# MCG-NJU/LinK

Hardware: AMD Instinct MI355X
Metric: voxels/s through one LinK (3x7)^3 block, 100k active voxels C=64 (higher is better)
Workload: dtype f32

## Files before the change

include/link_amd.h:

```cpp
#ifndef LINK_AMD_H_
#define LINK_AMD_H_

#include <stddef.h>
#include <stdint.h>

#ifdef __cplusplus
extern "C" {
#endif

#define LINK_OK 0
#define LINK_ERR_ARG (-1)
#define LINK_ERR_LAUNCH (-2)
#define LINK_ERR_WORKSPACE (-3)
#define LINK_BATCH_TIMEOUT (-4)

int link_abi_version(void);
int32_t link_abi_struct_size(int32_t which);
const char *link_last_error(void);


int link_hash(const int32_t *coords, int64_t n, int64_t *out, void *stream);

int link_kernel_hash(const int32_t *coords, int64_t n, const int32_t *offsets, int64_t k,
                     int64_t *out, void *stream);
// ... 70 lines not shown
                               const int32_t *counts, const int32_t *nbr_t, const float *denom,
                               int64_t n, int64_t m, int64_t c, int64_t k, float *g_new,
                               float *g_small, void *stream);
int link_aux_to_voxel_forward_grid(const float *small_f, const int32_t *counts, const int32_t *blk_coords,
                                   const int32_t *cell_blk, const link_grid_t *grid ,
                                   const int32_t *hdr, const int64_t *idx, int64_t n, int64_t m, int32_t w,
                                   int32_t r, float *S, float *new_feat, float *denom, float *out,
                                   void *stream);
int link_aux_to_voxel_forward_scatter(const float *small_f, const int32_t *counts, const int32_t *blk_coords,
                                      const int32_t *cell_blk, const link_grid_t *grid , const int32_t *hdr,
                                      const int32_t *blk_start, const int32_t *perm, int64_t n, int64_t m, int32_t w, int32_t r,
                                      float *S , float *denom, float *out, void *stream);


#define LINK_OP_COS 0
#define LINK_OP_SIN 1
#define LINK_OP_COSX 2

typedef struct {
  int32_t op;
  int32_t c;
  int32_t cg;
  int32_t r;
  float coord_div;
  float eps;
  int32_t flags;
} link_elk_desc_t;
#define LINK_ELK_LANE_CHANNEL 1
#define LINK_ELK_NO_PAIR 2
#define LINK_ELK_FUSED_GATHER 4
#define LINK_ELK_NO_DENSE_GRID 8
#define LINK_ELK_LEAN_CS 32
#define LINK_ELK_LEAN_NO_CS 64
#define LINK_ELK_LEAN_PM 128
#define LINK_ELK_LEAN_NO_PM 256
#define LINK_ELK_TILES 16

int link_premix_ln(const float *feats, const float *w_pre, const float *ln_w, const float *ln_b,
                   int64_t n, int32_t c, float eps, float *fin, void *stream);

int link_modulate_block_sum(const float *fin, const int32_t *vox_sorted, const float *w_pos,
                            const float *alpha, const int32_t *blk_start,
                            const int32_t *hdr, const link_elk_desc_t *desc , int64_t n,
                            int64_t m_cap, float *S, void *stream);

int link_gather_demod_ln(const float *S, const float *fin, const int32_t *vox_sorted,
                         const float *w_pos, const float *alpha, const float *ln_w, const float *ln_b,
                         const int32_t *blk_start, const int32_t *blk_coords,
                         const int32_t *cell_blk, const link_grid_t *grid ,
                         const int32_t *hdr, const link_elk_desc_t *desc , int64_t n,
                         int64_t m_cap, float *out, void *stream);

int link_block_gather(const float *S, const int32_t *blk_coords, const int32_t *cell_blk,
                      const link_grid_t *grid , const int32_t *hdr,
                      const link_elk_desc_t *desc , int64_t m_cap, float *A, void *stream);
int link_voxel_demod_ln(const float *A, const float *fin, const int32_t *vox_sorted,
                        const int32_t *pos_blk, const float *w_pos, const float *alpha, const float *ln_w,
                        const float *ln_b, const int32_t *hdr, const link_elk_desc_t *desc ,
                        int64_t n, float *out, void *stream);

typedef struct {
  const void *feats;
  const int32_t *coords;
  const float *w_pre, *pre_ln_w, *pre_ln_b;
  const float *w_pos, *alpha;
  const float *ln_w, *ln_b;
  uint32_t *cell_counts; void *scratch; size_t scratch_bytes;
  int32_t *cell_blk, *vox_blk; int64_t *idx_query; int32_t *perm, *vox_sorted, *pos_blk, *blk_start, *blk_coords, *counts, *hdr;
  float *fin;
  float *S;
  float *A;
  void *out;
  int64_t s_bytes;
  int32_t io_dtype;
  int32_t reserved;
  uint64_t *cell_pair;
} link_elk_buffers_t;

int64_t link_elk_tiles_table_bytes(const link_elk_desc_t *desc , int64_t n, int64_t m_cap);
int link_elk_premix_modsum_tiles(const float *feats, const int32_t *vox_sorted, const int32_t *pos_blk,
                                 const int32_t *blk_start, const int32_t *hdr, const float *w_pre,
                                 const float *pre_ln_w, const float *pre_ln_b, const float *w_pos, const float *alpha,
                                 const link_elk_desc_t *desc , int64_t n, int64_t m_cap, float *S,
                                 int64_t s_bytes, float *fin, void *stream);
int link_elk_gather_demod_tiles(const float *S, const float *fin, const int32_t *vox_sorted, const int32_t *pos_blk,
                                const int32_t *blk_coords, const int32_t *cell_blk, const link_grid_t *grid ,
                                const int32_t *hdr, const float *w_pos, const float *alpha, const float *ln_w,
                                const float *ln_b, const link_elk_desc_t *desc , int64_t n, int64_t m_cap,
                                float *out, void *stream);
int link_elk_premix_modsum_tiles_io(const void *feats, int32_t io_dtype, const int32_t *vox_sorted, const int32_t *pos_blk,
                                    const int32_t *blk_start, const int32_t *hdr, const float *w_pre, const float *pre_ln_w,
                                    const float *pre_ln_b, const float *w_pos, const float *alpha,
                                    const link_elk_desc_t *desc , int64_t n, int64_t m_cap, float *S,
                                    int64_t s_bytes, float *fin, void *stream);
int link_elk_gather_demod_tiles_io(const float *S, const float *fin, const int32_t *vox_sorted, const int32_t *pos_blk,
                                   const int32_t *blk_coords, const int32_t *cell_blk, const link_grid_t *grid ,
                                   const int32_t *hdr, const float *w_pos, const float *alpha, const float *ln_w,
                                   const float *ln_b, const link_elk_desc_t *desc , int64_t n, int64_t m_cap,
                                   void *out, int32_t io_dtype, void *stream);

int link_elk_core_forward(const link_elk_buffers_t *buf , const link_grid_t *grid ,
                          const link_elk_desc_t *desc , int64_t n, int64_t m_cap,
                          int32_t build_index, void *stream);

typedef struct {
  const void *feats;
  const int32_t *coords;
  const float *w_pre, *pre_ln_w, *pre_ln_b, *w_pos, *alpha, *ln_w, *ln_b;
  uint32_t *cnt, *cnt_prev;
  int32_t *list;
  int32_t *rec2;
  int32_t *occ, *occ_prev;
  uint32_t *ctrl, *ctrl_prev;
  float *X;
  float *S;
  int32_t *hdr;
  void *out;
  int64_t seg_cap;
  int32_t k;
  int32_t io_dtype;
  int32_t cnt_shift;
  int32_t reserved;
} link_lean_buffers_t;
int link_elk_core_lean_forward(const link_lean_buffers_t *buf , const link_grid_t *grid ,
                               const link_elk_desc_t *desc , int64_t n, int64_t n_prev, int32_t build_index,
                               void *stream);

int link_elk_mid_forward(const float *fin, const int32_t *vox_sorted, const int32_t *pos_blk,
                         const int32_t *blk_start, const int32_t *blk_coords, const int32_t *cell_blk,
                         const link_grid_t *grid , const int32_t *hdr, const float *w_pos,
                         const float *alpha, const link_elk_desc_t *desc , const float *ln_w,
                         const float *ln_b, int64_t n, int64_t m_cap, float *S, float *A, float *den,
                         float *out, void *stream);
int32_t link_elk_mid_partial_rows(void);
int link_elk_out_ln_backward(const float *g_out, const float *A, const float *fin, const int32_t *vox_sorted,
                             const int32_t *pos_blk, const float *w_pos, const float *alpha,
                             const float *ln_w, const int32_t *hdr, const link_elk_desc_t *desc ,
                             int64_t n, float *g_new, float *partials, void *stream);
int link_elk_mid_backward(const float *g_new, const float *fin, const float *A, const float *den,
                          const int32_t *vox_sorted, const int32_t *pos_blk, const int32_t *blk_start,
                          const int32_t *blk_coords, const int32_t *cell_blk,
                          const link_grid_t *grid , const int32_t *hdr, const float *w_pos,
                          const float *alpha, const link_elk_desc_t *desc , int64_t n, int64_t m_cap,
                          float *S, float *gS, float *g_fin, float *partials, void *stream);
int link_premix_ln_backward(const float *feats, const float *w_pre, const float *ln_w, const float *g_fin,
                            int64_t n, int32_t c, float eps, float *g_pre, float *g_feats, float *partials,
                            void *stream);
int link_ln_add_relu_forward(const float *x, const float *addend, const float *ln_w, const float *ln_b,
                             int64_t n, int32_t c, float eps, float *y, void *stream);
int link_ln_add_relu_backward(const float *g_y, const float *y, const float *x, const float *ln_w, int64_t n,
                              int32_t c, float eps, float *g_addend, float *g_x, float *partials, void *stream);
int link_premix_ln_io(const void *feats, int32_t io_dtype, const float *w_pre, const float *ln_w, const float *ln_b,
                      int64_t n, int32_t c, float eps, float *fin, void *stream);
int link_premix_ln_backward_io(const void *feats, int32_t io_dtype, const float *w_pre, const float *ln_w,
                               const float *g_fin, int64_t n, int32_t c, float eps, float *g_pre, void *g_feats,
                               float *partials, void *stream);
int link_ln_add_relu_forward_io(const void *x, int32_t io_dtype, const float *addend, const float *ln_w,
                                const float *ln_b, int64_t n, int32_t c, float eps, float *y, void *stream);
int link_ln_add_relu_backward_io(const float *g_y, const float *y, const void *x, int32_t io_dtype, const float *ln_w,
                                 int64_t n, int32_t c, float eps, float *g_addend, void *g_x, float *partials,
                                 void *stream);
int link_sum_partials(const float *p0, int32_t cols0, const float *p1, int32_t cols1, const float *p2,
                      int32_t cols2, int64_t rows, float *out, void *stream);

int link_subm_conv_forward(const float *feats, const int32_t *nbr, const float *w, const int32_t *order,
                           int64_t n, int32_t cin, int32_t cout, int32_t kvol, float *out, void *stream);
int link_subm_conv_ln_add_relu(const float *feats, const int32_t *nbr, const float *w, const int32_t *order,
                               int64_t n, int32_t cin, int32_t cout, int32_t kvol, const float *ln_w,
                               const float *ln_b, float eps, const float *addend, int32_t relu, float *out,
                               void *stream);
int32_t link_subm_conv_wgrad_chunks(void);
int link_subm_conv_wgrad(const float *feats, const float *gout, const int32_t *nbr_t, int64_t n, int32_t c,
                         int32_t kvol, float *partial, void *stream);
int link_subm_conv_wgrad_split(const float *feats, const float *gout, const int32_t *nbr_t, int64_t n, int32_t c, int32_t kvol,
                               int32_t chunks, int32_t centre_extra, float *partial, void *stream);
int link_subm_conv_wgrad_reduce(const float *partial, int32_t c, int32_t kvol, int32_t chunks, int32_t centre_extra, float *gw,
                                void *stream);

int link_conv_pairs_supported(int32_t cin, int32_t cout);
int link_conv_pairs_gemm(const float *feats, const int32_t *pair_in, const int32_t *wg_k, int64_t rows_pad,
                         const float *w, int32_t cin, int32_t cout, float *contrib, void *stream);
int link_conv_pairs_sum(const float *contrib, const int32_t *ext_start, const int32_t *ext_list, int64_t n,
                        int64_t n_direct, int32_t cout, const float *bias, const float *ln_w, const float *ln_b,
                        float eps, const float *addend, int32_t relu, float *out, void *stream);
int32_t link_conv_out_candidate_count(const int32_t *kernel, const int32_t *stride);
int link_conv_out_candidates(const int32_t *indices, int64_t n, const int32_t *kernel, const int32_t *stride,
                             const int32_t *padding, const int32_t *out_shape, int32_t *cand, void *stream);
int link_conv_site_table(const int32_t *indices, int64_t n, const int32_t *in_shape, int32_t batch, int32_t *table,
                         int32_t clear, void *stream);
int link_conv_gather_table(const int32_t *out_indices, int64_t m, const int32_t *kernel, const int32_t *stride,
                           const int32_t *padding, const int32_t *in_shape, int32_t batch, const int32_t *site_table,
                           int32_t *table, void *stream);
int32_t link_kmap_candidate_count(const int32_t *kernel, const int32_t *stride);
int link_kmap_out_candidates(const int32_t *coords, int64_t n, const int32_t *kernel, const int32_t *stride,
                             const int32_t *tensor_stride, const int32_t *lo, int32_t *cand, void *stream);
int link_kmap_box_table(const int32_t *rows, int64_t m, const int32_t *cell_tab, const link_grid_t *grid,
                        const int32_t *kernel, const int32_t *step, int32_t *table, void *stream);
int link_kmap_transpose(const int32_t *table, int64_t m, int32_t kvol, int64_t n_in, int32_t *back, void *stream);
int link_pair_plan_count(const int32_t *nbr, int64_t n, int32_t kvol, int32_t *wg_counts, int32_t *row_info, void *stream);
int link_pair_plan_fill(const int32_t *nbr, int64_t n, int32_t kvol, int32_t skip_centre, const int32_t *base_k,
                        const int32_t *wg_base, const int32_t *ext_start, int32_t *pair_in, int32_t *pair_out,
                        int32_t *ext_list, void *stream);
int link_pair_plan_layout(const int32_t *wg_counts, int64_t n, int32_t kvol, int32_t skip_centre, int64_t gran_cap,
                          int32_t *base_k, int32_t *wg_base, int32_t *gran_start, int32_t *wg_k, int32_t *hdr, void *stream);
int link_pair_plan_build(const int32_t *nbr, int64_t n, int32_t kvol, int32_t skip_centre, int64_t gran_cap, int32_t *wg_counts,
                         int32_t *row_info, int32_t *base_k, int32_t *wg_base, int32_t *gran_start, int32_t *wg_ext,
                         int32_t *wg_k, int32_t *hdr, int32_t *ext_start, int32_t *pair_in, int32_t *pair_out,
                         int32_t *ext_list, void *stream);
int link_conv_pairs_gemm_io(const void *feats, int32_t io_dtype, const int32_t *pair_in, const int32_t *wg_k, int64_t rows_pad,
                            const float *w, int32_t cin, int32_t cout, float *contrib, void *stream);
int link_conv_pairs_sum_io(const float *contrib, const int32_t *ext_start, const int32_t *ext_list, int64_t n,
                           int64_t n_direct, int32_t cout, const float *bias, const float *ln_w, const float *ln_b, float eps,
                           const void *addend, int32_t relu, void *out, int32_t io_dtype, void *stream);
int link_conv_centre_sum_io(const void *feats, const float *w, int32_t centre, const float *contrib, int64_t contrib_rows,
                            const int32_t *ext_start, const int32_t *ext_list, int64_t n, int32_t cin, int32_t cout,
                            const float *bias, const float *ln_w, const float *ln_b, float eps, const void *addend,
                            int32_t relu, void *out, int32_t io_dtype, void *stream);
int link_conv_pairs_gemm_split(const float *feats, const int32_t *pair_in, const int32_t *wg_k, int64_t rows_pad, const void *ws,
                               const float *w, const int32_t *w_big, int32_t cin, int32_t cout, float *contrib, void *stream);
int link_conv_pairs_gemm_amp(const void *feats, int32_t io_dtype, const int32_t *pair_in, const int32_t *wg_k, int64_t rows_pad,
                             const void *wt, int32_t cin, int32_t cout, void *contrib, int32_t contrib_dtype, void *stream);
int link_conv_centre_sum_amp(const void *feats, const void *wt, int32_t centre, const void *contrib, int32_t contrib_dtype,
                             int64_t contrib_rows, const int32_t *ext_start, const int32_t *ext_list, int64_t n, int32_t cin,
                             int32_t cout, const float *bias, const float *ln_w, const float *ln_b, float eps,
                             const void *addend, int32_t relu, void *out, int32_t io_dtype, void *stream);
int link_subm_conv_resident_amp(const void *feats, int32_t io_dtype, const int32_t *nbr, const void *wt, const int32_t *order,
                                int64_t n, int32_t cin, int32_t cout, int32_t kvol, const float *ln_w, const float *ln_b,
                                float eps, const void *addend, int32_t relu, void *out, void *stream);
int link_conv_pairs_wgrad(const float *feats, const float *gout, const int32_t *pair_in, const int32_t *pair_out,
                          const int32_t *wg_k, const int32_t *gran_start, int64_t rows_pad, int32_t kvol, int64_t n_direct,
                          int32_t cin, int32_t cout, float *partial, float *gw, void *stream);
int link_conv_centre_sum(const float *feats, const float *w, int32_t centre, const float *contrib,
                         int64_t contrib_rows, const int32_t *ext_start, const int32_t *ext_list, int64_t n, int32_t cin, int32_t cout,
                         const float *bias, const float *ln_w, const float *ln_b, float eps, const float *addend,
                         int32_t relu, float *out, void *stream);

typedef struct {
  int32_t s;
  int32_t lo[4];
  int32_t dim[4];
  int32_t pdim[3];
  int32_t k;
  int64_t vp;
} link_dc_grid_t;
int64_t link_dc_grid_from(const link_grid_t *grid, int32_t k, link_dc_grid_t *out);

#define LINK_HDR_STATUS_ACC 3

#define LINK_IO_F32 0
#define LINK_IO_F16 1
#define LINK_IO_BF16 2
typedef struct {
  int32_t k1_wgs;
  int32_t k2_zsplit;
  int32_t k1_lds_pad;
  int32_t k2_lds_pad;
  int32_t k1_form;
  int32_t k2_form;
  int32_t mode;
  int32_t reserved0;
  int32_t reserved;
  uint64_t *k1_dbg;
  uint64_t *k2_dbg;
} link_dc_tuning_t;

typedef struct {
  const void *feats;
  const int32_t *coords;
  const float *w_pre, *pre_ln_w, *pre_ln_b, *w_pos, *alpha, *ln_w, *ln_b;
  uint32_t *cnt;
  int32_t *slots;
  uint32_t *sid;
  int32_t *vrec;
  int32_t *vcell;
  int32_t *cell_n;
  int32_t *hdr;
  float *fin;
  float *S;
  float *A;
  void *out;
  int32_t io_dtype;
  link_dc_tuning_t tune;
} link_dc_buffers_t;

int link_dc_premix_insert(const float *feats, const int32_t *coords, const float *w_pre, const float *ln_w,
                          const float *ln_b, int64_t n, int32_t c, float eps, const link_dc_grid_t *g ,
                          int32_t insert, float *fin, uint32_t *cnt, int32_t *slots, int32_t *vrec,
                          int32_t *vcell, int32_t *hdr, void *stream);
int link_dc_modsum(const float *fin, const int32_t *slots, uint32_t *cnt, int32_t *cell_n, const float *w_pos,
                   const float *alpha, const link_elk_desc_t *desc , const link_dc_grid_t *g ,
                   int32_t warm, float *S, int32_t *hdr, void *stream);
int link_dc_gather(const float *S, const int32_t *cell_n, const link_elk_desc_t *desc ,
                   const link_dc_grid_t *g , float *A, void *stream);
int link_dc_index(const int32_t *coords, int64_t n, const link_dc_grid_t *g , uint32_t *cnt,
                  int32_t *slots, int32_t *vcell, int32_t *hdr, void *stream);
int link_dc_premix_modsum(const link_dc_buffers_t *buf , const link_dc_grid_t *g ,
                          const link_elk_desc_t *desc , int64_t n, int32_t warm, void *stream);
int link_dc_demod(const float *A, const float *fin, const int32_t *coords, const int32_t *vcell,
                  const float *w_pos, const float *alpha, const float *ln_w, const float *ln_b,
                  const link_elk_desc_t *desc , const link_dc_grid_t *g , int64_t n, void *out,
                  int32_t io_dtype, void *stream);
int link_dc_gather_demod(const link_dc_buffers_t *buf , const link_dc_grid_t *g ,
                         const link_elk_desc_t *desc , int64_t n, void *stream);
int link_elk_core_dense_forward(const link_dc_buffers_t *buf , const link_dc_grid_t *g ,
                                const link_elk_desc_t *desc , int64_t n, int32_t build_index,
                                void *stream);
int link_dc_index_probe(const link_dc_buffers_t *buf , const link_dc_grid_t *g , int64_t n, int32_t *stats,
                        void *stream);
int link_dc_index_ids(const int32_t *coords, int64_t n, const link_dc_grid_t *g , uint32_t *cnt,
                      uint32_t *sid, int32_t *vcell, int32_t *hdr, void *stream);

int32_t link_bn_partial_workgroups(int64_t n, int32_t c);
int link_bn_forward_stats(const float *x, int64_t n, int32_t c, float eps, float momentum, double *partial, float *mean,
                          float *invstd, float *running_mean, float *running_var, const float *weight ,
                          const float *bias , float *scale , float *shift, void *stream);
int link_bn_backward_reduce(const float *g, const float *x, const float *mean, const float *invstd, int64_t n, int32_t c,
                            double *partial, float *sum_g, float *sum_gx, const float *weight ,
                            float *coef , void *stream);
int link_bn_apply_forward(const float *x, const float *mean, const float *scale, const float *shift, int64_t n, int32_t c,
                          int32_t relu, float *y, void *stream);
int link_bn_backward_reduce_relu(const float *g, const float *x, const float *mean, const float *invstd, const float *scale,
                                 const float *shift, int64_t n, int32_t c, double *partial, float *sum_g, float *sum_gx,
                                 const float *weight , float *coef , void *stream);
int link_bn_apply_backward(const float *g, const float *x, const float *mean, const float *coef, const float *scale ,
                           const float *shift, int64_t n, int32_t c, float *gx, void *stream);
int link_bn_forward_stats_io(const void *x, int32_t io_dtype, int64_t n, int32_t c, float eps, float momentum, double *partial,
                             float *mean, float *invstd, float *running_mean, float *running_var, const float *weight,
                             const float *bias, float *scale, float *shift, void *stream);
int link_bn_apply_forward_io(const void *x, int32_t io_dtype, const float *mean, const float *scale, const float *shift, int64_t n,
                             int32_t c, int32_t relu, void *y, void *stream);
int link_bn_backward_reduce_io(const void *g, const void *x, int32_t io_dtype, const float *mean, const float *invstd, int64_t n,
                               int32_t c, double *partial, float *sum_g, float *sum_gx, const float *weight, float *coef,
                               void *stream);
int link_bn_backward_reduce_relu_io(const void *g, const void *x, int32_t io_dtype, const float *mean, const float *invstd,
                                    const float *scale, const float *shift, int64_t n, int32_t c, double *partial, float *sum_g,
                                    float *sum_gx, const float *weight, float *coef, void *stream);
int link_bn_apply_backward_io(const void *g, const void *x, int32_t io_dtype, const float *mean, const float *coef,
                              const float *scale , const float *shift, int64_t n, int32_t c, void *gx,
                              void *stream);

typedef struct link_block_ctx link_block_ctx_t;
int link_block_ctx_create(link_block_ctx_t **out);
int link_block_ctx_destroy(link_block_ctx_t *ctx);
int64_t link_pair_plan_arena(int64_t n, int32_t kvol, int32_t skip_centre, int64_t offs[11]);

int link_dc_neighbor_map(const int32_t *coords, int64_t n, const link_dc_grid_t *g , const uint32_t *cnt,
                         const int32_t *slots, int32_t step, int32_t *nbr, void *stream);

#define LINK_BLOCK_DONE 0
#define LINK_BLOCK_MISS 1
typedef struct {
  const link_dc_buffers_t *buf;
  const link_dc_grid_t *g;
  const link_elk_desc_t *desc;
  int64_t n;
  int32_t mean_max, cell_max;
  int32_t ts;
  int32_t subm;
  int32_t *nbr;
  int32_t *pair_arena;
  int64_t pair_arena_words;
  float *contrib;
  int64_t contrib_rows;
  const float *w;
  const void *ws;
  const int32_t *w_big;
  const float *nl_w, *nl_b;
  float nl_eps;
  int32_t flags;
  void *out;
  int32_t bbox[8];
  int32_t stats[4];
  int32_t verdict;
  int32_t reserved;
} link_block_args_t;
int link_elk_block_forward(link_block_ctx_t *ctx, link_block_args_t *args , void *stream);

typedef struct link_dc_batch link_dc_batch_t;
int link_dc_batch_create(link_dc_batch_t **out);
int link_dc_batch_destroy(link_dc_batch_t *ctx);
int link_elk_core_dense_forward_batch(link_dc_batch_t *ctx, const link_dc_buffers_t *frames ,
                                      const int64_t *n , int32_t nframes, const link_dc_grid_t *g ,
                                      const link_elk_desc_t *desc , void *stream);
int link_dc_batch_submit(link_dc_batch_t *ctx, const link_dc_buffers_t *frames , const int64_t *n ,
                         int32_t nframes, const link_dc_grid_t *g , const link_elk_desc_t *desc , void *stream,
                         int64_t *ticket );
int link_dc_batch_join(link_dc_batch_t *ctx, int64_t ticket, void *stream);
int link_dc_batch_status(link_dc_batch_t *ctx, int32_t *out );
int link_dc_batch_set_timing(link_dc_batch_t *ctx, int32_t on);
int link_dc_batch_kernel_times(link_dc_batch_t *ctx, int64_t ticket, float *ms );
int link_dc_batch_set_debug(link_dc_batch_t *ctx, uint64_t *k1_rows, uint64_t *k2_rows);
int link_streams_share_queue(void *stream_a, void *stream_b, double *delay_us );
int link_dc_batch_probe_streams(link_dc_batch_t *ctx, hipStream_t stream, double *delays_us );

#ifdef __cplusplus
}
#endif
#endif
```

link_amd/_lib.py:

```python
from __future__ import annotations

import ctypes
import os
from ctypes import POINTER, Structure, c_char_p, c_float, c_int, c_int32, c_int64, c_size_t, c_void_p

_HERE = os.path.dirname(os.path.abspath(__file__))
SO_PATH = os.path.join(_HERE, "lib", "liblink_amd.so")

LINK_OK, LINK_ERR_ARG, LINK_ERR_LAUNCH, LINK_ERR_WORKSPACE, LINK_BATCH_TIMEOUT = 0, -1, -2, -3, -4
HDR_M, HDR_STATUS, HDR_NVALID, HDR_STATUS_ACC, HDR_WORDS = 0, 1, 2, 3, 8
OP_COS, OP_SIN, OP_COSX = 0, 1, 2
ELK_LANE_CHANNEL, ELK_NO_PAIR, ELK_FUSED_GATHER, ELK_NO_DENSE_GRID, ELK_TILES = 1, 2, 4, 8, 16
ELK_LEAN_CS, ELK_LEAN_NO_CS, ELK_LEAN_PM, ELK_LEAN_NO_PM = 32, 64, 128, 256
IO_F32, IO_F16, IO_BF16 = 0, 1, 2
ABI_VERSION = 13
DEBUG = os.environ.get("LINK_AMD_DEBUG", "0") not in ("", "0")


class LinkGrid(Structure):
    _fields_ = [("s", c_int32), ("lo", c_int32 * 4), ("dim", c_int32 * 4)]

    @property
    def cells(self) -> int:
        v = 1
        for d in self.dim:
            v *= int(d)
        return v

    def key(self):
        return (int(self.s), tuple(int(x) for x in self.lo), tuple(int(x) for x in self.dim))


class LinkElkDesc(Structure):
    _fields_ = [("op", c_int32), ("c", c_int32), ("cg", c_int32), ("r", c_int32),
                ("coord_div", c_float), ("eps", c_float), ("flags", c_int32)]


class LinkElkBuffers(Structure):
    _fields_ = [(k, c_void_p) for k in ("feats", "coords", "w_pre", "pre_ln_w", "pre_ln_b", "w_pos", "alpha",
                                        "ln_w", "ln_b", "cell_counts", "scratch")] + \
               [("scratch_bytes", c_size_t)] + \
               [(k, c_void_p) for k in ("cell_blk", "vox_blk", "idx_query", "perm", "vox_sorted", "pos_blk", "blk_start",
                                        "blk_coords", "counts", "hdr", "fin", "S", "A", "out")] + \
               [("s_bytes", c_int64), ("io_dtype", c_int32), ("reserved", c_int32), ("cell_pair", c_void_p)]


class LinkDcGrid(Structure):
    _fields_ = [("s", c_int32), ("lo", c_int32 * 4), ("dim", c_int32 * 4), ("pdim", c_int32 * 3),
                ("k", c_int32), ("vp", c_int64)]

    @property
    def interior_cells(self) -> int:
        v = 1
        for d in self.dim:
            v *= int(d)
        return v


class LinkDcTuning(Structure):
    _fields_ = [(k, c_int32) for k in ("k1_wgs", "k2_zsplit", "k1_lds_pad", "k2_lds_pad", "k1_form", "k2_form", "mode",
                                       "reserved0", "reserved")] + [("k1_dbg", c_void_p), ("k2_dbg", c_void_p)]


class LinkDcBuffers(Structure):
    _fields_ = [(k, c_void_p) for k in ("feats", "coords", "w_pre", "pre_ln_w", "pre_ln_b", "w_pos", "alpha",
                                        "ln_w", "ln_b", "cnt", "slots", "sid", "vrec", "vcell", "cell_n", "hdr", "fin",
                                        "S", "A", "out")] + [("io_dtype", c_int32), ("tune", LinkDcTuning)]


class LinkLeanBuffers(Structure):
    _fields_ = [(k, c_void_p) for k in ("feats", "coords", "w_pre", "pre_ln_w", "pre_ln_b", "w_pos", "alpha", "ln_w", "ln_b",
                                        "cnt", "cnt_prev", "list", "rec2", "occ", "occ_prev", "ctrl", "ctrl_prev", "X", "S",
                                        "hdr", "out")] + [("seg_cap", c_int64), ("k", c_int32), ("io_dtype", c_int32), ("cnt_shift", c_int32), ("reserved", c_int32)]


LEAN_KMAX, LEAN_SEGS, LEAN_CHUNK = 352, 16, 32
BLOCK_DONE, BLOCK_MISS = 0, 1


class LinkBlockArgs(Structure):
    _fields_ = [("buf", POINTER(LinkDcBuffers)), ("g", POINTER(LinkDcGrid)), ("desc", POINTER(LinkElkDesc)), ("n", c_int64),
                ("mean_max", c_int32), ("cell_max", c_int32), ("ts", c_int32), ("subm", c_int32),
                ("nbr", c_void_p), ("pair_arena", c_void_p),
                ("pair_arena_words", c_int64), ("contrib", c_void_p), ("contrib_rows", c_int64), ("w", c_void_p), ("ws", c_void_p),
                ("w_big", c_void_p), ("nl_w", c_void_p), ("nl_b", c_void_p), ("nl_eps", c_float), ("flags", c_int32),
                ("out", c_void_p), ("bbox", c_int32 * 8), ("stats", c_int32 * 4), ("verdict", c_int32), ("reserved", c_int32)]


SIGNATURES = {
    "link_abi_version": (c_int, []),
    "link_abi_struct_size": (c_int32, [c_int32]),
    "link_last_error": (c_char_p, []),
    "link_hash": (c_int, [c_void_p, c_int64, c_void_p, c_void_p]),
    "link_kernel_hash": (c_int, [c_void_p, c_int64, c_void_p, c_int64, c_void_p, c_void_p]),
    "link_hash_query_workspace_bytes": (c_size_t, [c_int64]),
    "link_hash_query": (c_int, [c_void_p, c_int64, c_void_p, c_void_p, c_int64, c_void_p, c_void_p,
                                c_size_t, c_void_p]),
    "link_count": (c_int, [c_void_p, c_int64, c_void_p, c_int64, c_void_p]),
    "link_ti_weights": (c_int, [c_void_p, c_void_p, c_int64, c_float, c_void_p, c_void_p]),
    "link_voxelize_forward": (c_int, [c_void_p, c_void_p, c_void_p, c_int64, c_int64, c_int64, c_void_p,
                                      c_void_p]),
    "link_voxelize_backward": (c_int, [c_void_p, c_void_p, c_void_p, c_int64, c_int64, c_void_p, c_void_p]),
    "link_devoxelize_forward": (c_int, [c_void_p, c_void_p, c_void_p, c_int64, c_int64, c_int64, c_void_p,
                                        c_void_p]),
    "link_devoxelize_backward": (c_int, [c_void_p, c_void_p, c_void_p, c_int64, c_int64, c_int64, c_int64,
                                         c_void_p, c_void_p]),
    "link_grid_from_bounds": (c_int64, [POINTER(c_int32), POINTER(c_int32), c_int32, POINTER(LinkGrid)]),
    "link_coords_bbox": (c_int, [c_void_p, c_int64, c_void_p, c_void_p]),
    "link_index_scratch_bytes": (c_size_t, [c_int64, c_int64]),
    "link_index_build": (c_int, [c_void_p, c_int64, POINTER(LinkGrid), c_void_p, c_void_p, c_size_t,
                                 c_void_p, c_void_p, c_void_p, c_void_p, c_void_p, c_void_p, c_void_p,
                                 c_void_p, c_void_p, c_void_p, c_void_p]),
    "link_index_build_first": (c_int, [c_void_p, c_int64, POINTER(LinkGrid), c_void_p, c_void_p, c_size_t] + [c_void_p] * 11),
    "link_block_gather": (c_int, [c_void_p, c_void_p, c_void_p, POINTER(LinkGrid), c_void_p,
                                  POINTER(LinkElkDesc), c_int64, c_void_p, c_void_p]),
    "link_voxel_demod_ln": (c_int, [c_void_p, c_void_p, c_void_p, c_void_p, c_void_p, c_void_p, c_void_p,
                                    c_void_p, c_void_p, POINTER(LinkElkDesc), c_int64, c_void_p, c_void_p]),
    "link_neighbor_map": (c_int, [c_void_p, c_void_p, POINTER(LinkGrid), c_void_p, c_int64, c_int32,
                                  c_int32, c_int32, c_void_p, c_void_p]),
    "link_cell_table_build": (c_int, [c_void_p, c_int64, POINTER(LinkGrid), c_void_p, c_void_p, c_void_p]),
    "link_conv_site_table": (c_int, [c_void_p, c_int64, c_void_p, c_int32, c_void_p, c_int32, c_void_p]),
    "link_conv_gather_table": (c_int, [c_void_p, c_int64, c_void_p, c_void_p, c_void_p, c_void_p, c_int32, c_void_p, c_void_p,
                                       c_void_p]),
    "link_cell_table_clear": (c_int, [c_void_p, c_int64, POINTER(LinkGrid), c_void_p, c_void_p]),
    "link_block_mean": (c_int, [c_void_p, c_void_p, c_void_p, c_void_p, c_int64, c_int64, c_int64,
                                c_void_p, c_void_p]),
    "link_aux_to_voxel_forward": (c_int, [c_void_p, c_void_p, c_void_p, c_void_p, c_int64, c_int64,
                                          c_int64, c_int64, c_void_p, c_void_p, c_void_p, c_void_p]),
    "link_aux_to_voxel_backward": (c_int, [c_void_p, c_void_p, c_void_p, c_void_p, c_void_p, c_void_p,
                                           c_int64, c_int64, c_int64, c_int64, c_void_p, c_void_p,
                                           c_void_p]),
    "link_premix_ln": (c_int, [c_void_p, c_void_p, c_void_p, c_void_p, c_int64, c_int32, c_float,
                               c_void_p, c_void_p]),
    "link_modulate_block_sum": (c_int, [c_void_p, c_void_p, c_void_p, c_void_p, c_void_p,
                                        c_void_p, POINTER(LinkElkDesc), c_int64, c_int64, c_void_p,
                                        c_void_p]),
    "link_gather_demod_ln": (c_int, [c_void_p, c_void_p, c_void_p, c_void_p, c_void_p, c_void_p, c_void_p,
                                     c_void_p, c_void_p, c_void_p, POINTER(LinkGrid), c_void_p,
                                     POINTER(LinkElkDesc), c_int64, c_int64, c_void_p, c_void_p]),
    "link_elk_core_forward": (c_int, [POINTER(LinkElkBuffers), POINTER(LinkGrid), POINTER(LinkElkDesc),
                                      c_int64, c_int64, c_int32, c_void_p]),
    "link_elk_tiles_table_bytes": (c_int64, [POINTER(LinkElkDesc), c_int64, c_int64]),
    "link_elk_premix_modsum_tiles": (c_int, [c_void_p] * 10 + [POINTER(LinkElkDesc), c_int64, c_int64, c_void_p, c_int64,
                                             c_void_p, c_void_p]),
    "link_elk_gather_demod_tiles": (c_int, [c_void_p] * 6 + [POINTER(LinkGrid)] + [c_void_p] * 5 +
                                    [POINTER(LinkElkDesc), c_int64, c_int64, c_void_p, c_void_p]),
    "link_elk_premix_modsum_tiles_io": (c_int, [c_void_p, c_int32] + [c_void_p] * 9 + [POINTER(LinkElkDesc), c_int64, c_int64, c_void_p,
                                                c_int64, c_void_p, c_void_p]),
    "link_elk_gather_demod_tiles_io": (c_int, [c_void_p] * 6 + [POINTER(LinkGrid)] + [c_void_p] * 5 +
                                       [POINTER(LinkElkDesc), c_int64, c_int64, c_void_p, c_int32, c_void_p]),
    "link_elk_mid_forward": (c_int, [c_void_p] * 6 + [POINTER(LinkGrid), c_void_p, c_void_p, c_void_p,
                                     POINTER(LinkElkDesc), c_void_p, c_void_p, c_int64, c_int64] + [c_void_p] * 5),
    "link_elk_out_ln_backward": (c_int, [c_void_p] * 9 + [POINTER(LinkElkDesc), c_int64, c_void_p, c_void_p,
                                         c_void_p]),
    "link_subm_conv_forward": (c_int, [c_void_p, c_void_p, c_void_p, c_void_p, c_int64, c_int32, c_int32, c_int32,
                                       c_void_p, c_void_p]),
    "link_aux_to_voxel_forward_grid": (c_int, [c_void_p] * 4 + [POINTER(LinkGrid), c_void_p, c_void_p, c_int64,
                                               c_int64, c_int32, c_int32] + [c_void_p] * 5),
    "link_aux_to_voxel_forward_scatter": (c_int, [c_void_p] * 4 + [POINTER(LinkGrid), c_void_p, c_void_p, c_void_p, c_int64,
                                                  c_int64, c_int32, c_int32] + [c_void_p] * 4),
    "link_conv_pairs_supported": (c_int, [c_int32, c_int32]),
    "link_conv_pairs_gemm": (c_int, [c_void_p, c_void_p, c_void_p, c_int64, c_void_p, c_int32, c_int32, c_void_p, c_void_p]),
    "link_conv_pairs_sum": (c_int, [c_void_p, c_void_p, c_void_p, c_int64, c_int64, c_int32, c_void_p, c_void_p, c_void_p,
                                    c_float, c_void_p, c_int32, c_void_p, c_void_p]),
    "link_index_cells": (c_int, [c_void_p, c_int64, POINTER(LinkGrid), c_void_p, c_void_p, c_size_t, c_void_p, c_void_p, c_void_p,
                                 c_void_p, c_void_p, c_void_p]),
    "link_conv_out_candidate_count": (c_int32, [c_void_p, c_void_p]),
    "link_conv_out_candidates": (c_int, [c_void_p, c_int64, c_void_p, c_void_p, c_void_p, c_void_p, c_void_p, c_void_p]),
    "link_kmap_candidate_count": (c_int32, [c_void_p, c_void_p]),
    "link_kmap_out_candidates": (c_int, [c_void_p, c_int64, c_void_p, c_void_p, c_void_p, c_void_p, c_void_p, c_void_p]),
    "link_kmap_box_table": (c_int, [c_void_p, c_int64, c_void_p, POINTER(LinkGrid), c_void_p, c_void_p, c_void_p, c_void_p]),
    "link_kmap_transpose": (c_int, [c_void_p, c_int64, c_int32, c_int64, c_void_p, c_void_p]),
    "link_conv_pairs_gemm_io": (c_int, [c_void_p, c_int32, c_void_p, c_void_p, c_int64, c_void_p, c_int32, c_int32, c_void_p, c_void_p]),
    "link_conv_pairs_sum_io": (c_int, [c_void_p, c_void_p, c_void_p, c_int64, c_int64, c_int32, c_void_p, c_void_p, c_void_p,
                                       c_float, c_void_p, c_int32, c_void_p, c_int32, c_void_p]),
    "link_conv_centre_sum_io": (c_int, [c_void_p, c_void_p, c_int32, c_void_p, c_int64, c_void_p, c_void_p, c_int64, c_int32, c_int32,
                                        c_void_p, c_void_p, c_void_p, c_float, c_void_p, c_int32, c_void_p, c_int32, c_void_p]),
    "link_conv_pairs_gemm_amp": (c_int, [c_void_p, c_int32, c_void_p, c_void_p, c_int64, c_void_p, c_int32, c_int32, c_void_p, c_int32, c_void_p]),
    "link_conv_centre_sum_amp": (c_int, [c_void_p, c_void_p, c_int32, c_void_p, c_int32, c_int64, c_void_p, c_void_p, c_int64, c_int32, c_int32,
                                         c_void_p, c_void_p, c_void_p, c_float, c_void_p, c_int32, c_void_p, c_int32, c_void_p]),
    "link_bn_partial_workgroups": (c_int32, [c_int64, c_int32]),
    "link_bn_forward_stats": (c_int, [c_void_p, c_int64, c_int32, c_float, c_float, c_void_p, c_void_p, c_void_p, c_void_p, c_void_p,
                                      c_void_p, c_void_p, c_void_p, c_void_p, c_void_p]),
    "link_bn_backward_reduce": (c_int, [c_void_p, c_void_p, c_void_p, c_void_p, c_int64, c_int32, c_void_p, c_void_p, c_void_p,
                                        c_void_p, c_void_p, c_void_p]),
    "link_bn_apply_forward": (c_int, [c_void_p, c_void_p, c_void_p, c_void_p, c_int64, c_int32, c_int32, c_void_p, c_void_p]),
    "link_bn_backward_reduce_relu": (c_int, [c_void_p, c_void_p, c_void_p, c_void_p, c_void_p, c_void_p, c_int64, c_int32, c_void_p,
                                             c_void_p, c_void_p, c_void_p, c_void_p, c_void_p]),
    "link_bn_apply_backward": (c_int, [c_void_p, c_void_p, c_void_p, c_void_p, c_void_p, c_void_p, c_int64, c_int32, c_void_p, c_void_p]),
    "link_conv_pairs_gemm_split": (c_int, [c_void_p, c_void_p, c_void_p, c_int64, c_void_p, c_void_p, c_void_p, c_int32, c_int32, c_void_p, c_void_p]),
    "link_pair_plan_count": (c_int, [c_void_p, c_int64, c_int32, c_void_p, c_void_p, c_void_p]),
    "link_pair_plan_fill": (c_int, [c_void_p, c_int64, c_int32, c_int32, c_void_p, c_void_p, c_void_p, c_void_p, c_void_p, c_void_p,
                                    c_void_p]),
    "link_subm_conv_resident_amp": (c_int, [c_void_p, c_int32, c_void_p, c_void_p, c_void_p, c_int64, c_int32, c_int32, c_int32,
                                            c_void_p, c_void_p, c_float, c_void_p, c_int32, c_void_p, c_void_p]),
    "link_pair_plan_build": (c_int, [c_void_p, c_int64, c_int32, c_int32, c_int64] + [c_void_p] * 13),
    "link_pair_plan_layout": (c_int, [c_void_p, c_int64, c_int32, c_int32, c_int64, c_void_p, c_void_p, c_void_p, c_void_p, c_void_p,
                                      c_void_p]),
    "link_conv_pairs_wgrad": (c_int, [c_void_p, c_void_p, c_void_p, c_void_p, c_void_p, c_void_p, c_int64, c_int32, c_int64,
                                      c_int32, c_int32, c_void_p, c_void_p, c_void_p]),
    "link_conv_centre_sum": (c_int, [c_void_p, c_void_p, c_int32, c_void_p, c_int64, c_void_p, c_void_p, c_int64, c_int32, c_int32,
                                     c_void_p, c_void_p, c_void_p, c_float, c_void_p, c_int32, c_void_p, c_void_p]),
    "link_subm_conv_wgrad_chunks": (c_int32, []),
    "link_subm_conv_wgrad": (c_int, [c_void_p, c_void_p, c_void_p, c_int64, c_int32, c_int32, c_void_p, c_void_p]),
    "link_subm_conv_wgrad_split": (c_int, [c_void_p, c_void_p, c_void_p, c_int64, c_int32, c_int32, c_int32, c_int32, c_void_p, c_void_p]),
    "link_subm_conv_wgrad_reduce": (c_int, [c_void_p, c_int32, c_int32, c_int32, c_int32, c_void_p, c_void_p]),
    "link_subm_conv_ln_add_relu": (c_int, [c_void_p, c_void_p, c_void_p, c_void_p, c_int64, c_int32, c_int32, c_int32,
                                           c_void_p, c_void_p, c_float, c_void_p, c_int32, c_void_p, c_void_p]),
    "link_ln_add_relu_forward": (c_int, [c_void_p] * 4 + [c_int64, c_int32, c_float, c_void_p, c_void_p]),
    "link_ln_add_relu_backward": (c_int, [c_void_p] * 4 + [c_int64, c_int32, c_float] + [c_void_p] * 4),
    "link_sum_partials": (c_int, [c_void_p, c_int32, c_void_p, c_int32, c_void_p, c_int32, c_int64, c_void_p,
                                  c_void_p]),
    "link_premix_ln_backward": (c_int, [c_void_p] * 4 + [c_int64, c_int32, ctypes.c_float] + [c_void_p] * 4),
    "link_premix_ln_io": (c_int, [c_void_p, c_int32] + [c_void_p] * 3 + [c_int64, c_int32, c_float, c_void_p, c_void_p]),
    "link_premix_ln_backward_io": (c_int, [c_void_p, c_int32] + [c_void_p] * 3 + [c_int64, c_int32, c_float] + [c_void_p] * 4),
    "link_ln_add_relu_forward_io": (c_int, [c_void_p, c_int32] + [c_void_p] * 3 + [c_int64, c_int32, c_float, c_void_p, c_void_p]),
    "link_ln_add_relu_backward_io": (c_int, [c_void_p] * 3 + [c_int32, c_void_p, c_int64, c_int32, c_float] + [c_void_p] * 4),
    "link_bn_forward_stats_io": (c_int, [c_void_p, c_int32, c_int64, c_int32, c_float, c_float] + [c_void_p] * 10),
    "link_bn_apply_forward_io": (c_int, [c_void_p, c_int32, c_void_p, c_void_p, c_void_p, c_int64, c_int32, c_int32, c_void_p, c_void_p]),
    "link_bn_backward_reduce_io": (c_int, [c_void_p, c_void_p, c_int32, c_void_p, c_void_p, c_int64, c_int32] + [c_void_p] * 6),
    "link_bn_backward_reduce_relu_io": (c_int, [c_void_p, c_void_p, c_int32] + [c_void_p] * 4 + [c_int64, c_int32] + [c_void_p] * 6),
    "link_bn_apply_backward_io": (c_int, [c_void_p, c_void_p, c_int32] + [c_void_p] * 4 + [c_int64, c_int32, c_void_p, c_void_p]),
    "link_elk_mid_partial_rows": (c_int32, []),
    "link_dc_grid_from": (c_int64, [POINTER(LinkGrid), c_int32, POINTER(LinkDcGrid)]),
    "link_dc_premix_insert": (c_int, [c_void_p] * 5 + [c_int64, c_int32, c_float, POINTER(LinkDcGrid), c_int32] +
                              [c_void_p] * 7),
    "link_dc_modsum": (c_int, [c_void_p] * 6 + [POINTER(LinkElkDesc), POINTER(LinkDcGrid), c_int32, c_void_p,
                               c_void_p, c_void_p]),
    "link_dc_gather": (c_int, [c_void_p, c_void_p, POINTER(LinkElkDesc), POINTER(LinkDcGrid), c_void_p, c_void_p]),
    "link_elk_core_dense_forward": (c_int, [POINTER(LinkDcBuffers), POINTER(LinkDcGrid), POINTER(LinkElkDesc),
                                            c_int64, c_int32, c_void_p]),
    "link_elk_core_lean_forward": (c_int, [POINTER(LinkLeanBuffers), POINTER(LinkGrid), POINTER(LinkElkDesc), c_int64, c_int64,
                                           c_int32, c_void_p]),
    "link_dc_index_probe": (c_int, [POINTER(LinkDcBuffers), POINTER(LinkDcGrid), c_int64, c_void_p, c_void_p]),
    "link_dc_index_ids": (c_int, [c_void_p, c_int64, POINTER(LinkDcGrid)] + [c_void_p] * 5),
    "link_dc_index": (c_int, [c_void_p, c_int64, POINTER(LinkDcGrid)] + [c_void_p] * 5),
    "link_dc_premix_modsum": (c_int, [POINTER(LinkDcBuffers), POINTER(LinkDcGrid), POINTER(LinkElkDesc), c_int64,
                                      c_int32, c_void_p]),
    "link_dc_gather_demod": (c_int, [POINTER(LinkDcBuffers), POINTER(LinkDcGrid), POINTER(LinkElkDesc), c_int64, c_void_p]),
    "link_dc_demod": (c_int, [c_void_p] * 8 + [POINTER(LinkElkDesc), POINTER(LinkDcGrid), c_int64, c_void_p, c_int32,
                              c_void_p]),
    "link_block_ctx_create": (c_int, [POINTER(c_void_p)]),
    "link_block_ctx_destroy": (c_int, [c_void_p]),
    "link_pair_plan_arena": (c_int64, [c_int64, c_int32, c_int32, POINTER(c_int64)]),
    "link_dc_neighbor_map": (c_int, [c_void_p, c_int64, POINTER(LinkDcGrid), c_void_p, c_void_p, c_int32, c_void_p, c_void_p]),
    "link_elk_block_forward": (c_int, [c_void_p, POINTER(LinkBlockArgs), c_void_p]),
    "link_dc_batch_create": (c_int, [POINTER(c_void_p)]),
    "link_dc_batch_destroy": (c_int, [c_void_p]),
    "link_elk_core_dense_forward_batch": (c_int, [c_void_p, POINTER(LinkDcBuffers), POINTER(c_int64), c_int32, POINTER(LinkDcGrid),
                                                  POINTER(LinkElkDesc), c_void_p]),
    "link_dc_batch_submit": (c_int, [c_void_p, POINTER(LinkDcBuffers), POINTER(c_int64), c_int32, POINTER(LinkDcGrid),
                                     POINTER(LinkElkDesc), c_void_p, POINTER(c_int64)]),
    "link_dc_batch_join": (c_int, [c_void_p, c_int64, c_void_p]),
    "link_dc_batch_set_timing": (c_int, [c_void_p, c_int32]),
    "link_dc_batch_kernel_times": (c_int, [c_void_p, c_int64, POINTER(c_float)]),
    "link_dc_batch_status": (c_int, [c_void_p, POINTER(c_int32)]),
    "link_dc_batch_set_debug": (c_int, [c_void_p, c_void_p, c_void_p]),
    "link_dc_batch_probe_streams": (c_int, [c_void_p, c_void_p, POINTER(ctypes.c_double)]),
    "link_streams_share_queue": (c_int, [c_void_p, c_void_p, POINTER(ctypes.c_double)]),
    "link_elk_mid_backward": (c_int, [c_void_p] * 9 + [POINTER(LinkGrid), c_void_p, c_void_p, c_void_p,
                                      POINTER(LinkElkDesc), c_int64, c_int64] + [c_void_p] * 5),
}

_lib = None


class LinkAmdError(RuntimeError):
    pass


def lib() -> ctypes.CDLL:
    global _lib
    if _lib is None:
        if not os.path.exists(SO_PATH):
            raise LinkAmdError(
                f"{SO_PATH} not found: the HIP extension is not built. Run `python link_amd/build.py` "
                "(or __graft_entry__.build()). link_amd has no CPU/PyTorch fallback.")
        handle = ctypes.CDLL(SO_PATH)
        for name, (res, args) in SIGNATURES.items():
            fn = getattr(handle, name)
            fn.restype = res
            fn.argtypes = args
        if handle.link_abi_version() != ABI_VERSION:
            raise LinkAmdError("liblink_amd.so ABI version mismatch; rebuild with link_amd/build.py")
        for which, cls in enumerate((LinkGrid, LinkElkDesc, LinkElkBuffers, LinkDcGrid, LinkDcTuning, LinkDcBuffers, LinkLeanBuffers, LinkBlockArgs)):
            if handle.link_abi_struct_size(which) != ctypes.sizeof(cls):
                raise LinkAmdError(f"liblink_amd.so: layout of {cls.__name__} differs from include/link_amd.h "
                                   f"({ctypes.sizeof(cls)} bytes here, {handle.link_abi_struct_size(which)} in the library)")
        _lib = handle
    return _lib


def current_stream_handle() -> int:
    import torch
    try:
        return torch._C._cuda_getCurrentRawStream(torch._C._cuda_getDevice())
    except AttributeError:
        return torch.cuda.current_stream().cuda_stream


def check(rc: int, what: str) -> None:
    if rc != LINK_OK:
        msg = {LINK_ERR_ARG: "invalid argument", LINK_ERR_LAUNCH: "HIP launch failure",
               LINK_ERR_WORKSPACE: "workspace too small",
               LINK_BATCH_TIMEOUT: "a bounded wait inside a persistent batch kernel gave up"}.get(rc, f"error {rc}")
        detail = lib().link_last_error()
        raise LinkAmdError(f"{what}: {msg}" + (f" ({detail.decode()})" if detail else ""))


def grid_from_bounds(lo, hi, s: int) -> LinkGrid:
    g = LinkGrid()
    lo_a = (c_int32 * 4)(*[int(x) for x in lo])
    hi_a = (c_int32 * 4)(*[int(x) for x in hi])
    v = lib().link_grid_from_bounds(lo_a, hi_a, int(s), ctypes.byref(g))
    if v < 0:
        raise LinkAmdError(f"grid_from_bounds({list(lo)}, {list(hi)}, s={s}): bounds invalid or grid "
                           ">= 2^30 cells")
    return g


def dc_grid_from(grid: LinkGrid, k: int = 0):
    g = LinkDcGrid()
    v = lib().link_dc_grid_from(ctypes.byref(grid), int(k), ctypes.byref(g))
    return g if v > 0 else None
```

link_amd/csrc/dense_batch_impl.h:

```cpp
#include <stdlib.h>

#include <type_traits>
#include <vector>

#include "dense_batch_common.h"
#include "dense_gather.h"
#include "dense_io.h"

namespace DC_IO_NS {
using namespace link;

#include "dense_k1_impl.h"
#include "dense_k2_cfg.h"
#include "dense_gather_quad_impl.h"

static_assert(DC_ST_AUX == 16, "the S rows must leave the L2 (sc1) for the in-launch hand-off K1 -> K2");

struct dc_bt_frame_t {
  const void *feats; const int4 *coords; int4 *slots; uint32_t *cnt; int32_t *cell_n; int32_t *vcell; float *S; int32_t *hdr;
  void *out; int64_t n;
};
struct dc_bt_frames_t { dc_bt_frame_t f[DC_BT_MAX]; };
struct dc_bt_par_t {
  const float *w_pre, *pre_ln_w, *pre_ln_b, *w_pos, *ln_w, *ln_b;
  int cg; float eps;
  unsigned long long *dbg1, *dbg2;
};
__device__ __forceinline__ void bt_row(unsigned long long *dbg, unsigned long long r, unsigned long long a, unsigned long long b,
                                       unsigned long long c, unsigned long long d, unsigned long long e, unsigned long long f) {
  if (!DC_BT_PROF || !dbg) return;
  if (r + 1 >= dbg[1]) return;
  unsigned long long *o = dbg + 8 * (r + 1);
  o[0] = a; o[1] = b; o[2] = c; o[3] = d; o[4] = e; o[5] = f; o[6] = 1;
}


template <typename P>
__device__ __forceinline__ bool bt_wait_ge(P sync, int word, int target, const int nap = 8) {
  int ok = 1;
  if ((threadIdx.x & 63) == 0) {
    const unsigned long long t0 = __builtin_amdgcn_s_memrealtime();
    int spins = 0;
    while (__hip_atomic_load(&sync[word], __ATOMIC_RELAXED, __HIP_MEMORY_SCOPE_AGENT) < target) {
      if (nap > 8) __builtin_amdgcn_s_sleep(64); else __builtin_amdgcn_s_sleep(8);
      if ((++spins & 15) == 0) {
        if (__hip_atomic_load(&sync[bt_err()], __ATOMIC_RELAXED, __HIP_MEMORY_SCOPE_AGENT) != 0) { ok = 0; break; }
        if (__builtin_amdgcn_s_memrealtime() - t0 > DC_BT_TIMEOUT_TICKS) {
          __hip_atomic_store(&sync[bt_err()], 1 + word, __ATOMIC_RELAXED, __HIP_MEMORY_SCOPE_AGENT);
          ok = 0;
          break;
        }
      }
    }
  }
  return __builtin_amdgcn_readfirstlane(ok) != 0;
}

struct dc_bt_ins_args_t { dc_bt_frames_t fr; link_dc_grid_t g; int nframes, wpf; int32_t *sync; };
__global__ void __launch_bounds__(64) k_dc_batch_insert(dc_bt_ins_args_t args_by_value) {
  (void)args_by_value;
#if defined(__HIP_DEVICE_COMPILE__)
  typedef const __attribute__((address_space(4))) dc_bt_ins_args_t *args_ptr_t;
  for (;;) {
    args_ptr_t a = (args_ptr_t)__builtin_amdgcn_kernarg_segment_ptr();
    asm volatile("" : "+s"(a));
    int t = 0;
    if (threadIdx.x == 0) t = __hip_atomic_fetch_add(&a->sync[bt_inscur()], 1, __ATOMIC_RELAXED, __HIP_MEMORY_SCOPE_AGENT);
    t = __builtin_amdgcn_readfirstlane(t);
    const int wpf = a->wpf;
    if (t >= a->nframes * wpf) break;
    const int f = t / wpf, j = t - f * wpf;
    if (f >= DC_BT_INS_LEAD && !bt_wait_ge(a->sync, bt_k1(f - DC_BT_INS_LEAD), 1, 64)) break;
    const link_dc_grid_t g = a->g;
    const int n = (int)a->fr.f[f].n;
    const int4 *__restrict__ coords = a->fr.f[f].coords;
    int32_t *__restrict__ vcell = a->fr.f[f].vcell;
    int32_t *__restrict__ hdr = a->fr.f[f].hdr;
    const __amdgpu_buffer_rsrc_t r_slots = dc_rsrc(a->fr.f[f].slots, (uint32_t)((int64_t)g.vp * g.k * 16));
    const __amdgpu_buffer_rsrc_t r_cnt = dc_rsrc(a->fr.f[f].cnt, (uint32_t)(g.vp * 4));
    if (j == 0 && threadIdx.x == 0) hdr[LINK_HDR_NVALID] = n;
    _Pragma("unroll 1") for (int k = 0; k < 4; k++) {
      const int v = (4 * j + k) * 64 + (int)threadIdx.x;
      if (v >= n) break;
      const int4 rc = coords[v];
      const unsigned ux = (unsigned)(floordiv(rc.x, g.s) - g.lo[0]), uy = (unsigned)(floordiv(rc.y, g.s) - g.lo[1]);
      const unsigned uz = (unsigned)(floordiv(rc.z, g.s) - g.lo[2]), ub = (unsigned)(rc.w - g.lo[3]);
      const bool inside = ux < (unsigned)g.dim[0] && uy < (unsigned)g.dim[1] && uz < (unsigned)g.dim[2] && ub < (unsigned)g.dim[3];
      if (!inside) atomicOr(&hdr[LINK_HDR_STATUS_ACC], 1);
      const int pcell = inside ? dc_cell(g, (int)ux, (int)uy, (int)uz, (int)ub) : 0;
      const int rank = __builtin_amdgcn_raw_ptr_buffer_atomic_add_i32(1, r_cnt, pcell ? (uint32_t)pcell * 4u : DC_OOB, 0, 0);
      const bool full = pcell != 0 && rank >= g.k;
      if (full) atomicOr(&hdr[LINK_HDR_STATUS_ACC], 2);
      const bool keep = pcell != 0 && !full;
      st16i_c<true>(r_slots, keep ? dc_slot(g, pcell, rank) * 16u : DC_OOB, make_int4(rc.x, rc.y, rc.z, v));
      vcell[v] = keep ? pcell : 0;
    }
    asm volatile("s_waitcnt vmcnt(0)" ::: "memory");
    if (threadIdx.x == 0) __hip_atomic_fetch_add(&a->sync[bt_ins(f)], 1, __ATOMIC_RELAXED, __HIP_MEMORY_SCOPE_AGENT);
  }
#endif
}

template <int OP, int NB>
__global__ void __launch_bounds__(64 * DC_K1_NW, DC_K1_WAVES) k_dc_batch_k1(dc_bt_frames_t fr, dc_bt_par_t p, link_dc_grid_t g, int nframes,
                                                                           int cpw, int nranges, int wpf, int32_t *__restrict__ sync) {
  constexpr int C = 64;
  extern __shared__ __attribute__((aligned(16))) char smem_raw[];
  const int tid = threadIdx.x, lane = tid & 63;
  bool w_big = false, th_big = false;
  dc_k1_stage<C, OP>(smem_raw, p.w_pre, p.pre_ln_w, p.pre_ln_b, p.w_pos, nullptr, p.cg, 1.0f, g, tid, w_big, th_big);
  w_big = DC_K1_SPLIT ? (__syncthreads_or(w_big) != 0) : (__syncthreads(), false);
  const bool th_slow = DC_THETA_BOUND ? __syncthreads_or(th_big) != 0 : false;
  const int Vi = g.dim[0] * g.dim[1] * g.dim[2] * g.dim[3];
  const int x = (int)(__builtin_amdgcn_s_getreg((4 - 1) << 11 | 0 << 6 | 20) & 7u);
  const int per = (nranges + 7) >> 3;
  const int lo = x * per;
  const int mine = (lo + per < nranges ? lo + per : nranges) - lo;
  if (mine <= 0) return;
  const int total = nframes * mine;
  int32_t *cur = &sync[bt_k1cur(x)];
  int t_next = 0;
  if (lane == 0) t_next = __hip_atomic_fetch_add(cur, 1, __ATOMIC_RELAXED, __HIP_MEMORY_SCOPE_AGENT);
  int pend_f = -1;
  int ins_known = -1;
  for (;;) {
    const int t = __builtin_amdgcn_readfirstlane(t_next);
    if (t >= total) break;
    const unsigned long long tp0 = DC_BT_PROF ? __builtin_amdgcn_s_memrealtime() : 0;
    const int f = t / mine, i = lo + (t - f * mine);
    if (lane == 0) t_next = __hip_atomic_fetch_add(cur, 1, __ATOMIC_RELAXED, __HIP_MEMORY_SCOPE_AGENT);
    const dc_bt_frame_t &F = fr.f[f];
    int ins_a = wpf, ins_b = wpf;
    if (lane == 0) {
      if (f > ins_known) ins_a = __hip_atomic_load(&sync[bt_ins(f)], __ATOMIC_RELAXED, __HIP_MEMORY_SCOPE_AGENT);
      if (f + 1 < nframes && f + 1 > ins_known) ins_b = __hip_atomic_load(&sync[bt_ins(f + 1)], __ATOMIC_RELAXED, __HIP_MEMORY_SCOPE_AGENT);
    }
    const int c_begin = i * cpw;
    const int c_end = (c_begin + cpw < Vi) ? c_begin + cpw : Vi;
    int pc_f, nv_f;
    int4 rf0, rf1, rf2, rf3;
    if (f <= ins_known) dc_k1_prefetch<true>(pc_f, nv_f, rf0, rf1, rf2, rf3, g, F.slots, F.cnt, c_begin, c_end, lane);
    asm volatile("s_waitcnt vmcnt(0)" ::: "memory");
    if (pend_f >= 0 && lane == 0) __hip_atomic_fetch_add(&sync[bt_k1(pend_f)], 1, __ATOMIC_RELAXED, __HIP_MEMORY_SCOPE_AGENT);
    pend_f = f;
    if (f > ins_known) {
      if (__builtin_amdgcn_readfirstlane(ins_a) < wpf && !bt_wait_ge(sync, bt_ins(f), wpf)) return;
      ins_known = f;
      dc_k1_prefetch<true>(pc_f, nv_f, rf0, rf1, rf2, rf3, g, F.slots, F.cnt, c_begin, c_end, lane);
    }
    if (f + 1 < nframes && f + 1 > ins_known && __builtin_amdgcn_readfirstlane(ins_b) >= wpf) ins_known = f + 1;
    if (i == 0 && lane == 0) {
      F.hdr[LINK_HDR_STATUS] = __hip_atomic_load(&F.hdr[LINK_HDR_STATUS_ACC], __ATOMIC_RELAXED, __HIP_MEMORY_SCOPE_AGENT);
      __hip_atomic_store(&F.hdr[LINK_HDR_STATUS_ACC], 0, __ATOMIC_RELAXED, __HIP_MEMORY_SCOPE_AGENT);
    }
    const unsigned long long tp1 = DC_BT_PROF ? __builtin_amdgcn_s_memrealtime() : 0;
    dc_k1_range<C, OP, NB, false, true>(smem_raw, F.feats, F.slots, F.cnt, F.cell_n, p.w_pre, 1.0f, p.eps, F.n, g, false, F.S, nullptr,
                                        nullptr, c_begin, c_end, pc_f, nv_f, rf0, rf1, rf2, rf3, w_big, th_slow, i, 0, 0);
    if (DC_BT_PROF && lane == 0) bt_row(p.dbg1, (unsigned long long)f * nranges + i, (unsigned long long)f, (unsigned long long)i, tp0, tp1, __builtin_amdgcn_s_memrealtime(), (unsigned long long)(blockIdx.x * 4 + (tid >> 6)));
  }
  asm volatile("s_waitcnt vmcnt(0)" ::: "memory");
#if DC_BT_RELEASE_FENCE
  __builtin_amdgcn_fence(__ATOMIC_RELEASE, "agent");
  asm volatile("s_waitcnt vmcnt(0)" ::: "memory");
#endif
  if (pend_f >= 0 && lane == 0) __hip_atomic_fetch_add(&sync[bt_k1(pend_f)], 1, __ATOMIC_RELAXED, __HIP_MEMORY_SCOPE_AGENT);
}

struct dc_bt_k2_args_t {
  dc_bt_frames_t fr;
  dc_bt_par_t p;
  link_dc_grid_t g;
  int nframes, txn, tyn, zsplit, nwg, k1_target;
  int32_t *sync;
};

template <int OP, int R>
__global__ void __launch_bounds__(256 + 64 * (DC_K2Q_CW + (DC_K2Q_PMAP ? 1 : 0)), 4) k_dc_batch_k2(dc_bt_k2_args_t args_by_value) {
  (void)args_by_value;
#if defined(__HIP_DEVICE_COMPILE__)
  static_assert(DC_K2Q_PMAP == 1, "the mapper wave draws the items");
  typedef const __attribute__((address_space(4))) dc_bt_k2_args_t *args_ptr_t;
  constexpr unsigned CTL_THREAD = 256 + 64 * DC_K2Q_CW;
  __shared__ int s_ctl[2];
  const int x = (int)(__builtin_amdgcn_s_getreg((4 - 1) << 11 | 0 << 6 | 20) & 7u);
  int t_next = 0;
  if (threadIdx.x == CTL_THREAD) {
    args_ptr_t a = (args_ptr_t)__builtin_amdgcn_kernarg_segment_ptr();
    int32_t *sy = a->sync;
    const int per = (a->nwg + 7) >> 3;
    if (DC_BT_PROF)
      bt_row(a->p.dbg2, (unsigned long long)a->nframes * (8 * per) + blockIdx.x, 9999, 0, __builtin_amdgcn_s_memrealtime(), 0, 0, blockIdx.x);
    const int t = __hip_atomic_fetch_add(&sy[bt_cursor(x)], 1, __ATOMIC_RELAXED, __HIP_MEMORY_SCOPE_AGENT);
    t_next = __hip_atomic_fetch_add(&sy[bt_cursor(x)], 1, __ATOMIC_RELAXED, __HIP_MEMORY_SCOPE_AGENT);
    int f = t < a->nframes * per ? t / per : -1;
    if (f >= 0 && !bt_wait_ge(sy, bt_k1(f), a->k1_target)) f = -1;
    s_ctl[0] = f; s_ctl[1] = f >= 0 ? (t - f * per) * 8 + x : 0;
  }
  __syncthreads();
  for (;;) {
    args_ptr_t a = (args_ptr_t)__builtin_amdgcn_kernarg_segment_ptr();
    asm volatile("" : "+s"(a));
    const int f = __builtin_amdgcn_readfirstlane(s_ctl[0]), bid = __builtin_amdgcn_readfirstlane(s_ctl[1]);
    if (f < 0) break;
    const unsigned long long tq0 = DC_BT_PROF ? __builtin_amdgcn_s_memrealtime() : 0;
    __syncthreads();
    {
      const link_dc_grid_t g = a->g;
      unsigned tidx = threadIdx.x;
      asm volatile("" : "+v"(tidx));
      dc_k2q_body<OP, R, false, true>(a->fr.f[f].S, a->fr.f[f].cell_n, a->fr.f[f].slots, a->p.w_pos, nullptr, a->p.ln_w, a->p.ln_b, a->p.cg,
                                      1.0f, a->p.eps, a->fr.f[f].n, g, a->txn, a->tyn, a->zsplit, a->nwg, a->fr.f[f].out, nullptr, bid, tidx);
    }
    if (threadIdx.x == CTL_THREAD) {
      const unsigned long long tq1 = DC_BT_PROF ? __builtin_amdgcn_s_memrealtime() : 0;
      int32_t *sy = a->sync;
      const int per = (a->nwg + 7) >> 3;
      const int t = t_next;
      int fn = t < a->nframes * per ? t / per : -1;
      if (fn >= 0) {
        t_next = __hip_atomic_fetch_add(&sy[bt_cursor(x)], 1, __ATOMIC_RELAXED, __HIP_MEMORY_SCOPE_AGENT);
        if (!bt_wait_ge(sy, bt_k1(fn), a->k1_target)) fn = -1;
      }
      s_ctl[0] = fn; s_ctl[1] = fn >= 0 ? (t - fn * per) * 8 + x : 0;
      if (DC_BT_PROF) bt_row(a->p.dbg2, (unsigned long long)f * (8 * per) + bid, (unsigned long long)f, (unsigned long long)bid, tq0, tq1, __builtin_amdgcn_s_memrealtime(), (unsigned long long)blockIdx.x);
    }
    __syncthreads();
  }
#endif
}


template <int OP, int R>
static int batch_launch(const dc_bt_host_t &c, const dc_bt_frames_t &fr, const dc_bt_par_t &p, const link_dc_grid_t &g, const link_elk_desc_t &d,
                        int nframes, int64_t nmax) {
  using K1 = dc_k1_cfg<64, OP>;
  using KQ = dc_k2q_cfg<OP, R>;
  using KG = typename dc_k2_cfg<OP, R>::G;
  constexpr int LDS_GRAN = 1280, LDS_GRANS = 128, K1_STATIC = 256, K2_STATIC = 16;
  constexpr int k1_lds = 65 * LDS_GRAN - K1_STATIC;
  constexpr int k2_lds = KQ::LDS_BYTES;
  static_assert(k1_lds >= K1::LDS_BYTES && (k2_lds + K2_STATIC + LDS_GRAN - 1) / LDS_GRAN <= LDS_GRANS - 65, "LDS shaping of the two persistent roles");
  int32_t *sync = c.sync;
  const int64_t vi = (int64_t)g.dim[0] * g.dim[1] * g.dim[2] * g.dim[3];
  const int k1_wgs = c.cus;
  static const int rpw = [] { const char *e = getenv("LINK_DC_BATCH_RPW"); const int v = e ? atoi(e) : 1; return v < 1 ? 1 : (v > 16 ? 16 : v); }();
  int cpw = (int)((vi + (int64_t)k1_wgs * K1::NW * rpw - 1) / ((int64_t)k1_wgs * K1::NW * rpw));
  if (cpw < 1) cpw = 1;
  const int k1_target = (int)((vi + cpw - 1) / cpw);
  const int txn = (g.dim[0] + KG::TX - 1) / KG::TX, tyn = (g.dim[1] + KG::TY - 1) / KG::TY;
  static const int zs_env = [] { const char *e = getenv("LINK_DC_BATCH_ZSPLIT"); const int v = e ? atoi(e) : 1; return v < 1 ? 1 : (v > 8 ? 8 : v); }();
  int zsplit = zs_env;
  if (zsplit > g.dim[2]) zsplit = g.dim[2];
  const int64_t nwg = (int64_t)txn * tyn * g.dim[3] * zsplit;
  if (nwg > (1 << 20)) return LINK_ERR_ARG;
  int wpf = (int)((nmax + 255) / 256);
  if (wpf < 1) wpf = 1;
  (void)hipFuncSetAttribute(reinterpret_cast<const void *>(&k_dc_batch_k1<OP, 2>), hipFuncAttributeMaxDynamicSharedMemorySize, k1_lds);
  (void)hipFuncSetAttribute(reinterpret_cast<const void *>(&k_dc_batch_k2<OP, R>), hipFuncAttributeMaxDynamicSharedMemorySize, k2_lds);
  const int ins_wgs = c.cus;
  const dc_bt_ins_args_t a0{fr, g, nframes, wpf, sync};
  hipLaunchKernelGGL(k_dc_batch_insert, dim3((unsigned)ins_wgs * DC_BT_INS_WAVES), dim3(64), 0, c.sc, a0);
  int rc = check_launch("link_elk_core_dense_forward_batch (insert)");
  if (rc != LINK_OK) return rc;
  hipLaunchKernelGGL((k_dc_batch_k1<OP, 2>), dim3((unsigned)k1_wgs), dim3(64 * K1::NW), k1_lds, c.sa, fr, p, g, nframes, cpw, k1_target, wpf, sync);
  rc = check_launch("link_elk_core_dense_forward_batch (K1)");
  if (rc != LINK_OK) return rc;
  const dc_bt_k2_args_t a2{fr, p, g, nframes, txn, tyn, zsplit, (int)nwg, k1_target, sync};
  static_assert(sizeof(dc_bt_k2_args_t) <= 4096, "kernel arguments");
  hipLaunchKernelGGL((k_dc_batch_k2<OP, R>), dim3((unsigned)c.cus), dim3(KQ::THREADS), k2_lds, c.sb, a2);
  return check_launch("link_elk_core_dense_forward_batch (K2)");
}

int batch_set_launch(const dc_bt_host_t &c, const link_dc_buffers_t *frames, const int64_t *n, int nb, const link_dc_grid_t &g,
                     const link_elk_desc_t &d) {
  const link_dc_buffers_t &b0 = frames[0];
  const dc_bt_par_t p{b0.w_pre, b0.pre_ln_w, b0.pre_ln_b, b0.w_pos, b0.ln_w, b0.ln_b, d.cg, d.eps, c.dbg1, c.dbg2};
  dc_bt_frames_t fr{};
  int64_t nmax = 0;
  for (int i = 0; i < nb; i++) {
    const link_dc_buffers_t &b = frames[i];
    fr.f[i] = dc_bt_frame_t{b.feats, reinterpret_cast<const int4 *>(b.coords), reinterpret_cast<int4 *>(b.slots), b.cnt, b.cell_n, b.vcell, b.S,
                            b.hdr, b.out, n[i]};
    nmax = n[i] > nmax ? n[i] : nmax;
  }
  if (d.op == LINK_OP_COS) return d.r == 3 ? batch_launch<LINK_OP_COS, 3>(c, fr, p, g, d, nb, nmax) : batch_launch<LINK_OP_COS, 2>(c, fr, p, g, d, nb, nmax);
  return d.r == 3 ? batch_launch<LINK_OP_SIN, 3>(c, fr, p, g, d, nb, nmax) : batch_launch<LINK_OP_SIN, 2>(c, fr, p, g, d, nb, nmax);
}
}
```

link_amd/csrc/dense_fused.hip:

```cpp
#define DC_IO 0
#define DC_IO_NS dcio_f32
#include "dense_fused_impl.h"

using namespace link;

namespace link {
int dc_tiles_modsum(const link_dc_buffers_t *b, const link_dc_grid_t *g, const link_elk_desc_t *d, int64_t n, bool warm, hipStream_t st);
}

#define DC_DECL_IO(NS)                                                                                                    \
  namespace NS {                                                                                                           \
  int run_premix_modsum(const link_dc_buffers_t *, const link_dc_grid_t &, const link_elk_desc_t &, int64_t, bool,        \
                        hipStream_t);                                                                                      \
  int run_demod(const float *, const float *, const int32_t *, const int32_t *, const float *, const float *,             \
                const float *, const float *, const link_elk_desc_t &, const link_dc_grid_t &, int64_t, void *,            \
                hipStream_t);                                                                                              \
  int run_gather_demod(const link_dc_buffers_t *, const link_dc_grid_t &, const link_elk_desc_t &, int64_t, hipStream_t); \
  }
DC_DECL_IO(dcio_f16)
DC_DECL_IO(dcio_bf16)
#undef DC_DECL_IO

template <bool STATS>
#ifndef DC_INDEX_THREADS
#define DC_INDEX_THREADS 256
#endif
__global__ void __launch_bounds__(DC_INDEX_THREADS) k_dc_index(const int4 *__restrict__ coords, int64_t n, link_dc_grid_t g,
                                                  uint32_t *__restrict__ cnt, int4 *__restrict__ slots,
                                                  int32_t *__restrict__ vcell, int32_t *__restrict__ hdr,
                                                  int32_t *__restrict__ stats) {
  int st_in = 0, st_first = 0, st_max = 0;
  dc_index_body<STATS>(coords, n, g, cnt, slots, vcell, hdr, (int)blockIdx.x, (int)gridDim.x, DC_INDEX_THREADS, st_in, st_first, st_max);
  if (STATS) dc_index_stats_flush(stats, st_in, st_first, st_max);
}

extern "C" int link_dc_index(const int32_t *coords, int64_t n, const link_dc_grid_t *g, uint32_t *cnt,
                             int32_t *slots, int32_t *vcell, int32_t *hdr, void *stream) {
  if (n < 0 || !g) return LINK_ERR_ARG;
  if (n == 0) return LINK_OK;
  if (!coords || !cnt || !slots || !vcell || !hdr) return LINK_ERR_ARG;
  if (g->k < DC_INL || g->vp * (int64_t)g->k * 16 >= (1LL << 32) || n >= (1LL << 29)) return LINK_ERR_ARG;
  int64_t wgs = (n + DC_INDEX_THREADS - 1) / DC_INDEX_THREADS;
  if (wgs > 4096) wgs = 4096;
  hipLaunchKernelGGL(k_dc_index<false>, dim3((unsigned)wgs), dim3(DC_INDEX_THREADS), 0, S(stream), reinterpret_cast<const int4 *>(coords), n,
                     *g, cnt, reinterpret_cast<int4 *>(slots), vcell, hdr, (int32_t *)nullptr);
  return check_launch("link_dc_index");
}

__device__ __host__ inline int dc_probe_scratch_word(int i) {
  const int j = i >= 16 ? (i - 16) & 15 : -1;
  return (j >= 4 && j < 8) ? INT_MAX : ((j >= 8 && j < 12) ? INT_MIN : 0);
}
__global__ void k_dc_probe_scratch_init(int32_t *w) { w[threadIdx.x] = dc_probe_scratch_word((int)threadIdx.x); }
__global__ void __launch_bounds__(256) k_dc_index_probe_bbox(const int4 *__restrict__ coords, int64_t n, link_dc_grid_t g,
                                                             uint32_t *__restrict__ cnt, int4 *__restrict__ slots,
                                                             int32_t *__restrict__ vcell, int32_t *__restrict__ hdr,
                                                             int32_t *__restrict__ cur, int32_t *__restrict__ next,
                                                             int32_t *__restrict__ host, int seq) {
  const __amdgpu_buffer_rsrc_t r_slots = dc_rsrc(slots, (uint32_t)((int64_t)g.vp * g.k * 16));
  const __amdgpu_buffer_rsrc_t r_cnt = dc_rsrc(cnt, (uint32_t)(g.vp * 4));
  if (blockIdx.x == 0) {
    if (threadIdx.x == 0) hdr[LINK_HDR_NVALID] = (int32_t)n;
    for (int i = threadIdx.x; i < 272; i += 256) next[i] = dc_probe_scratch_word(i);
  }
  int st_in = 0, st_first = 0, st_max = 0;
  int mn[4] = {INT_MAX, INT_MAX, INT_MAX, INT_MAX}, mx[4] = {INT_MIN, INT_MIN, INT_MIN, INT_MIN};
  for (int64_t v = (int64_t)blockIdx.x * 256 + threadIdx.x; v < n; v += (int64_t)gridDim.x * 256) {
    const int4 rc = coords[v];
    mn[0] = min(mn[0], rc.x); mx[0] = max(mx[0], rc.x); mn[1] = min(mn[1], rc.y); mx[1] = max(mx[1], rc.y);
    mn[2] = min(mn[2], rc.z); mx[2] = max(mx[2], rc.z); mn[3] = min(mn[3], rc.w); mx[3] = max(mx[3], rc.w);
    const unsigned ux = (unsigned)(floordiv(rc.x, g.s) - g.lo[0]), uy = (unsigned)(floordiv(rc.y, g.s) - g.lo[1]);
    const unsigned uz = (unsigned)(floordiv(rc.z, g.s) - g.lo[2]), ub = (unsigned)(rc.w - g.lo[3]);
    const bool inside = ux < (unsigned)g.dim[0] && uy < (unsigned)g.dim[1] && uz < (unsigned)g.dim[2] && ub < (unsigned)g.dim[3];
    if (!inside) atomicOr(&hdr[LINK_HDR_STATUS_ACC], 1);
    const int pcell = inside ? dc_cell(g, (int)ux, (int)uy, (int)uz, (int)ub) : 0;
    const int rank = __builtin_amdgcn_raw_ptr_buffer_atomic_add_i32(1, r_cnt, pcell ? (uint32_t)pcell * 4u : DC_OOB, 0, 0);
    const bool full = pcell != 0 && rank >= g.k;
    if (full) atomicOr(&hdr[LINK_HDR_STATUS_ACC], 2);
    const bool keep = pcell != 0 && !full;
    st16i(r_slots, keep ? dc_slot(g, pcell, rank) * 16u : DC_OOB, make_int4(rc.x, rc.y, rc.z, (int)v));
    vcell[v] = keep ? pcell : 0;
    st_in += pcell != 0; st_first += (pcell != 0 && rank == 0); st_max = max(st_max, pcell != 0 ? rank + 1 : 0);
  }
#pragma unroll
  for (int o = 32; o > 0; o >>= 1) {
    st_in += __shfl_xor(st_in, o, 64); st_first += __shfl_xor(st_first, o, 64); st_max = max(st_max, __shfl_xor(st_max, o, 64));
#pragma unroll
    for (int a = 0; a < 4; a++) { mn[a] = min(mn[a], __shfl_xor(mn[a], o, 64)); mx[a] = max(mx[a], __shfl_xor(mx[a], o, 64)); }
  }
  __shared__ int s_part[4][11];
  __shared__ int s_last;
  const int lane = (int)(threadIdx.x & 63), wave = (int)(threadIdx.x >> 6);
  if (lane == 0) {
    s_part[wave][0] = st_in; s_part[wave][1] = st_first; s_part[wave][2] = st_max;
    for (int a = 0; a < 4; a++) { s_part[wave][3 + a] = mn[a]; s_part[wave][7 + a] = mx[a]; }
  }
  __syncthreads();
  if (threadIdx.x == 0) {
    int a_ = 0, f_ = 0, m_ = 0;
    for (int w = 0; w < 4; w++) { a_ += s_part[w][0]; f_ += s_part[w][1]; m_ = max(m_, s_part[w][2]); }
    int32_t *slot = cur + 16 + (blockIdx.x % DC_STATS_SLOTS) * 16;
    int dep = atomicAdd(&slot[0], a_) & 0;
    dep |= atomicAdd(&slot[1], f_) & 0;
    dep |= atomicMax(&slot[2], m_) & 0;
    for (int a = 0; a < 4; a++) {
      dep |= atomicMin(&slot[4 + a], min(min(s_part[0][3 + a], s_part[1][3 + a]), min(s_part[2][3 + a], s_part[3][3 + a]))) & 0;
      dep |= atomicMax(&slot[8 + a], max(max(s_part[0][7 + a], s_part[1][7 + a]), max(s_part[2][7 + a], s_part[3][7 + a]))) & 0;
    }
    asm volatile("s_waitcnt vmcnt(0)" ::: "memory");
    const int share = ((int)gridDim.x - 1 - (int)(blockIdx.x % DC_STATS_SLOTS)) / DC_STATS_SLOTS + 1;
    int last = 0;
    if (atomicAdd(&slot[3], 1 + dep) == share - 1) {
      const int live = (int)gridDim.x < DC_STATS_SLOTS ? (int)gridDim.x : DC_STATS_SLOTS;
      last = atomicAdd(&cur[8], 1) == live - 1;
    }
    s_last = last;
  }
  __syncthreads();
  if (!s_last) return;
  if (threadIdx.x < 64) {
    const int k = (int)threadIdx.x & 15;
    int32_t *slot = cur + 16 + k * 16;
    int vin = __hip_atomic_load(&slot[0], __ATOMIC_RELAXED, __HIP_MEMORY_SCOPE_AGENT);
    int vfi = __hip_atomic_load(&slot[1], __ATOMIC_RELAXED, __HIP_MEMORY_SCOPE_AGENT);
    int vmx = __hip_atomic_load(&slot[2], __ATOMIC_RELAXED, __HIP_MEMORY_SCOPE_AGENT);
    int bmn[4], bmx[4];
#pragma unroll
    for (int a = 0; a < 4; a++) {
      bmn[a] = __hip_atomic_load(&slot[4 + a], __ATOMIC_RELAXED, __HIP_MEMORY_SCOPE_AGENT);
      bmx[a] = __hip_atomic_load(&slot[8 + a], __ATOMIC_RELAXED, __HIP_MEMORY_SCOPE_AGENT);
    }
#pragma unroll
    for (int o = 8; o > 0; o >>= 1) {
      vin += __shfl_xor(vin, o, 64); vfi += __shfl_xor(vfi, o, 64); vmx = max(vmx, __shfl_xor(vmx, o, 64));
#pragma unroll
      for (int a = 0; a < 4; a++) { bmn[a] = min(bmn[a], __shfl_xor(bmn[a], o, 64)); bmx[a] = max(bmx[a], __shfl_xor(bmx[a], o, 64)); }
    }
    if (threadIdx.x == 0) {
#pragma unroll
      for (int a = 0; a < 4; a++) {
        __hip_atomic_store(&host[a], bmn[a], __ATOMIC_RELAXED, __HIP_MEMORY_SCOPE_SYSTEM);
        __hip_atomic_store(&host[4 + a], bmx[a], __ATOMIC_RELAXED, __HIP_MEMORY_SCOPE_SYSTEM);
      }
      __hip_atomic_store(&host[16], vin, __ATOMIC_RELAXED, __HIP_MEMORY_SCOPE_SYSTEM);
      __hip_atomic_store(&host[17], vfi, __ATOMIC_RELAXED, __HIP_MEMORY_SCOPE_SYSTEM);
      __hip_atomic_store(&host[18], vmx, __ATOMIC_RELAXED, __HIP_MEMORY_SCOPE_SYSTEM);
      __threadfence_system();
      __hip_atomic_store(&host[8], seq, __ATOMIC_RELEASE, __HIP_MEMORY_SCOPE_SYSTEM);
    }
  }
}

namespace link {
int dc_probe_scratch_init_run(int32_t *w, hipStream_t st) {
  hipLaunchKernelGGL(k_dc_probe_scratch_init, dim3(1), dim3(272), 0, st, w);
  return check_launch("link_elk_block_forward (init)");
}
int dc_index_probe_bbox_run(const link_dc_buffers_t *b, const link_dc_grid_t *g, int64_t n, int32_t *cur, int32_t *next,
                            int32_t *host_dev, int seq, hipStream_t st) {
  if (!b->coords || !b->cnt || !b->slots || !b->vcell || !b->hdr || !cur || !next || !host_dev) return LINK_ERR_ARG;
  if (g->k < DC_INL || g->vp * (int64_t)g->k * 16 >= (1LL << 32) || n >= (1LL << 29) || n <= 0) return LINK_ERR_ARG;
  int64_t wgs = (n + 255) / 256;
  if (wgs > 4096) wgs = 4096;
  hipLaunchKernelGGL(k_dc_index_probe_bbox, dim3((unsigned)wgs), dim3(256), 0, st, reinterpret_cast<const int4 *>(b->coords), n, *g, b->cnt,
                     reinterpret_cast<int4 *>(b->slots), b->vcell, b->hdr, cur, next, host_dev, seq);
  return check_launch("link_elk_block_forward (probe)");
}
}

__device__ __forceinline__ int dc_floordiv_fast(int a, int s, float inv) {
  if (__builtin_expect(a >= (1 << 22) || a <= -(1 << 22), 0)) return link::floordiv(a, s);
  int q = (int)floorf((float)a * inv);
  const int r = a - q * s;
  q += (r >= s ? 1 : 0) - (r < 0 ? 1 : 0);
  return q;
}
template <bool COUNT>
__global__ void __launch_bounds__(768) k_dc_neighbor_map(const int4 *__restrict__ coords, int64_t n, link_dc_grid_t g,
                                                         const uint32_t *__restrict__ cnt, const int4 *__restrict__ slots, int step,
                                                         int32_t *__restrict__ nbr, int32_t *__restrict__ wg_counts,
                                                         int32_t *__restrict__ row_info) {
  __shared__ int32_t tile[256 * 27];
  __shared__ int32_t wcnt[4 * 28];
  const int64_t row0 = (int64_t)blockIdx.x * 256;
  const int rows = (int)((n - row0 < 256) ? n - row0 : 256);
  const int r = (int)threadIdx.x / 3, kx = (int)threadIdx.x - 3 * r;
  if (r < rows) {
    const int4 c = coords[row0 + r];
    const float inv = 1.0f / (float)g.s;
    const int tx = c.x + (kx - 1) * step;
    const unsigned ux = (unsigned)(dc_floordiv_fast(tx, g.s, inv) - g.lo[0]), ub = (unsigned)(c.w - g.lo[3]);
    const bool okx = ux < (unsigned)g.dim[0] && ub < (unsigned)g.dim[3];
    const int bz = dc_floordiv_fast(c.z, g.s, inv);
    const int rz = c.z - bz * g.s;
    const bool lowc = rz - step < 0, upc = rz + step >= g.s;
    const unsigned uzA = (unsigned)(bz - g.lo[2]);
    const unsigned uzB = (unsigned)((lowc ? dc_floordiv_fast(c.z - step, g.s, inv) : dc_floordiv_fast(c.z + step, g.s, inv)) - g.lo[2]);
    const unsigned uzU = (unsigned)(dc_floordiv_fast(c.z + step, g.s, inv) - g.lo[2]);
    const bool hasB = lowc || upc, both = lowc && upc;
    const bool any_both = __any(both);
#pragma unroll
    for (int ky = 0; ky < 3; ky++) {
      const int ty = c.y + (ky - 1) * step;
      const unsigned uy = (unsigned)(dc_floordiv_fast(ty, g.s, inv) - g.lo[1]);
      int f[3] = {-1, -1, -1};
      const bool okxy = okx && uy < (unsigned)g.dim[1];
      auto take = [&](const int4 &q) {
        if (q.x == tx && q.y == ty) {
          const int d = q.z - c.z;
          if (d == -step && (f[0] < 0 || q.w < f[0])) f[0] = q.w;
          if (d == 0 && (f[1] < 0 || q.w < f[1])) f[1] = q.w;
          if (d == step && (f[2] < 0 || q.w < f[2])) f[2] = q.w;
        }
      };
      const int pcA = (okxy && uzA < (unsigned)g.dim[2]) ? link::dc_cell(g, (int)ux, (int)uy, (int)uzA, (int)ub) : 0;
      const int pcB = (okxy && hasB && uzB < (unsigned)g.dim[2]) ? link::dc_cell(g, (int)ux, (int)uy, (int)uzB, (int)ub) : 0;
      int nA = (int)cnt[pcA], nB = (int)cnt[pcB];
      const int4 *iA = slots + (int64_t)pcA * DC_INL, *iB = slots + (int64_t)pcB * DC_INL;
      const int4 rA[4] = {iA[0], iA[1], iA[2], iA[3]}, rB[4] = {iB[0], iB[1], iB[2], iB[3]};
      nA = pcA ? (nA < g.k ? nA : g.k) : 0;
      nB = pcB ? (nB < g.k ? nB : g.k) : 0;
#pragma unroll
      for (int j = 0; j < 4; j++) {
        if (j < nA) take(rA[j]);
        if (j < nB) take(rB[j]);
      }
      for (int j = DC_INL; j < nA; j++) take(slots[link::dc_slot(g, pcA, j)]);
      for (int j = DC_INL; j < nB; j++) take(slots[link::dc_slot(g, pcB, j)]);
      if (any_both) {
        const int pcU = (okxy && both && uzU < (unsigned)g.dim[2]) ? link::dc_cell(g, (int)ux, (int)uy, (int)uzU, (int)ub) : 0;
        int nU = pcU ? (int)cnt[pcU] : 0;
        nU = nU < g.k ? nU : g.k;
        for (int j = 0; j < nU; j++) take(slots[link::dc_slot(g, pcU, j)]);
      }
      int32_t *o = tile + r * 27 + kx + 3 * ky;
      o[0] = f[0]; o[9] = f[1]; o[18] = f[2];
    }
  }
  __syncthreads();
  {
    const int tot = rows * 27;
    int32_t *dst = nbr + row0 * 27;
    if ((reinterpret_cast<uintptr_t>(nbr) & 15) == 0) {
      for (int e = threadIdx.x; e < (tot >> 2); e += 768) reinterpret_cast<int4 *>(dst)[e] = reinterpret_cast<const int4 *>(tile)[e];
      for (int e = (tot & ~3) + threadIdx.x; e < tot; e += 768) dst[e] = tile[e];
    } else {
      for (int e = threadIdx.x; e < tot; e += 768) dst[e] = tile[e];
    }
  }
  if (!COUNT) return;
  const int rr = (int)threadIdx.x;
  if (rr < 256) {
    const bool live = rr < rows;
    const int32_t *mine = tile + (live ? rr : 0) * 27;
    const int lane = rr & 63, wave = rr >> 6;
    int nvalid = 0, cvalid = 0;
    for (int k = 0; k < 27; k++) {
      const int v = live ? mine[k] : -1;
      const bool valid = v >= 0;
      if (k == 13) {
        cvalid = valid ? 1 : 0;
        const unsigned long long bad = __ballot(live && v != (int)(row0 + rr));
        if (lane == 0) wcnt[wave * 28 + 27] = __popcll(bad);
      }
      const unsigned long long m = __ballot(valid);
      if (lane == 0) wcnt[wave * 28 + k] = __popcll(m);
      nvalid += valid ? 1 : 0;
    }
    if (live) row_info[row0 + rr] = nvalid | (cvalid << 16);
  }
  __syncthreads();
  if (rr <= 27) wg_counts[(int64_t)blockIdx.x * 28 + rr] = wcnt[rr] + wcnt[28 + rr] + wcnt[56 + rr] + wcnt[84 + rr];
}

static int dc_neighbor_map_run(const int32_t *coords, int64_t n, const link_dc_grid_t *g, const uint32_t *cnt, const int32_t *slots,
                               int32_t step, int32_t *nbr, int32_t *wg_counts, int32_t *row_info, hipStream_t st) {
  if (n < 0 || !g || step <= 0) return LINK_ERR_ARG;
  if (n == 0) return LINK_OK;
  if (!coords || !cnt || !slots || !nbr || n * 27 >= (1LL << 31)) return LINK_ERR_ARG;
  const unsigned wgs = (unsigned)((n + 255) / 256);
  if (wg_counts && row_info)
    hipLaunchKernelGGL(k_dc_neighbor_map<true>, dim3(wgs), dim3(768), 0, st, reinterpret_cast<const int4 *>(coords), n, *g, cnt,
                       reinterpret_cast<const int4 *>(slots), (int)step, nbr, wg_counts, row_info);
  else
    hipLaunchKernelGGL(k_dc_neighbor_map<false>, dim3(wgs), dim3(768), 0, st, reinterpret_cast<const int4 *>(coords), n, *g, cnt,
                       reinterpret_cast<const int4 *>(slots), (int)step, nbr, (int32_t *)nullptr, (int32_t *)nullptr);
  return link::check_launch("link_dc_neighbor_map");
}
extern "C" int link_dc_neighbor_map(const int32_t *coords, int64_t n, const link_dc_grid_t *g, const uint32_t *cnt,
                                    const int32_t *slots, int32_t step, int32_t *nbr, void *stream) {
  return dc_neighbor_map_run(coords, n, g, cnt, slots, step, nbr, nullptr, nullptr, link::S(stream));
}
namespace link {
int dc_neighbor_map_count_run(const int32_t *coords, int64_t n, const link_dc_grid_t *g, const uint32_t *cnt, const int32_t *slots,
                              int32_t step, int32_t *nbr, int32_t *wg_counts, int32_t *row_info, hipStream_t st) {
  if (!wg_counts || !row_info) return LINK_ERR_ARG;
  return dc_neighbor_map_run(coords, n, g, cnt, slots, step, nbr, wg_counts, row_info, st);
}
}

namespace link {
int dc_index_stats_run(const link_dc_buffers_t *b, const link_dc_grid_t *g, int64_t n, int32_t *stats, hipStream_t st) {
  if (!b->coords || !b->cnt || !b->slots || !b->vcell || !b->hdr) return LINK_ERR_ARG;
  if (g->k < DC_INL || g->vp * (int64_t)g->k * 16 >= (1LL << 32) || n >= (1LL << 29)) return LINK_ERR_ARG;
  int64_t wgs = (n + DC_INDEX_THREADS - 1) / DC_INDEX_THREADS;
  if (wgs > 4096) wgs = 4096;
  hipLaunchKernelGGL(k_dc_index<true>, dim3((unsigned)wgs), dim3(DC_INDEX_THREADS), 0, st, reinterpret_cast<const int4 *>(b->coords), n, *g, b->cnt,
                     reinterpret_cast<int4 *>(b->slots), b->vcell, b->hdr, stats);
  return check_launch("link_dc_index_probe");
}
}

static int dc_common_ok(const link_dc_buffers_t *b, const link_dc_grid_t *g, const link_elk_desc_t *d, int64_t n) {
  if (!b || !g || !d || n < 0) return LINK_ERR_ARG;
  if (b->io_dtype < 0 || b->io_dtype > 2) return LINK_ERR_ARG;
  if (d->op < 0 || d->op > 2 || d->cg <= 0 || d->c % d->cg != 0 || g->k < DC_INL) return LINK_ERR_ARG;
  const int parts = d->op == LINK_OP_COSX ? 3 : 2;
  if ((g->vp + 1) * (int64_t)parts * d->c * 4 >= (1LL << 32) || g->vp * (int64_t)g->k * 16 >= (1LL << 32)) return LINK_ERR_ARG;
  if (n * (int64_t)d->c * 4 >= (1LL << 32)) return LINK_ERR_ARG;
  return LINK_OK;
}

extern "C" int link_dc_premix_modsum(const link_dc_buffers_t *b, const link_dc_grid_t *g, const link_elk_desc_t *d,
                                     int64_t n, int32_t warm, void *stream) {
  if (dc_common_ok(b, g, d, n) != LINK_OK) return LINK_ERR_ARG;
  if (d->c != 16 && d->c != 32 && d->c != 64) return LINK_ERR_ARG;
  if (g->k > 352) return LINK_ERR_ARG;
  if (d->op == LINK_OP_COSX && !b->fin) return LINK_ERR_ARG;
  if (n == 0) return LINK_OK;
  if (!b->feats || !b->slots || !b->cnt || !b->cell_n || !b->w_pre || !b->pre_ln_w || !b->pre_ln_b || !b->w_pos ||
      !b->S || !b->hdr)
    return LINK_ERR_ARG;
  hipStream_t st = S(stream);
  if (b->tune.k1_form == 1) return dc_tiles_modsum(b, g, d, n, warm != 0, st);
  switch (b->io_dtype) {
    case 1: return dcio_f16::run_premix_modsum(b, *g, *d, n, warm != 0, st);
    case 2: return dcio_bf16::run_premix_modsum(b, *g, *d, n, warm != 0, st);
    default: return dcio_f32::run_premix_modsum(b, *g, *d, n, warm != 0, st);
  }
}

extern "C" int link_dc_demod(const float *A, const float *fin, const int32_t *coords, const int32_t *vcell,
                             const float *w_pos, const float *alpha, const float *ln_w, const float *ln_b,
                             const link_elk_desc_t *d, const link_dc_grid_t *g, int64_t n, void *out, int32_t io_dtype,
                             void *stream) {
  if (!d || !g || n < 0 || !dc_width_ok(d->c) || d->op < 0 || d->op > 2 || d->cg <= 0 || d->c % d->cg != 0) return LINK_ERR_ARG;
  if (io_dtype < 0 || io_dtype > 2) return LINK_ERR_ARG;
  if (n == 0) return LINK_OK;
  if (!A || !coords || !vcell || !w_pos || !ln_w || !ln_b || !out || (d->op == LINK_OP_COSX && !fin)) return LINK_ERR_ARG;
  const int parts = d->op == LINK_OP_COSX ? 3 : 2;
  if ((g->vp + 1) * (int64_t)parts * d->c * 4 >= (1LL << 32) || n * (int64_t)d->c * 4 >= (1LL << 32)) return LINK_ERR_ARG;
  hipStream_t st = S(stream);
  switch (io_dtype) {
    case 1: return dcio_f16::run_demod(A, fin, coords, vcell, w_pos, alpha, ln_w, ln_b, *d, *g, n, out, st);
    case 2: return dcio_bf16::run_demod(A, fin, coords, vcell, w_pos, alpha, ln_w, ln_b, *d, *g, n, out, st);
    default: return dcio_f32::run_demod(A, fin, coords, vcell, w_pos, alpha, ln_w, ln_b, *d, *g, n, out, st);
  }
}

extern "C" int link_dc_gather_demod(const link_dc_buffers_t *b, const link_dc_grid_t *g, const link_elk_desc_t *d,
                                    int64_t n, void *stream) {
  if (dc_common_ok(b, g, d, n) != LINK_OK || !dc_width_ok(d->c) || (d->r != 2 && d->r != 3)) return LINK_ERR_ARG;
  if (n == 0) return LINK_OK;
  if (!b->S || !b->cell_n || !b->slots || !b->w_pos || !b->ln_w || !b->ln_b || !b->out || (d->op == LINK_OP_COSX && !b->fin))
    return LINK_ERR_ARG;
  hipStream_t st = S(stream);
  if (d->c != 64) return LINK_ERR_ARG;
  switch (b->io_dtype) {
    case 1: return dcio_f16::run_gather_demod(b, *g, *d, n, st);
    case 2: return dcio_bf16::run_gather_demod(b, *g, *d, n, st);
    default: return dcio_f32::run_gather_demod(b, *g, *d, n, st);
  }
}
```

link_amd/csrc/dense_fused_impl.h:

```cpp
#pragma once
#include <type_traits>

#include "dense_gather.h"
#include "dense_io.h"

namespace DC_IO_NS {
using namespace link;

#include "dense_k1_impl.h"

template <int C, int OP, int NB, bool PIPE>
static int launch_k1p(const link_dc_buffers_t *b, const link_dc_grid_t &g, const link_elk_desc_t &d, int64_t n,
                     bool warm, hipStream_t st) {
  using K = dc_k1_cfg<C, OP>;
  const int64_t vi = (int64_t)g.dim[0] * g.dim[1] * g.dim[2] * g.dim[3];
  int64_t waves = (int64_t)(b->tune.k1_wgs > 0 ? b->tune.k1_wgs : 512) * 4;
  int cpw = (int)((vi + waves - 1) / waves);
  if (cpw < 1) cpw = 1;
  const int64_t wgs = (vi + (int64_t)cpw * K::NW - 1) / ((int64_t)cpw * K::NW);
  int k1_pad = b->tune.k1_lds_pad;
  k1_pad = k1_pad < 0 ? 0 : (k1_pad > 16384 ? 16384 : k1_pad);
  const int lds_k1 = K::LDS_BYTES + k1_pad <= 160 * 1024 ? K::LDS_BYTES + k1_pad : K::LDS_BYTES;
  if (lds_k1 > 64 * 1024)
    (void)hipFuncSetAttribute(reinterpret_cast<const void *>(&k_dc_premix_modsum<C, OP, NB, PIPE>),
// ... 497 lines not shown
  const int tid = threadIdx.x & 255, lane = tid & 63, wave = __builtin_amdgcn_readfirstlane((threadIdx.x & 255) >> 6);
  const int per = (nwg + 7) >> 3;
  const int L = (blockIdx.x & 7) * per + (blockIdx.x >> 3);
  if (L >= nwg) return;
  int t = L;
  const int zseg = t % zsplit; t /= zsplit;
  const int ty = t % tyn; t /= tyn;
  const int tx = t % txn;
  const int b = t / txn;
  const int Dx = g.dim[0], Dy = g.dim[1], Dz = g.dim[2];
  const int PDx = g.pdim[0], PDy = g.pdim[1], PDz = g.pdim[2];
  const int x0 = tx * TX, y0 = ty * TY;
  const int zs = (int)(((long long)Dz * zseg) / zsplit), ze = (int)(((long long)Dz * (zseg + 1)) / zsplit);
  if (zs >= ze) return;
  const int nplanes = (ze - zs) + R - 1;
  const int pz0 = zs + 1 - HLO;
  auto col_cell0 = [&](int hx, int hy) {
    int px = x0 + 1 - HLO + hx, py = y0 + 1 - HLO + hy;
    px = px < PDx - 1 ? px : PDx - 1;
    py = py < PDy - 1 ? py : PDy - 1;
    return (uint32_t)(((b * PDx + px) * PDy + py) * PDz);
  };
  uint32_t src_off[K::PASSES];
#pragma unroll
  for (int i = 0; i < K::PASSES; i++) {
    int pid = i * 256 + tid;
    if (pid >= K::NPC) pid = K::NPC - 1;
    const int col = pid / K::RP, pcs = pid % K::RP;
    src_off[i] = col_cell0(col / HY, col % HY) * (uint32_t)RB + (uint32_t)pcs * 16u;
  }
  uint32_t cnt_cell0;
  {
    int e = wave * 64 + lane;
    if (e >= K::NCOL) e = K::NCOL - 1;
    cnt_cell0 = col_cell0(e / HY, e % HY);
  }
  uint32_t rec_cell0;
  int rec_k;
  {
    const int piece = wave * 16 + (lane & 15);
    const int col = piece >> 2;
    rec_k = piece & 3;
    rec_cell0 = col_cell0(col / TY + HLO, col % TY + HLO);
  }
  const char *Sb = reinterpret_cast<const char *>(S_);
  auto issue = [&](int plane) {
    int pz = pz0 + plane;
    pz = pz < PDz - 1 ? pz : PDz - 1;
    char *buf = lds + (plane % 3) * K2::SPLIT_BUF_BYTES;
#pragma unroll
    for (int i = 0; i < K::PASSES; i++) {
      const bool surplus = (i * 256 + wave * 64) >= K::NPC;
      const int ii = surplus ? 0 : i;
      const char *src = Sb + (size_t)(surplus ? src_off[0] : src_off[i]) + (size_t)pz * RB;
      __builtin_amdgcn_global_load_lds((const __attribute__((address_space(1))) void *)src,
                                       (__attribute__((address_space(3))) void *)(buf + (ii * 256 + wave * 64) * 16), 16, 0, 0);
    }
    const int32_t *csrc = cell_n + cnt_cell0 + pz;
    __builtin_amdgcn_global_load_lds((const __attribute__((address_space(1))) void *)csrc,
                                     (__attribute__((address_space(3))) void *)(buf + K2::SPLIT_PLANE + wave * 256), 4, 0, 0);
    int po = pz0 + plane - (R - 1) + HLO;
    po = po < 0 ? 0 : (po < PDz - 1 ? po : PDz - 1);
    const int4 *rsrc = slots + ((size_t)(rec_cell0 + po) * DC_INL + rec_k);
    if (lane < 16)
      __builtin_amdgcn_global_load_lds((const __attribute__((address_space(1))) void *)rsrc,
                                       (__attribute__((address_space(3))) void *)(lds + K2::SPLIT_REC_OFF + (plane & 3) * K2::REC_BYTES + wave * 256), 16, 0, 0);
  };
  const int grp = tid >> 4, li = tid & 15;
  const int ix = grp / TY, iy = grp % TY;
  const bool col_ok = (x0 + ix < Dx) && (y0 + iy < Dy);
  const uint32_t lds_base = (uint32_t)(size_t)(__attribute__((address_space(3))) char *)lds;
  const uint32_t row_lane = (uint32_t)((ix * HY + iy) * RB + li * 16);
  const uint32_t cnt_lane = (uint32_t)((ix * HY + iy) * 4);
  const uint32_t abuf0 = lds_base + K2::SPLIT_ABUF_OFF, ncnt0 = lds_base + K2::SPLIT_NCNT_OFF;
  const int rowbase = lane & ~15;
  const int ch0 = 4 * li;
  const bool hi = PAIR && li >= 8;
  const __amdgpu_buffer_rsrc_t r_out = dc_rsrc(out, (uint32_t)(n * C * IO_BYTES));
  float w0[4], w1[4], w2[4], al[4], gw[4], gb[4];
#pragma unroll
  for (int e = 0; e < 4; e++) {
    const int ch = ch0 + e, tc = ch % cg;
    w0[e] = w_pos[3 * tc + 0]; w1[e] = w_pos[3 * tc + 1]; w2[e] = w_pos[3 * tc + 2];
    al[e] = alpha ? alpha[tc] : 1.0f;
    gw[e] = ln_w[ch]; gb[e] = ln_b[ch];
  }
  float4 r0[P], r1[P];
  float c0 = 0.f, c1 = 0.f;
  int n_prev = 0;
#pragma unroll
  for (int pp = 0; pp < P; pp++) r0[pp] = r1[pp] = make_float4(0.f, 0.f, 0.f, 0.f);
  auto pairs_of = [&](int jp, int pstart) {
      if (DC_K2_ABL & 4) return;
      const uint32_t abuf = abuf0 + (uint32_t)((jp & 1) * K2::NG * RB), ncnt = ncnt0 + (uint32_t)((jp & 1) * K2::NG * 4);
      const int po = pz0 + jp - (R - 1) + HLO;
      const int nli = lds_rd_b32(ncnt + (uint32_t)(li * 4));
      int incl = nli;
      incl += __builtin_amdgcn_update_dpp(0, incl, 0x111, 0xF, 0xF, true);
      incl += __builtin_amdgcn_update_dpp(0, incl, 0x112, 0xF, 0xF, true);
      incl += __builtin_amdgcn_update_dpp(0, incl, 0x114, 0xF, 0xF, true);
      incl += __builtin_amdgcn_update_dpp(0, incl, 0x118, 0xF, 0xF, true);
      const int Tv = __builtin_amdgcn_readlane(incl, 15);
      const int npair = single ? Tv : (Tv + 1) >> 1;
      const uint32_t recb = lds_base + (uint32_t)(K2::SPLIT_REC_OFF + (jp & 3) * K2::REC_BYTES);
      for (int p = pstart; p < npair; p += DC_K2_SECOND_ROUND ? 32 : 16) {
        if (dbg) tq_iters++;
        const int vA = single ? p : 2 * p, vB = (!single && 2 * p + 1 < Tv) ? 2 * p + 1 : vA;
        const bool hasB = !single && 2 * p + 1 < Tv;
        const unsigned long long mA = __ballot(incl <= vA), mB = __ballot(incl <= vB);
        const int cA = __popc((unsigned)(mA >> rowbase) & 0xFFFFu), cB = __popc((unsigned)(mB >> rowbase) & 0xFFFFu);
        const int eA = cA ? __shfl(incl, rowbase + cA - 1, 64) : 0, eB = cB ? __shfl(incl, rowbase + cB - 1, 64) : 0;
        const int kA = vA - eA, kB = vB - eB;
        v4f_t qa, qb;
        v4f_t A0v, A1v, B0v, B1v, A2v = {0.f, 0.f, 0.f, 0.f}, B2v = {0.f, 0.f, 0.f, 0.f};
        lds_rd6_b128(recb + (uint32_t)((cA * DC_INL + (kA < DC_INL ? kA : 0)) * 16),
                     recb + (uint32_t)((cB * DC_INL + (kB < DC_INL ? kB : 0)) * 16),
                     abuf + (uint32_t)(cA * RB + li * 16), abuf + (uint32_t)(cA * RB + C * 4 + li * 16),
                     abuf + (uint32_t)(cB * RB + li * 16), abuf + (uint32_t)(cB * RB + C * 4 + li * 16), qa, qb, A0v, A1v, B0v, B1v);
        int4 recA = make_int4(__float_as_int(qa.x), __float_as_int(qa.y), __float_as_int(qa.z), __float_as_int(qa.w));
        int4 recB = make_int4(__float_as_int(qb.x), __float_as_int(qb.y), __float_as_int(qb.z), __float_as_int(qb.w));
        if (kA >= DC_INL || kB >= DC_INL) {
          const int pcA = ((b * PDx + x0 + cA / TY + 1) * PDy + y0 + cA % TY + 1) * PDz + po;
          const int pcB = ((b * PDx + x0 + cB / TY + 1) * PDy + y0 + cB % TY + 1) * PDz + po;
          if (kA >= DC_INL) recA = slots[dc_slot(g, pcA, kA)];
          if (kB >= DC_INL) recB = slots[dc_slot(g, pcB, kB)];
        }
        float4 fx = make_float4(0.f, 0.f, 0.f, 0.f), fy = fx;
        if (OP == LINK_OP_COSX) {
          lds_rd2_b128(abuf + (uint32_t)(cA * RB + 2 * C * 4 + li * 16), abuf + (uint32_t)(cB * RB + 2 * C * 4 + li * 16), A2v, B2v);
          fx = *reinterpret_cast<const float4 *>(&fin[(int64_t)recA.w * C + ch0]);
          fy = *reinterpret_cast<const float4 *>(&fin[(int64_t)recB.w * C + ch0]);
        }
        float thA[4], thB[4];
        bool big = false;
        {
          const bool swapped = PAIR && hi && hasB;
          float xa = (float)(swapped ? recB.x : recA.x), ya = (float)(swapped ? recB.y : recA.y), za = (float)(swapped ? recB.z : recA.z);
          float xb = (float)recB.x, yb = (float)recB.y, zb = (float)recB.z;
          if (DIV) { xa = xa / coord_div; ya = ya / coord_div; za = za / coord_div; xb = xb / coord_div; yb = yb / coord_div; zb = zb / coord_div; }
#pragma unroll
          for (int e = 0; e < 4; e++) {
            thA[e] = theta_of(xa, ya, za, w0[e], w1[e], w2[e], al[e]);
            thB[e] = PAIR ? thA[e] : theta_of(xb, yb, zb, w0[e], w1[e], w2[e], al[e]);
            big |= !(fabsf(thA[e]) < 32768.0f) || !(fabsf(thB[e]) < 32768.0f);
          }
        }
        float snA[4], csA[4], snB[4], csB[4];
        if (__builtin_expect(__any(big), 0)) {
#pragma unroll
          for (int e = 0; e < 4; e++) {
            sincos_nocall(thA[e], snA[e], csA[e]);
            if (PAIR) { snB[e] = snA[e]; csB[e] = csA[e]; } else sincos_nocall(thB[e], snB[e], csB[e]);
          }
        } else {
#pragma unroll
          for (int e = 0; e < 4; e++) {
            if (DC_K2_ABL & 1) { snA[e] = thA[e]; csA[e] = 1.0f - thA[e]; snB[e] = thB[e]; csB[e] = 1.0f - thB[e]; continue; }
            sincos_small(thA[e], snA[e], csA[e]);
            if (PAIR) { snB[e] = snA[e]; csB[e] = csA[e]; } else sincos_small(thB[e], snB[e], csB[e]);
          }
        }
        if (PAIR) {
          const bool swapped = hi && hasB;
#pragma unroll
          for (int e = 0; e < 4; e++) {
            const float sn = snA[e], cs = csA[e];
            const float so = partner<LPR>(sn), co = partner<LPR>(cs);
            snA[e] = swapped ? so : sn; csA[e] = swapped ? co : cs;
            snB[e] = hi ? sn : so;      csB[e] = hi ? cs : co;
          }
        }
        const float fxa[4] = {fx.x, fx.y, fx.z, fx.w}, fya[4] = {fy.x, fy.y, fy.z, fy.w};
        float nvA[4], nvB[4], sA = 0.f, sB = 0.f;
#pragma unroll
        for (int e = 0; e < 4; e++) {
          const float A0 = A0v[e], A1 = A1v[e], B0 = B0v[e], B1 = B1v[e];
          if (OP == LINK_OP_SIN) {
            nvA[e] = __fsub_rn(__fmul_rn(A0, csA[e]), __fmul_rn(A1, snA[e]));
            nvB[e] = __fsub_rn(__fmul_rn(B0, csB[e]), __fmul_rn(B1, snB[e]));
          } else {
            nvA[e] = __fadd_rn(__fmul_rn(A0, csA[e]), __fmul_rn(A1, snA[e]));
            nvB[e] = __fadd_rn(__fmul_rn(B0, csB[e]), __fmul_rn(B1, snB[e]));
          }
          if (OP == LINK_OP_COSX) {
            nvA[e] = __fadd_rn(nvA[e], __fsub_rn(A2v[e], link_mul_rn(fxa[e], thA[e])));
            nvB[e] = __fadd_rn(nvB[e], __fsub_rn(B2v[e], link_mul_rn(fya[e], thB[e])));
          }
          sA += nvA[e]; sB += nvB[e];
        }
        if (!(DC_K2_ABL & 2)) { sA = grp_sum<LPR>(sA); sB = grp_sum<LPR>(sB); }
        const float meanA = sA * (1.0f / C), meanB = sB * (1.0f / C);
        float qA = 0.f, qB = 0.f;
#pragma unroll
        for (int e = 0; e < 4; e++) {
          const float dA = nvA[e] - meanA, dB = nvB[e] - meanB;
          qA += dA * dA; qB += dB * dB;
        }
        if (!(DC_K2_ABL & 2)) { qA = grp_sum<LPR>(qA); qB = grp_sum<LPR>(qB); }
        const float rsA = __builtin_amdgcn_rsqf(qA * (1.0f / C) + eps), rsB = __builtin_amdgcn_rsqf(qB * (1.0f / C) + eps);
        float4 oa, ob;
        oa.x = (nvA[0] - meanA) * rsA * gw[0] + gb[0]; oa.y = (nvA[1] - meanA) * rsA * gw[1] + gb[1];
        oa.z = (nvA[2] - meanA) * rsA * gw[2] + gb[2]; oa.w = (nvA[3] - meanA) * rsA * gw[3] + gb[3];
        ob.x = (nvB[0] - meanB) * rsB * gw[0] + gb[0]; ob.y = (nvB[1] - meanB) * rsB * gw[1] + gb[1];
        ob.z = (nvB[2] - meanB) * rsB * gw[2] + gb[2]; ob.w = (nvB[3] - meanB) * rsB * gw[3] + gb[3];
        io_st4(r_out, (uint32_t)recA.w * (uint32_t)C + (uint32_t)ch0, !(DC_K2_ABL & 8) || oa.x == 123.456f, oa);
        io_st4(r_out, (uint32_t)recB.w * (uint32_t)C + (uint32_t)ch0, (!(DC_K2_ABL & 8) || ob.x == 123.456f) && hasB, ob);
      }
  };
  if (producer) {
    issue(0);
    if (nplanes > 1) issue(1);
  }
  for (int i = 0; i <= nplanes; i++) {
    unsigned long long tqa = dbg ? __builtin_amdgcn_s_memtime() : 0;
    if (producer) {
      if (i + 1 < nplanes) wait_vmcnt<K2::NI>(); else wait_vmcnt<0>();
      asm volatile("s_waitcnt lgkmcnt(0)" ::: "memory");
    }
    if (dbg) { const unsigned long long tqb = __builtin_amdgcn_s_memtime(); tq_dma += tqb - tqa; tqa = tqb; }
    asm volatile("s_barrier" ::: "memory");
    if (dbg) { const unsigned long long tqb = __builtin_amdgcn_s_memtime(); tq_bar += tqb - tqa; tqa = tqb; }
    if (producer && i >= nplanes) {
      if (DC_K2_SECOND_ROUND && i - 1 >= R - 1) pairs_of(i - 1, grp + 16);
      if (dbg) { const unsigned long long tqb = __builtin_amdgcn_s_memtime(); tq_pairs += tqb - tqa; }
      continue;
    }
    if (producer && i + 2 < nplanes) issue(i + 2);
    const uint32_t bufa = lds_base + (uint32_t)((i % 3) * K2::SPLIT_BUF_BYTES);
    const int j = producer ? i : i - 1;
    const uint32_t abuf = abuf0 + (uint32_t)((j & 1) * K2::NG * RB), ncnt = ncnt0 + (uint32_t)((j & 1) * K2::NG * 4);
    if (!producer) {
      if (j >= R - 1 && j < nplanes) pairs_of(j, grp);
      if (dbg) { const unsigned long long tqb = __builtin_amdgcn_s_memtime(); tq_pairs += tqb - tqa; }
      continue;
    }
    float4 cur[P];
    float cc = 0.f;
    int n_here = 0;
#pragma unroll
    for (int pp = 0; pp < P; pp++) cur[pp] = make_float4(0.f, 0.f, 0.f, 0.f);
    {
      const uint32_t ra = bufa + row_lane, ca = bufa + (uint32_t)K2::SPLIT_PLANE + cnt_lane;
      if constexpr (P == 2 && R == 3 && DC_K2_PIPE_READS) {
        dc_read_plane_p2r3<C>(ra, ca, cur, cc);
      } else {
        dc_read_dx<C, P, R, 0>(ra, ca, cur, cc);
        dc_read_dx<C, P, R, 1>(ra, ca, cur, cc);
        if (R == 3) dc_read_dx<C, P, R, R == 3 ? 2 : 1>(ra, ca, cur, cc);
      }
    }
    n_here = lds_rd_b32(bufa + (uint32_t)K2::SPLIT_PLANE + cnt_lane + (uint32_t)((HLO * HY + HLO) * 4));
    if (j >= R - 1) {
      float4 a[P];
      float den;
      if (R == 3) {
        den = (c0 + c1) + cc;
#pragma unroll
        for (int pp = 0; pp < P; pp++) {
          a[pp].x = (r0[pp].x + r1[pp].x) + cur[pp].x; a[pp].y = (r0[pp].y + r1[pp].y) + cur[pp].y;
          a[pp].z = (r0[pp].z + r1[pp].z) + cur[pp].z; a[pp].w = (r0[pp].w + r1[pp].w) + cur[pp].w;
        }
      } else {
        den = c1 + cc;
#pragma unroll
        for (int pp = 0; pp < P; pp++) {
          a[pp].x = r1[pp].x + cur[pp].x; a[pp].y = r1[pp].y + cur[pp].y;
          a[pp].z = r1[pp].z + cur[pp].z; a[pp].w = r1[pp].w + cur[pp].w;
        }
      }
      const float inv = den > 0.f ? 1.0f / den : 0.f;
#pragma unroll
      for (int pp = 0; pp < P; pp++)
        lds_wr_b128(abuf + (uint32_t)(grp * RB + pp * C * 4 + li * 16),
                    make_float4(a[pp].x * inv, a[pp].y * inv, a[pp].z * inv, a[pp].w * inv));
      if (li == 0) lds_wr_b32(ncnt + (uint32_t)(grp * 4), col_ok ? n_prev : 0);
    }
#pragma unroll
    for (int pp = 0; pp < P; pp++) { r0[pp] = r1[pp]; r1[pp] = cur[pp]; }
    c0 = c1; c1 = cc;
    n_prev = n_here;
    asm volatile("s_waitcnt lgkmcnt(0)" ::: "memory");
    if (dbg) { const unsigned long long tqb = __builtin_amdgcn_s_memtime(); tq_box += tqb - tqa; tqa = tqb; }
    if (DC_K2_SECOND_ROUND && i - 1 >= R - 1) pairs_of(i - 1, grp + 16);
    if (dbg) { const unsigned long long tqb = __builtin_amdgcn_s_memtime(); tq_pairs += tqb - tqa; }
  }
  if (dbg && lane == 0) {
    unsigned long long *d = dbg + ((size_t)L * 8 + (threadIdx.x >> 6)) * 8;
    const unsigned long long te = __builtin_amdgcn_s_memtime();
    d[0] = te - tq0; d[1] = tq_dma; d[2] = tq_bar; d[3] = tq_box; d[4] = tq_pairs; d[5] = tq_iters; d[6] = nplanes; d[7] = producer ? 1 : 2;
  }
}


template <int OP, int R>
static int launch_k2(const link_dc_buffers_t *b, const link_dc_grid_t &g, const link_elk_desc_t &d, int64_t n,
                     hipStream_t st) {
  using K2 = dc_k2_cfg<OP, R>;
  using K = typename K2::G;
  const int txn = (g.dim[0] + K::TX - 1) / K::TX, tyn = (g.dim[1] + K::TY - 1) / K::TY;
  int zsplit = b->tune.k2_zsplit;
  int k2_pad = b->tune.k2_lds_pad;
  k2_pad = k2_pad < 0 ? 0 : (k2_pad > 4096 ? 4096 : k2_pad);
  const int k2_single = (b->tune.k2_form & 2) ? 1 : 0;
  if (zsplit <= 0) {
    const int64_t tiles = (int64_t)txn * tyn * g.dim[3];
    zsplit = (int)(512 / tiles);
    if (zsplit < 1) zsplit = 1;
  }
  if (zsplit > g.dim[2]) zsplit = g.dim[2];
  const int64_t nwg = (int64_t)txn * tyn * g.dim[3] * zsplit;
  const int64_t grid = (nwg + 7) / 8 * 8;
  const bool two_part = d.op == LINK_OP_COS || d.op == LINK_OP_SIN;
  const bool pair = d.c == 2 * d.cg && two_part;
  const bool div = d.coord_div != 1.0f;
#define LINK_K2S(PP, DD)                                                                                              \
  do {                                                                                                                \
    (void)hipFuncSetAttribute(reinterpret_cast<const void *>(&k_dc_gather_demod_split<OP, R, PP, DD>),                \
                              hipFuncAttributeMaxDynamicSharedMemorySize, K2::SPLIT_LDS_BYTES + k2_pad);        \
    hipLaunchKernelGGL((k_dc_gather_demod_split<OP, R, PP, DD>), dim3((unsigned)grid), dim3(512), K2::SPLIT_LDS_BYTES + k2_pad, st, \
                       b->S, b->cell_n, reinterpret_cast<const int4 *>(b->slots), b->fin, b->w_pos, b->alpha, b->ln_w, \
                       b->ln_b, d.cg, d.coord_div, d.eps, n, g, txn, tyn, zsplit, (int)nwg, b->out, k2_single,       \
                       reinterpret_cast<unsigned long long *>(b->tune.k2_dbg));                                       \
  } while (0)
  const bool own = (b->tune.k2_form & 4) || (!(b->tune.k2_form & 1) && !K2::SPLIT_FITS && R == 3);
  if (own) {
    using KO = dc_k2o_cfg<OP, R>;
#define LINK_K2O(PP, DD)                                                                                              \
  do {                                                                                                                \
    (void)hipFuncSetAttribute(reinterpret_cast<const void *>(&k_dc_gather_demod_own<OP, R, PP, DD>),                  \
                              hipFuncAttributeMaxDynamicSharedMemorySize, KO::LDS_BYTES + k2_pad);                   \
    hipLaunchKernelGGL((k_dc_gather_demod_own<OP, R, PP, DD>), dim3((unsigned)grid), dim3(320), KO::LDS_BYTES + k2_pad, st, b->S, \
                       b->cell_n, reinterpret_cast<const int4 *>(b->slots), b->fin, b->w_pos, b->alpha, b->ln_w,      \
                       b->ln_b, d.cg, d.coord_div, d.eps, n, g, txn, tyn, zsplit, (int)nwg, b->out,                   \
                       reinterpret_cast<unsigned long long *>(b->tune.k2_dbg));                                       \
  } while (0)
    if (pair) { if (div) LINK_K2O(true, true); else LINK_K2O(true, false); }
    else { if (div) LINK_K2O(false, true); else LINK_K2O(false, false); }
#undef LINK_K2O
    return check_launch("link_dc_gather_demod");
  }
  if constexpr (dc_k2q_cfg<OP, R>::FITS) {
    if (pair && !b->alpha && !(b->tune.k2_form & 9) && !k2_single) {
      using KQ = dc_k2q_cfg<OP, R>;
#define LINK_K2Q(DD)                                                                                                  \
  do {                                                                                                                \
    (void)hipFuncSetAttribute(reinterpret_cast<const void *>(&k_dc_gather_demod_quad<OP, R, DD>),                     \
                              hipFuncAttributeMaxDynamicSharedMemorySize, KQ::LDS_BYTES + k2_pad);                   \
    hipLaunchKernelGGL((k_dc_gather_demod_quad<OP, R, DD>), dim3((unsigned)grid), dim3(KQ::THREADS), KQ::LDS_BYTES + k2_pad, st, b->S, \
                       b->cell_n, reinterpret_cast<const int4 *>(b->slots), b->w_pos, b->alpha, b->ln_w, b->ln_b, d.cg, \
                       d.coord_div, d.eps, n, g, txn, tyn, zsplit, (int)nwg, b->out,                                   \
                       reinterpret_cast<unsigned long long *>(b->tune.k2_dbg));                                       \
  } while (0)
      if (div) LINK_K2Q(true); else LINK_K2Q(false);
#undef LINK_K2Q
      return check_launch("link_dc_gather_demod");
    }
  }
  if (!(b->tune.k2_form & 1) && K2::SPLIT_FITS) {
    if (pair) { if (div) LINK_K2S(true, true); else LINK_K2S(true, false); }
    else { if (div) LINK_K2S(false, true); else LINK_K2S(false, false); }
    return check_launch("link_dc_gather_demod");
  }
#undef LINK_K2S
#define LINK_K2(PP, DD)                                                                                               \
  do {                                                                                                                \
    (void)hipFuncSetAttribute(reinterpret_cast<const void *>(&k_dc_gather_demod<OP, R, PP, DD>),                      \
                              hipFuncAttributeMaxDynamicSharedMemorySize, K2::LDS_BYTES);                             \
    hipLaunchKernelGGL((k_dc_gather_demod<OP, R, PP, DD>), dim3((unsigned)grid), dim3(256), K2::LDS_BYTES, st, b->S,  \
                       b->cell_n, reinterpret_cast<const int4 *>(b->slots), b->fin, b->w_pos, b->alpha, b->ln_w,      \
                       b->ln_b, d.cg, d.coord_div, d.eps, n, g, txn, tyn, zsplit, (int)nwg, b->out, k2_single);     \
  } while (0)
  if (pair) { if (div) LINK_K2(true, true); else LINK_K2(true, false); }
  else { if (div) LINK_K2(false, true); else LINK_K2(false, false); }
#undef LINK_K2
  return check_launch("link_dc_gather_demod");
}

int run_premix_modsum(const link_dc_buffers_t *b, const link_dc_grid_t &g, const link_elk_desc_t &d, int64_t n,
                      bool warm, hipStream_t st) {
  if (b->tune.k1_form == 2) {
    if (d.c == 64) return dispatch_k1m_op<64>(b, g, d, n, warm, st);
    if (d.c == 32) return dispatch_k1m_op<32>(b, g, d, n, warm, st);
  }
  switch (d.c) {
    case 16: return dispatch_k1_op<16>(b, g, d, n, warm, st);
    case 32: return dispatch_k1_op<32>(b, g, d, n, warm, st);
    default: return dispatch_k1_op<64>(b, g, d, n, warm, st);
  }
}

int run_demod(const float *A, const float *fin, const int32_t *coords, const int32_t *vcell, const float *w_pos,
              const float *alpha, const float *ln_w, const float *ln_b, const link_elk_desc_t &d,
              const link_dc_grid_t &g, int64_t n, void *out, hipStream_t st) {
  switch (d.c) {
    case 16: launch_dc_demod<4>(d, n, g.vp + 1, st, A, fin, coords, vcell, w_pos, alpha, ln_w, ln_b, out); break;
    case 32: launch_dc_demod<8>(d, n, g.vp + 1, st, A, fin, coords, vcell, w_pos, alpha, ln_w, ln_b, out); break;
    case 64: launch_dc_demod<16>(d, n, g.vp + 1, st, A, fin, coords, vcell, w_pos, alpha, ln_w, ln_b, out); break;
    default: launch_dc_demod<32>(d, n, g.vp + 1, st, A, fin, coords, vcell, w_pos, alpha, ln_w, ln_b, out); break;
  }
  return check_launch("link_dc_demod");
}

int run_gather_demod(const link_dc_buffers_t *b, const link_dc_grid_t &g, const link_elk_desc_t &d, int64_t n,
                     hipStream_t st) {
  if (d.r == 3) {
    switch (d.op) {
      case LINK_OP_COS: return launch_k2<LINK_OP_COS, 3>(b, g, d, n, st);
      case LINK_OP_SIN: return launch_k2<LINK_OP_SIN, 3>(b, g, d, n, st);
      default: return launch_k2<LINK_OP_COSX, 3>(b, g, d, n, st);
    }
  }
  switch (d.op) {
    case LINK_OP_COS: return launch_k2<LINK_OP_COS, 2>(b, g, d, n, st);
    case LINK_OP_SIN: return launch_k2<LINK_OP_SIN, 2>(b, g, d, n, st);
    default: return launch_k2<LINK_OP_COSX, 2>(b, g, d, n, st);
  }
}

}
```

link_amd/csrc/dense_gather.h:

```cpp
#pragma once
#include "dense_common.h"

namespace link {

template <int C, int P, int R>
struct dc_gather_cfg {
  static constexpr int LPR = C / 4;
  static constexpr int NG = 256 / LPR;
  static constexpr int TY = NG >= 64 ? 8 : (NG >= 16 ? 4 : 2);
  static constexpr int TX = NG / TY;
  static constexpr int HLO = (R == 3) ? 1 : 0;
  static constexpr int HX = TX + R - 1, HY = TY + R - 1;
  static constexpr int NCOL = HX * HY;
  static constexpr int RP = P * C / 4;
  static constexpr int NPC = NCOL * RP;
  static constexpr int PASSES = (NPC + 255) / 256;
  static constexpr int EPW = 64;
  static constexpr int NI = PASSES + 1;
  static constexpr int PLANE_BYTES = PASSES * 256 * 16;
  static constexpr int CNT_BYTES = 4 * 256;
  static constexpr int BUF_BYTES = PLANE_BYTES + CNT_BYTES;
  static constexpr int LDS_BYTES = 3 * BUF_BYTES;
  static_assert(NCOL <= 256, "count image: 4 waves x 64 entries");
  static_assert(NCOL * P * C * 4 + 3 * C * 4 < 65536, "ds_read immediate offsets are 16 bit");
};


typedef float v4f_t __attribute__((ext_vector_type(4)));
template <int C, int P, int R, int DX>
__device__ __forceinline__ void dc_read_dx(uint32_t ra, uint32_t ca, float4 (&cur)[P], float &cc) {
  using K = dc_gather_cfg<C, P, R>;
  constexpr int RB = P * C * 4;
#define O_(dy, pp) "i"(((DX * K::HY + (dy)) * RB) + (pp) * C * 4)
#define Q_(dy) "i"((DX * K::HY + (dy)) * 4)
  v4f_t v0, v1, v2, v3, v4, v5, v6, v7, v8;
  int n0, n1, n2 = 0;
  if constexpr (P == 2 && R == 3) {
    asm volatile(
        "ds_read_b128 %0, %9 offset:%c11\n\tds_read_b128 %1, %9 offset:%c12\n\t"
        "ds_read_b128 %2, %9 offset:%c13\n\tds_read_b128 %3, %9 offset:%c14\n\t"
        "ds_read_b128 %4, %9 offset:%c15\n\tds_read_b128 %5, %9 offset:%c16\n\t"
        "ds_read_b32 %6, %10 offset:%c17\n\tds_read_b32 %7, %10 offset:%c18\n\tds_read_b32 %8, %10 offset:%c19\n\t"
        "s_waitcnt lgkmcnt(0)"
        : "=&v"(v0), "=&v"(v1), "=&v"(v2), "=&v"(v3), "=&v"(v4), "=&v"(v5), "=&v"(n0), "=&v"(n1), "=&v"(n2)
        : "v"(ra), "v"(ca), O_(0, 0), O_(0, 1), O_(1, 0), O_(1, 1), O_(2, 0), O_(2, 1), Q_(0), Q_(1), Q_(2)
        : "memory");
    const v4f_t a = (v0 + v2) + v4, b = (v1 + v3) + v5;
    cur[0].x += a.x; cur[0].y += a.y; cur[0].z += a.z; cur[0].w += a.w;
    cur[1].x += b.x; cur[1].y += b.y; cur[1].z += b.z; cur[1].w += b.w;
  } else if constexpr (P == 3 && R == 3) {
    asm volatile(
        "ds_read_b128 %0, %12 offset:%c14\n\tds_read_b128 %1, %12 offset:%c15\n\tds_read_b128 %2, %12 offset:%c16\n\t"
        "ds_read_b128 %3, %12 offset:%c17\n\tds_read_b128 %4, %12 offset:%c18\n\tds_read_b128 %5, %12 offset:%c19\n\t"
        "ds_read_b128 %6, %12 offset:%c20\n\tds_read_b128 %7, %12 offset:%c21\n\tds_read_b128 %8, %12 offset:%c22\n\t"
        "ds_read_b32 %9, %13 offset:%c23\n\tds_read_b32 %10, %13 offset:%c24\n\tds_read_b32 %11, %13 offset:%c25\n\t"
        "s_waitcnt lgkmcnt(0)"
        : "=&v"(v0), "=&v"(v1), "=&v"(v2), "=&v"(v3), "=&v"(v4), "=&v"(v5), "=&v"(v6), "=&v"(v7), "=&v"(v8),
          "=&v"(n0), "=&v"(n1), "=&v"(n2)
        : "v"(ra), "v"(ca), O_(0, 0), O_(0, 1), O_(0, 2), O_(1, 0), O_(1, 1), O_(1, 2), O_(2, 0), O_(2, 1), O_(2, 2),
          Q_(0), Q_(1), Q_(2)
        : "memory");
    const v4f_t a = (v0 + v3) + v6, b = (v1 + v4) + v7, d = (v2 + v5) + v8;
    cur[0].x += a.x; cur[0].y += a.y; cur[0].z += a.z; cur[0].w += a.w;
    cur[1].x += b.x; cur[1].y += b.y; cur[1].z += b.z; cur[1].w += b.w;
    cur[P - 1].x += d.x; cur[P - 1].y += d.y; cur[P - 1].z += d.z; cur[P - 1].w += d.w;
  } else if constexpr (P == 2 && R == 2) {
    asm volatile(
        "ds_read_b128 %0, %6 offset:%c8\n\tds_read_b128 %1, %6 offset:%c9\n\t"
        "ds_read_b128 %2, %6 offset:%c10\n\tds_read_b128 %3, %6 offset:%c11\n\t"
        "ds_read_b32 %4, %7 offset:%c12\n\tds_read_b32 %5, %7 offset:%c13\n\t"
        "s_waitcnt lgkmcnt(0)"
        : "=&v"(v0), "=&v"(v1), "=&v"(v2), "=&v"(v3), "=&v"(n0), "=&v"(n1)
        : "v"(ra), "v"(ca), O_(0, 0), O_(0, 1), O_(1, 0), O_(1, 1), Q_(0), Q_(1)
        : "memory");
    const v4f_t a = v0 + v2, b = v1 + v3;
    cur[0].x += a.x; cur[0].y += a.y; cur[0].z += a.z; cur[0].w += a.w;
    cur[1].x += b.x; cur[1].y += b.y; cur[1].z += b.z; cur[1].w += b.w;
  } else {
    static_assert(P == 3 || P == 2, "parts");
    asm volatile(
        "ds_read_b128 %0, %8 offset:%c10\n\tds_read_b128 %1, %8 offset:%c11\n\tds_read_b128 %2, %8 offset:%c12\n\t"
        "ds_read_b128 %3, %8 offset:%c13\n\tds_read_b128 %4, %8 offset:%c14\n\tds_read_b128 %5, %8 offset:%c15\n\t"
        "ds_read_b32 %6, %9 offset:%c16\n\tds_read_b32 %7, %9 offset:%c17\n\t"
        "s_waitcnt lgkmcnt(0)"
        : "=&v"(v0), "=&v"(v1), "=&v"(v2), "=&v"(v3), "=&v"(v4), "=&v"(v5), "=&v"(n0), "=&v"(n1)
        : "v"(ra), "v"(ca), O_(0, 0), O_(0, 1), O_(0, 2), O_(1, 0), O_(1, 1), O_(1, 2), Q_(0), Q_(1)
        : "memory");
    const v4f_t a = v0 + v3, b = v1 + v4, d = v2 + v5;
    cur[0].x += a.x; cur[0].y += a.y; cur[0].z += a.z; cur[0].w += a.w;
    cur[1].x += b.x; cur[1].y += b.y; cur[1].z += b.z; cur[1].w += b.w;
    cur[P - 1].x += d.x; cur[P - 1].y += d.y; cur[P - 1].z += d.z; cur[P - 1].w += d.w;
  }
  cc += (float)n0 + (float)n1 + (float)n2;
#undef O_
#undef Q_
}

template <int C>
__device__ __forceinline__ void dc_read_plane_p2r3(uint32_t ra, uint32_t ca, float4 (&cur)[2], float &cc) {
  using K = dc_gather_cfg<C, 2, 3>;
  constexpr int RB = 2 * C * 4;
#define O_(dx, dy, pp) "i"((((dx) * K::HY + (dy)) * RB) + (pp) * C * 4)
#define Q_(dx, dy) "i"(((dx) * K::HY + (dy)) * 4)
  v4f_t a0, a1, a2, a3, a4, a5, b0, b1, b2, b3, b4, b5;
  int m0, m1, m2, n0, n1, n2;
  asm volatile(
      "ds_read_b128 %0, %18 offset:%c20\n\tds_read_b128 %1, %18 offset:%c21\n\t"
      "ds_read_b128 %2, %18 offset:%c22\n\tds_read_b128 %3, %18 offset:%c23\n\t"
      "ds_read_b128 %4, %18 offset:%c24\n\tds_read_b128 %5, %18 offset:%c25\n\t"
      "ds_read_b32 %6, %19 offset:%c26\n\tds_read_b32 %7, %19 offset:%c27\n\tds_read_b32 %8, %19 offset:%c28\n\t"
      "ds_read_b128 %9, %18 offset:%c29\n\tds_read_b128 %10, %18 offset:%c30\n\t"
      "ds_read_b128 %11, %18 offset:%c31\n\tds_read_b128 %12, %18 offset:%c32\n\t"
      "ds_read_b128 %13, %18 offset:%c33\n\tds_read_b128 %14, %18 offset:%c34\n\t"
      "ds_read_b32 %15, %19 offset:%c35\n\tds_read_b32 %16, %19 offset:%c36\n\tds_read_b32 %17, %19 offset:%c37\n\t"
      "s_waitcnt lgkmcnt(9)"
      : "=&v"(a0), "=&v"(a1), "=&v"(a2), "=&v"(a3), "=&v"(a4), "=&v"(a5), "=&v"(m0), "=&v"(m1), "=&v"(m2),
        "=&v"(b0), "=&v"(b1), "=&v"(b2), "=&v"(b3), "=&v"(b4), "=&v"(b5), "=&v"(n0), "=&v"(n1), "=&v"(n2)
      : "v"(ra), "v"(ca), O_(0, 0, 0), O_(0, 0, 1), O_(0, 1, 0), O_(0, 1, 1), O_(0, 2, 0), O_(0, 2, 1), Q_(0, 0), Q_(0, 1), Q_(0, 2),
        O_(1, 0, 0), O_(1, 0, 1), O_(1, 1, 0), O_(1, 1, 1), O_(1, 2, 0), O_(1, 2, 1), Q_(1, 0), Q_(1, 1), Q_(1, 2)
      : "memory");
  {
    const v4f_t a = (a0 + a2) + a4, b = (a1 + a3) + a5;
    cur[0].x += a.x; cur[0].y += a.y; cur[0].z += a.z; cur[0].w += a.w;
    cur[1].x += b.x; cur[1].y += b.y; cur[1].z += b.z; cur[1].w += b.w;
    cc += (float)m0 + (float)m1 + (float)m2;
  }
  asm volatile(
      "ds_read_b128 %0, %18 offset:%c20\n\tds_read_b128 %1, %18 offset:%c21\n\t"
      "ds_read_b128 %2, %18 offset:%c22\n\tds_read_b128 %3, %18 offset:%c23\n\t"
      "ds_read_b128 %4, %18 offset:%c24\n\tds_read_b128 %5, %18 offset:%c25\n\t"
      "ds_read_b32 %6, %19 offset:%c26\n\tds_read_b32 %7, %19 offset:%c27\n\tds_read_b32 %8, %19 offset:%c28\n\t"
      "s_waitcnt lgkmcnt(9)"
      : "=&v"(a0), "=&v"(a1), "=&v"(a2), "=&v"(a3), "=&v"(a4), "=&v"(a5), "=&v"(m0), "=&v"(m1), "=&v"(m2),
        "+v"(b0), "+v"(b1), "+v"(b2), "+v"(b3), "+v"(b4), "+v"(b5), "+v"(n0), "+v"(n1), "+v"(n2)
      : "v"(ra), "v"(ca), O_(2, 0, 0), O_(2, 0, 1), O_(2, 1, 0), O_(2, 1, 1), O_(2, 2, 0), O_(2, 2, 1), Q_(2, 0), Q_(2, 1), Q_(2, 2)
      : "memory");
  {
    const v4f_t a = (b0 + b2) + b4, b = (b1 + b3) + b5;
    cur[0].x += a.x; cur[0].y += a.y; cur[0].z += a.z; cur[0].w += a.w;
    cur[1].x += b.x; cur[1].y += b.y; cur[1].z += b.z; cur[1].w += b.w;
    cc += (float)n0 + (float)n1 + (float)n2;
  }
  asm volatile("s_waitcnt lgkmcnt(0)"
               : "+v"(a0), "+v"(a1), "+v"(a2), "+v"(a3), "+v"(a4), "+v"(a5), "+v"(m0), "+v"(m1), "+v"(m2)
               :
               : "memory");
  {
    const v4f_t a = (a0 + a2) + a4, b = (a1 + a3) + a5;
    cur[0].x += a.x; cur[0].y += a.y; cur[0].z += a.z; cur[0].w += a.w;
    cur[1].x += b.x; cur[1].y += b.y; cur[1].z += b.z; cur[1].w += b.w;
    cc += (float)m0 + (float)m1 + (float)m2;
  }
#undef O_
#undef Q_
}


}
```

link_amd/csrc/dense_gather_quad_impl.h:

```cpp
#pragma once
#ifndef DC_K2_MAP
#define DC_K2_MAP 1
#endif

#ifndef DC_K2Q_CW
#define DC_K2Q_CW 3
#endif
#ifndef DC_K2Q_PMAP
#define DC_K2Q_PMAP 1
#endif
#ifndef DC_K2Q_EARLY
#define DC_K2Q_EARLY 1
#endif
#ifndef DC_K2Q_RIM
#define DC_K2Q_RIM 1
#endif
#ifndef DC_K2Q_FMA
#define DC_K2Q_FMA 1
#endif

template <int OP, int R>
struct dc_k2q_cfg {
  using K2 = dc_k2_cfg<OP, R>;
  static constexpr int PAR_OFF = K2::SPLIT_LDS_BYTES;
  static constexpr int MAP_OFF = PAR_OFF + 2 * 64 * 4;
  static constexpr int MAP_BYTES = 64 * 4 + 16;
  static constexpr int LDS_BYTES = MAP_OFF + (DC_K2Q_PMAP ? 3 * MAP_BYTES : 0);
  static constexpr int THREADS = 256 + 64 * (DC_K2Q_CW + (DC_K2Q_PMAP ? 1 : 0));
  static constexpr bool FITS = K2::P == 2 && 2 * LDS_BYTES <= 160 * 1024;
};

__device__ __forceinline__ void lds_rd9_b128(uint32_t ar, uint32_t a0, uint32_t a1, v4f_t &r, v4f_t (&x)[2][4]) {
  asm volatile("ds_read_b128 %0, %9\n\t"
               "ds_read_b128 %1, %10\n\tds_read_b128 %2, %10 offset:64\n\tds_read_b128 %3, %10 offset:128\n\tds_read_b128 %4, %10 offset:192\n\t"
               "ds_read_b128 %5, %11\n\tds_read_b128 %6, %11 offset:64\n\tds_read_b128 %7, %11 offset:128\n\tds_read_b128 %8, %11 offset:192\n\t"
               "s_waitcnt lgkmcnt(0)"
               : "=&v"(r), "=&v"(x[0][0]), "=&v"(x[0][1]), "=&v"(x[0][2]), "=&v"(x[0][3]), "=&v"(x[1][0]), "=&v"(x[1][1]),
                 "=&v"(x[1][2]), "=&v"(x[1][3])
               : "v"(ar), "v"(a0), "v"(a1)
               : "memory");
}
__device__ __forceinline__ void lds_rd8_b128(uint32_t a0, uint32_t a1, v4f_t (&x)[2][4]) {
  asm volatile("ds_read_b128 %0, %8\n\tds_read_b128 %1, %8 offset:64\n\tds_read_b128 %2, %8 offset:128\n\tds_read_b128 %3, %8 offset:192\n\t"
               "ds_read_b128 %4, %9\n\tds_read_b128 %5, %9 offset:64\n\tds_read_b128 %6, %9 offset:128\n\tds_read_b128 %7, %9 offset:192\n\t"
               "s_waitcnt lgkmcnt(0)"
               : "=&v"(x[0][0]), "=&v"(x[0][1]), "=&v"(x[0][2]), "=&v"(x[0][3]), "=&v"(x[1][0]), "=&v"(x[1][1]), "=&v"(x[1][2]),
                 "=&v"(x[1][3])
               : "v"(a0), "v"(a1)
               : "memory");
}
#ifndef DC_K2Q_OVERLAP
#define DC_K2Q_OVERLAP 1
#endif
__device__ __forceinline__ void lds_rd9_b128_rec_first(uint32_t ar, uint32_t a0, uint32_t a1, v4f_t &r, v4f_t (&x)[2][4]) {
  asm volatile("ds_read_b128 %0, %9\n\t"
               "ds_read_b128 %1, %10\n\tds_read_b128 %2, %10 offset:64\n\tds_read_b128 %3, %10 offset:128\n\tds_read_b128 %4, %10 offset:192\n\t"
               "ds_read_b128 %5, %11\n\tds_read_b128 %6, %11 offset:64\n\tds_read_b128 %7, %11 offset:128\n\tds_read_b128 %8, %11 offset:192\n\t"
               "s_waitcnt lgkmcnt(8)"
               : "=&v"(r), "=&v"(x[0][0]), "=&v"(x[0][1]), "=&v"(x[0][2]), "=&v"(x[0][3]), "=&v"(x[1][0]), "=&v"(x[1][1]),
                 "=&v"(x[1][2]), "=&v"(x[1][3])
               : "v"(ar), "v"(a0), "v"(a1)
               : "memory");
}
__device__ __forceinline__ void lds_rd8_b128_nowait(uint32_t a0, uint32_t a1, v4f_t (&x)[2][4]) {
  asm volatile("ds_read_b128 %0, %8\n\tds_read_b128 %1, %8 offset:64\n\tds_read_b128 %2, %8 offset:128\n\tds_read_b128 %3, %8 offset:192\n\t"
               "ds_read_b128 %4, %9\n\tds_read_b128 %5, %9 offset:64\n\tds_read_b128 %6, %9 offset:128\n\tds_read_b128 %7, %9 offset:192"
               : "=&v"(x[0][0]), "=&v"(x[0][1]), "=&v"(x[0][2]), "=&v"(x[0][3]), "=&v"(x[1][0]), "=&v"(x[1][1]), "=&v"(x[1][2]),
                 "=&v"(x[1][3])
               : "v"(a0), "v"(a1)
               : "memory");
}
__device__ __forceinline__ void lds_wait_pieces(v4f_t (&x)[2][4]) {
  asm volatile("s_waitcnt lgkmcnt(0)"
               : "+v"(x[0][0]), "+v"(x[0][1]), "+v"(x[0][2]), "+v"(x[0][3]), "+v"(x[1][0]), "+v"(x[1][1]), "+v"(x[1][2]), "+v"(x[1][3])
               :
               : "memory");
}
template <int N>
__device__ __forceinline__ void lds_rd_counts(uint32_t base, const uint32_t (&off)[N], int (&cn)[N]) {
  if constexpr (N == 5) {
    asm volatile("ds_read_b32 %0, %5\n\tds_read_b32 %1, %6\n\tds_read_b32 %2, %7\n\tds_read_b32 %3, %8\n\tds_read_b32 %4, %9\n\t"
                 "s_waitcnt lgkmcnt(0)"
                 : "=&v"(cn[0]), "=&v"(cn[1]), "=&v"(cn[2]), "=&v"(cn[3]), "=&v"(cn[4])
                 : "v"(base + off[0]), "v"(base + off[1]), "v"(base + off[2]), "v"(base + off[3]), "v"(base + off[4])
                 : "memory");
  } else if constexpr (N == 4) {
    asm volatile("ds_read_b32 %0, %4\n\tds_read_b32 %1, %5\n\tds_read_b32 %2, %6\n\tds_read_b32 %3, %7\n\ts_waitcnt lgkmcnt(0)"
                 : "=&v"(cn[0]), "=&v"(cn[1]), "=&v"(cn[2]), "=&v"(cn[3])
                 : "v"(base + off[0]), "v"(base + off[1]), "v"(base + off[2]), "v"(base + off[3])
                 : "memory");
  } else {
#pragma unroll
    for (int i = 0; i < N; i++) cn[i] = lds_rd_b32(base + off[i]);
  }
}
__device__ __forceinline__ float dc_quad_sum(float v) {
  v += __builtin_bit_cast(float, __builtin_amdgcn_update_dpp(0, __builtin_bit_cast(int, v), 0xB1, 0xF, 0xF, true));
  v += __builtin_bit_cast(float, __builtin_amdgcn_update_dpp(0, __builtin_bit_cast(int, v), 0x4E, 0xF, 0xF, true));
  return v;
}

template <int OP, int R, bool DIV, bool COH = false>
__device__ __forceinline__ void dc_k2q_body(
    const float *__restrict__ S_, const int32_t *__restrict__ cell_n, const int4 *__restrict__ slots,
    const float *__restrict__ w_pos, const float *__restrict__ alpha, const float *__restrict__ ln_w,
    const float *__restrict__ ln_b, int cg, float coord_div, float eps, int64_t n, const link_dc_grid_t &g, int txn, int tyn,
    int zsplit, int nwg, void *__restrict__ out, unsigned long long *__restrict__ dbg, const int bid, const unsigned tidx) {
  using K2 = dc_k2_cfg<OP, R>;
  using KQ = dc_k2q_cfg<OP, R>;
  DC_PROF_PTR(dbg);
  unsigned long long tq0 = dbg ? DC_NOW() : 0, tq_dma = 0, tq_bar = 0, tq_work = 0;
  int tq_rounds = 0;
  using K = typename K2::G;
  constexpr int C = 64, P = 2, TY = K::TY, TX = K::TX, HY = K::HY, HLO = K::HLO;
  constexpr int RB = P * C * 4;
  static_assert(K2::P == 2, "two-part rows");
  extern __shared__ __attribute__((aligned(16))) char lds[];
  const bool producer = tidx < 256;
  const int tid = tidx & 255, lane = tid & 63, wave = __builtin_amdgcn_readfirstlane((tidx & 255) >> 6);
  const int per = (nwg + 7) >> 3;
  const int L = (bid & 7) * per + (bid >> 3);
  if (L >= nwg) return;
  int t = L;
  const int zseg = t % zsplit; t /= zsplit;
#if DC_K2_MAP
  const int per_b = txn * tyn;
  const int b = t / per_b;
  int tt2 = t - b * per_b;
  const int H = (tyn + 1) >> 1;
  int tx, ty;
  if (tt2 < txn * H) { tx = tt2 / H; ty = tt2 - tx * H; }
  else { tt2 -= txn * H; const int H2 = tyn - H; tx = tt2 / H2; ty = H + tt2 - tx * H2; }
#else
  const int ty = t % tyn; t /= tyn;
  const int tx = t % txn;
  const int b = t / txn;
#endif
  const int Dx = g.dim[0], Dy = g.dim[1], Dz = g.dim[2];
  const int PDx = g.pdim[0], PDy = g.pdim[1], PDz = g.pdim[2];
  const int x0 = tx * TX, y0 = ty * TY;
  const int zs = (int)(((long long)Dz * zseg) / zsplit), ze = (int)(((long long)Dz * (zseg + 1)) / zsplit);
  if (zs >= ze) return;
  const int nplanes = (ze - zs) + R - 1;
  const int pz0 = zs + 1 - HLO;
  const uint32_t lds_base = (uint32_t)(size_t)(__attribute__((address_space(3))) char *)lds;
  const uint32_t abuf0 = lds_base + K2::SPLIT_ABUF_OFF, ncnt0 = lds_base + K2::SPLIT_NCNT_OFF;
  if (tidx < 128) {
    float *par = reinterpret_cast<float *>(lds + KQ::PAR_OFF);
    par[tidx] = tidx < 64 ? ln_w[tidx] : ln_b[tidx - 64];
  }
  if (producer) {
    auto col_cell0 = [&](int hx, int hy) {
      int px = x0 + 1 - HLO + hx, py = y0 + 1 - HLO + hy;
      px = px < PDx - 1 ? px : PDx - 1;
      py = py < PDy - 1 ? py : PDy - 1;
      return (uint32_t)(((b * PDx + px) * PDy + py) * PDz);
    };
    uint32_t src_off[K::PASSES], cnt_off[K::PASSES];
#pragma unroll
    for (int i = 0; i < K::PASSES; i++) {
      int pid = i * 256 + tid;
      if (pid >= K::NPC) pid = K::NPC - 1;
      const int col = pid / K::RP, pcs = pid % K::RP;
      src_off[i] = col_cell0(col / HY, col % HY) * (uint32_t)RB + (uint32_t)pcs * 16u;
      cnt_off[i] = (uint32_t)col * 4u;
    }
    uint32_t cnt_cell0;
    {
      int e = wave * 64 + lane;
      if (e >= K::NCOL) e = K::NCOL - 1;
      cnt_cell0 = col_cell0(e / HY, e % HY);
    }
    const __amdgpu_buffer_rsrc_t r_S = dc_rsrc(S_, (uint32_t)((g.vp + 1) * RB));
    auto cnt_slot = [&](int plane, int pm3) -> uint32_t {
      (void)plane;
      return (uint32_t)(pm3 * K2::SPLIT_BUF_BYTES + K2::SPLIT_PLANE);
    };
    auto issue_cnt = [&](int plane, int pm3) {
      int pz = pz0 + plane;
      pz = pz < PDz - 1 ? pz : PDz - 1;
      const int32_t *csrc = cell_n + cnt_cell0 + pz;
      __builtin_amdgcn_global_load_lds((const __attribute__((address_space(1))) void *)csrc,
                                       (__attribute__((address_space(3))) void *)(lds + cnt_slot(plane, pm3) + wave * 256), 4, 0, COH ? 16 : 0);
    };
    uint32_t rec_cell0;
    int rec_k;
    {
      const int piece = wave * 16 + (lane & 15);
      const int col = piece >> 2;
      rec_k = piece & 3;
      rec_cell0 = col_cell0(col / TY + HLO, col % TY + HLO);
    }
    const char *Sb = reinterpret_cast<const char *>(S_);
    auto issue = [&](int plane, int pm3, bool) {
      int pz = pz0 + plane;
      pz = pz < PDz - 1 ? pz : PDz - 1;
      char *buf = lds + pm3 * K2::SPLIT_BUF_BYTES;
#pragma unroll
      for (int i = 0; i < K::PASSES; i++) {
        const bool surplus = (i * 256 + wave * 64) >= K::NPC;
        const int ii = surplus ? 0 : i;
        const char *src = Sb + (size_t)(surplus ? src_off[0] : src_off[i]) + (size_t)pz * RB;
        __builtin_amdgcn_global_load_lds((const __attribute__((address_space(1))) void *)src,
                                         (__attribute__((address_space(3))) void *)(buf + (ii * 256 + wave * 64) * 16), 16, 0, COH ? 16 : 0);
      }
      issue_cnt(plane, pm3);
      int po = pz0 + plane - (R - 1) + HLO;
      po = po < 0 ? 0 : (po < PDz - 1 ? po : PDz - 1);
      const int4 *rsrc = slots + ((size_t)(rec_cell0 + po) * DC_INL + rec_k);
      if (lane < 16)
        __builtin_amdgcn_global_load_lds((const __attribute__((address_space(1))) void *)rsrc,
                                         (__attribute__((address_space(3))) void *)(lds + K2::SPLIT_REC_OFF + (plane & 3) * K2::REC_BYTES + wave * 256), 16, 0, COH ? 16 : 0);
    };
    const int grp = tid >> 4, li = tid & 15;
    const bool rim_t = DC_K2Q_RIM && (y0 + TY > Dy) && (x0 + TX <= Dx);
    const int ix = rim_t ? grp % TX : grp / TY, iy = rim_t ? grp / TX : grp % TY;
    const int cell = ix * TY + iy;
    const bool col_ok = (x0 + ix < Dx) && (y0 + iy < Dy);
    const bool wave_has = (DC_K2Q_RIM && DC_K2Q_PMAP) ? __any(col_ok) : true;
    if (!wave_has && li == 0) {
      lds_wr_b32(ncnt0 + (uint32_t)(cell * 4), 0);
      lds_wr_b32(ncnt0 + (uint32_t)(K2::NG * 4 + cell * 4), 0);
    }
    const uint32_t row_lane = (uint32_t)((ix * HY + iy) * RB + li * 16);
    const uint32_t cnt_lane = (uint32_t)((ix * HY + iy) * 4);
    float4 r0[P], r1[P];
    float c0 = 0.f, c1 = 0.f;
    int n_prev = 0;
#pragma unroll
    for (int pp = 0; pp < P; pp++) r0[pp] = r1[pp] = make_float4(0.f, 0.f, 0.f, 0.f);
    issue(0, 0, false);
    if (nplanes > 1) issue(1, 1, false);
    int m3 = 0, m3p2 = 2;
    for (int i = 0; i <= nplanes; i++, m3 = m3 == 2 ? 0 : m3 + 1, m3p2 = m3p2 == 2 ? 0 : m3p2 + 1) {
      unsigned long long tqa = dbg ? DC_NOW() : 0;
      if (i < nplanes) {
        if (i + 1 < nplanes) wait_vmcnt<K2::NI>(); else wait_vmcnt<0>();
      }
      asm volatile("s_waitcnt lgkmcnt(0)" ::: "memory");
      if (dbg) { const unsigned long long tqb = DC_NOW(); tq_dma += tqb - tqa; tqa = tqb; }
      asm volatile("s_barrier" ::: "memory");
      if (dbg) { const unsigned long long tqb = DC_NOW(); tq_bar += tqb - tqa; tqa = tqb; }
      if (i >= nplanes) break;
      if (i + 2 < nplanes) issue(i + 2, m3p2, true);
      const uint32_t bufa = lds_base + (uint32_t)(m3 * K2::SPLIT_BUF_BYTES);
      if (!wave_has) continue;
      float4 cur[P];
      float cc = 0.f;
#pragma unroll
      for (int pp = 0; pp < P; pp++) cur[pp] = make_float4(0.f, 0.f, 0.f, 0.f);
      {
        const uint32_t ra = bufa + row_lane, ca = lds_base + cnt_slot(i, m3) + cnt_lane;
        if constexpr (R == 3) {
          dc_read_plane_p2r3<C>(ra, ca, cur, cc);
        } else {
          dc_read_dx<C, P, R, 0>(ra, ca, cur, cc);
          dc_read_dx<C, P, R, 1>(ra, ca, cur, cc);
        }
      }
      const int n_here = lds_rd_b32(lds_base + cnt_slot(i, m3) + cnt_lane + (uint32_t)((HLO * HY + HLO) * 4));
      if (i >= R - 1) {
        const uint32_t abuf = abuf0 + (uint32_t)((i & 1) * K2::NG * RB), ncnt = ncnt0 + (uint32_t)((i & 1) * K2::NG * 4);
        float4 a[P];
        float den;
        if (R == 3) {
          den = (c0 + c1) + cc;
#pragma unroll
          for (int pp = 0; pp < P; pp++) {
            a[pp].x = (r0[pp].x + r1[pp].x) + cur[pp].x; a[pp].y = (r0[pp].y + r1[pp].y) + cur[pp].y;
            a[pp].z = (r0[pp].z + r1[pp].z) + cur[pp].z; a[pp].w = (r0[pp].w + r1[pp].w) + cur[pp].w;
          }
        } else {
          den = c1 + cc;
#pragma unroll
          for (int pp = 0; pp < P; pp++) {
            a[pp].x = r1[pp].x + cur[pp].x; a[pp].y = r1[pp].y + cur[pp].y;
            a[pp].z = r1[pp].z + cur[pp].z; a[pp].w = r1[pp].w + cur[pp].w;
          }
        }
        const float inv = den > 0.f ? 1.0f / den : 0.f;
#pragma unroll
        for (int pp = 0; pp < P; pp++)
          lds_wr_b128(abuf + (uint32_t)(cell * RB + pp * C * 4 + li * 16),
                      make_float4(a[pp].x * inv, a[pp].y * inv, a[pp].z * inv, a[pp].w * inv));
        if (li == 0) lds_wr_b32(ncnt + (uint32_t)(cell * 4), col_ok ? n_prev : 0);
      }
#pragma unroll
      for (int pp = 0; pp < P; pp++) { r0[pp] = r1[pp]; r1[pp] = cur[pp]; }
      c0 = c1; c1 = cc;
      n_prev = n_here;
      if (dbg) { asm volatile("s_waitcnt lgkmcnt(0)" ::: "memory"); tq_work += DC_NOW() - tqa; }
    }
    if (dbg && lane == 0) {
      unsigned long long *d = dbg + ((size_t)L * 8 + (tidx >> 6)) * 8;
      d[0] = DC_NOW() - tq0; d[1] = tq_dma; d[2] = tq_bar; d[3] = tq_work; d[4] = tq0; d[5] = 0; d[6] = nplanes; d[7] = 1;
    }
    return;
  }
  constexpr int CW = DC_K2Q_CW, SLOTS = 16 * CW;
  if (DC_K2Q_PMAP && wave == CW) {
    int m3 = 0;
    for (int i = 0; i <= nplanes; i++, m3 = m3 == 2 ? 0 : m3 + 1) {
      asm volatile("s_barrier" ::: "memory");
      if (i >= nplanes) break;
      const uint32_t ca = lds_base + (uint32_t)(m3 * K2::SPLIT_BUF_BYTES + K2::SPLIT_PLANE);
      int run = 0, c_ = 0, start = 0;
#define Q_(k) "i"(((((k) / TY) + HLO) * HY + ((k) % TY) + HLO) * 4)
#define DC_MAP4(K0)                                                                                                          \
      {                                                                                                                      \
        int n0, n1, n2, n3;                                                                                                  \
        asm volatile("ds_read_b32 %0, %4 offset:%c5\n\tds_read_b32 %1, %4 offset:%c6\n\tds_read_b32 %2, %4 offset:%c7\n\t"     \
                     "ds_read_b32 %3, %4 offset:%c8\n\ts_waitcnt lgkmcnt(0)"                                                \
                     : "=&v"(n0), "=&v"(n1), "=&v"(n2), "=&v"(n3)                                                            \
                     : "v"(ca), Q_(K0), Q_(K0 + 1), Q_(K0 + 2), Q_(K0 + 3)                                                   \
                     : "memory");                                                                                            \
        const int nn[4] = {n0, n1, n2, n3};                                                                                  \
        _Pragma("unroll") for (int kk = 0; kk < 4; kk++) {                                                                   \
          const int k = K0 + kk;                                                                                             \
          const bool okk = (x0 + k / TY < Dx) && (y0 + k % TY < Dy);    \
          run += okk ? nn[kk] : 0;                                                                                           \
          if (k < 15) {                                                                                                      \
            const bool le = run <= lane;                                                                                     \
            c_ += le ? 1 : 0;                                                                                                \
            start = le ? run : start;                                                                                        \
          }                                                                                                                  \
        }                                                                                                                    \
      }
      DC_MAP4(0) DC_MAP4(4) DC_MAP4(8) DC_MAP4(12)
#undef DC_MAP4
#undef Q_
      const uint32_t mb = lds_base + (uint32_t)(KQ::MAP_OFF + m3 * KQ::MAP_BYTES);
      lds_wr_b32(mb + (uint32_t)(lane * 4), (c_ << 12) | ((lane - start) & 4095));
      if (lane == 0) lds_wr_b32(mb + 256u, run);
      asm volatile("s_waitcnt lgkmcnt(0)" ::: "memory");
    }
    return;
  }
  const int q = lane & 3, li16 = lane & 15;
  const int qd = wave * 16 + (lane >> 2);
  const __amdgpu_buffer_rsrc_t r_out = dc_rsrc(out, (uint32_t)(n * C * IO_BYTES));
  float w0[2][4], w1[2][4], w2[2][4];
#pragma unroll
  for (int j = 0; j < 2; j++)
#pragma unroll
    for (int e = 0; e < 4; e++) {
      const int tc = (16 * j + 4 * q + e) % cg;
      w0[j][e] = w_pos[3 * tc + 0]; w1[j][e] = w_pos[3 * tc + 1]; w2[j][e] = w_pos[3 * tc + 2];
    }
  const uint32_t par = lds_base + (uint32_t)KQ::PAR_OFF + (uint32_t)(q * 16);
  bool slow_k = false;
  if (DC_THETA_BOUND) {
    float ax, ay, az;
    dc_coord_absmax(g, DIV ? coord_div : 1.0f, ax, ay, az);
    bool b_ = false;
#pragma unroll
    for (int j = 0; j < 2; j++)
#pragma unroll
      for (int e = 0; e < 4; e++) b_ |= dc_theta_leaves_fast_range(ax, ay, az, w0[j][e], w1[j][e], w2[j][e], 1.0f);
    slow_k = __any(b_);
  }
  int m3p1 = 1;
  for (int i = 0; i <= nplanes; i++, m3p1 = m3p1 == 2 ? 0 : m3p1 + 1) {
    unsigned long long tqa = dbg ? DC_NOW() : 0;
    asm volatile("s_barrier" ::: "memory");
    if (dbg) { const unsigned long long tqb = DC_NOW(); tq_bar += tqb - tqa; tqa = tqb; }
    const int jp = i - 1;
    if (jp < R - 1 || jp >= nplanes) continue;
    const uint32_t abuf = abuf0 + (uint32_t)((jp & 1) * K2::NG * RB), ncnt = ncnt0 + (uint32_t)((jp & 1) * K2::NG * 4);
    const uint32_t recb = lds_base + (uint32_t)(K2::SPLIT_REC_OFF + (jp & 3) * K2::REC_BYTES);
    const int po = pz0 + jp - (R - 1) + HLO;
    int Tv, m0 = 0;
    uint32_t mb = 0;
    if (DC_K2Q_PMAP) {
      mb = lds_base + (uint32_t)(KQ::MAP_OFF + m3p1 * KQ::MAP_BYTES);
      int tv_;
      asm volatile("ds_read_b32 %0, %2\n\tds_read_b32 %1, %3 offset:256\n\ts_waitcnt lgkmcnt(0)"
                   : "=&v"(m0), "=&v"(tv_) : "v"(mb + (uint32_t)(qd * 4)), "v"(mb) : "memory");
      Tv = __builtin_amdgcn_readfirstlane(tv_);
    } else {
      Tv = 0;
    }
    int e_[16];
    if (!DC_K2Q_PMAP) {
      int incl = lds_rd_b32(ncnt + (uint32_t)(li16 * 4));
      incl += __builtin_amdgcn_update_dpp(0, incl, 0x111, 0xF, 0xF, true);
      incl += __builtin_amdgcn_update_dpp(0, incl, 0x112, 0xF, 0xF, true);
      incl += __builtin_amdgcn_update_dpp(0, incl, 0x114, 0xF, 0xF, true);
      incl += __builtin_amdgcn_update_dpp(0, incl, 0x118, 0xF, 0xF, true);
#pragma unroll
      for (int k = 0; k < 16; k++) e_[k] = __builtin_amdgcn_readlane(incl, k);
      Tv = e_[15];
    }
    for (int base = 0; base < Tv; base += SLOTS) {
      if (DC_K2Q_EARLY && base + wave * 16 >= Tv) break;
      if (dbg) tq_rounds++;
      const bool valid = base + qd < Tv;
      int c, k;
      if (DC_K2Q_PMAP) {
        if (Tv <= 64) {
          const int mm = base == 0 ? m0 : lds_rd_b32(mb + (uint32_t)((valid ? base + qd : 0) * 4));
          c = valid ? (mm >> 12) : 0;
          k = valid ? (mm & 4095) : 0;
        } else {
          const int v = valid ? base + qd : 0;
          int run = 0, start = 0;
          c = 0;
          for (int kk = 0; kk < 15; kk++) {
            run += lds_rd_b32(ncnt + (uint32_t)(kk * 4));
            const bool le = run <= v;
            c += le ? 1 : 0;
            start = le ? run : start;
          }
          k = v - start;
        }
      } else {
        const int v = valid ? base + qd : Tv - 1;
        c = 0;
        int start = 0;
#pragma unroll
        for (int kk = 0; kk < 15; kk++) {
          const bool le = e_[kk] <= v;
          c += le ? 1 : 0;
          start = le ? e_[kk] : start;
        }
        k = v - start;
      }
      v4f_t rq, Av[2][4];
      if (DC_K2Q_OVERLAP)
        lds_rd9_b128_rec_first(recb + (uint32_t)((c * DC_INL + (k < DC_INL ? k : 0)) * 16), abuf + (uint32_t)(c * RB + q * 16),
                               abuf + (uint32_t)(c * RB + C * 4 + q * 16), rq, Av);
      else
        lds_rd9_b128(recb + (uint32_t)((c * DC_INL + (k < DC_INL ? k : 0)) * 16), abuf + (uint32_t)(c * RB + q * 16),
                     abuf + (uint32_t)(c * RB + C * 4 + q * 16), rq, Av);
      int4 rec = make_int4(__float_as_int(rq.x), __float_as_int(rq.y), __float_as_int(rq.z), __float_as_int(rq.w));
      if (k >= DC_INL) {
        const int pcell = ((b * PDx + x0 + c / TY + 1) * PDy + y0 + c % TY + 1) * PDz + po;
        rec = ld16i_c<COH>(dc_rsrc(slots, (uint32_t)((int64_t)g.vp * g.k * 16)), slots, dc_slot(g, pcell, k));
      }
      float x = (float)rec.x, y = (float)rec.y, z = (float)rec.z;
      if (DIV) { x = x / coord_div; y = y / coord_div; z = z / coord_div; }
      float th[2][4], sn[2][4], cs[2][4];
      bool big = false;
#pragma unroll
      for (int j = 0; j < 2; j++)
#pragma unroll
        for (int e = 0; e < 4; e++) {
          th[j][e] = fmaf(z, w2[j][e], fmaf(y, w1[j][e], x * w0[j][e]));
        }
      if (!DC_THETA_BOUND) {
        float mx = fmaxf(fmaxf(fabsf(th[0][0]), fabsf(th[0][1])), fabsf(th[0][2]));
        mx = fmaxf(fmaxf(mx, fabsf(th[0][3])), fabsf(th[1][0]));
        mx = fmaxf(fmaxf(mx, fabsf(th[1][1])), fabsf(th[1][2]));
        mx = fmaxf(mx, fabsf(th[1][3]));
        big = valid && !(mx < 32768.0f);
      }
      if (__builtin_expect(DC_THETA_BOUND ? slow_k : __any(big), 0)) {
#pragma unroll
        for (int j = 0; j < 2; j++)
#pragma unroll
          for (int e = 0; e < 4; e++) sincos_nocall(th[j][e], sn[j][e], cs[j][e]);
      } else {
#pragma unroll
        for (int j = 0; j < 2; j++)
#pragma unroll
          for (int e = 0; e < 4; e++) sincos_small(th[j][e], sn[j][e], cs[j][e]);
      }
      if (DC_K2Q_OVERLAP) lds_wait_pieces(Av);
      float nv[4][4], s = 0.f;
#pragma unroll
      for (int j = 0; j < 4; j++)
#pragma unroll
        for (int e = 0; e < 4; e++) {
          const float A0 = Av[0][j][e], A1 = Av[1][j][e], cc_ = cs[j & 1][e], ss_ = sn[j & 1][e];
          if (DC_K2Q_FMA) {
            nv[j][e] = fmaf(OP == LINK_OP_SIN ? -A1 : A1, ss_, A0 * cc_);
          } else {
            if (OP == LINK_OP_SIN) nv[j][e] = __fsub_rn(__fmul_rn(A0, cc_), __fmul_rn(A1, ss_));
            else nv[j][e] = __fadd_rn(__fmul_rn(A0, cc_), __fmul_rn(A1, ss_));
          }
          s += nv[j][e];
        }
      v4f_t gwb[2][4];
      if (DC_K2Q_OVERLAP) lds_rd8_b128_nowait(par, par + 256u, gwb);
      s = dc_quad_sum(s);
      const float mean = s * (1.0f / C);
      float qq = 0.f;
#pragma unroll
      for (int j = 0; j < 4; j++)
#pragma unroll
        for (int e = 0; e < 4; e++) {
          const float d = nv[j][e] - mean;
          qq += d * d;
        }
      qq = dc_quad_sum(qq);
      const float rs = __builtin_amdgcn_rsqf(qq * (1.0f / C) + eps);
      if (DC_K2Q_OVERLAP) lds_wait_pieces(gwb); else lds_rd8_b128(par, par + 256u, gwb);
#pragma unroll
      for (int j = 0; j < 4; j++) {
        float4 o;
        o.x = (nv[j][0] - mean) * rs * gwb[0][j][0] + gwb[1][j][0]; o.y = (nv[j][1] - mean) * rs * gwb[0][j][1] + gwb[1][j][1];
        o.z = (nv[j][2] - mean) * rs * gwb[0][j][2] + gwb[1][j][2]; o.w = (nv[j][3] - mean) * rs * gwb[0][j][3] + gwb[1][j][3];
        io_st4(r_out, (uint32_t)rec.w * (uint32_t)C + (uint32_t)(16 * j + 4 * q), valid, o);
      }
    }
    if (dbg) tq_work += DC_NOW() - tqa;
  }
  if (dbg && lane == 0) {
    unsigned long long *d = dbg + ((size_t)L * 8 + (tidx >> 6)) * 8;
    d[0] = DC_NOW() - tq0; d[1] = tq0; d[2] = tq_bar; d[3] = 0; d[4] = tq_work; d[5] = tq_rounds; d[6] = nplanes; d[7] = 2;
  }
}

template <int OP, int R, bool DIV>
__global__ void __launch_bounds__(256 + 64 * (DC_K2Q_CW + (DC_K2Q_PMAP ? 1 : 0)), 4) k_dc_gather_demod_quad(
    const float *__restrict__ S_, const int32_t *__restrict__ cell_n, const int4 *__restrict__ slots,
    const float *__restrict__ w_pos, const float *__restrict__ alpha, const float *__restrict__ ln_w,
    const float *__restrict__ ln_b, int cg, float coord_div, float eps, int64_t n, link_dc_grid_t g, int txn, int tyn,
    int zsplit, int nwg, void *__restrict__ out, unsigned long long *__restrict__ dbg) {
  dc_k2q_body<OP, R, DIV>(S_, cell_n, slots, w_pos, alpha, ln_w, ln_b, cg, coord_div, eps, n, g, txn, tyn, zsplit, nwg, out, dbg,
                          (int)blockIdx.x, threadIdx.x);
}
```

Baseline: 2.963 billion.

## Pack rim tiles of the gather-demod kernel into half-populated paired workgroups

Moves the K2 tile enumeration into a shared header with a tile descriptor and an occupancy bitmask. When a grid dimension leaves a single-column remainder (dim mod 4 == 1), two such rim strips are packed into one 4x4 workgroup instead of launching mostly-empty tiles. The goal is to cut workgroups that do little work. The cost is a more complex tile decode, per-cell half offsets, and extra readfirstlane scalarisation. A host tile-map query function is also added. The packed layout is enabled in the batch kernel, but the standalone quad launch keeps it off by default through the DC_K2Q_PACK_LAUNCH switch.

```diff
diff --git a/include/link_amd.h b/include/link_amd.h
--- a/include/link_amd.h
+++ b/include/link_amd.h
@@ -396,6 +396,7 @@
                   int32_t io_dtype, void *stream);
 int link_dc_gather_demod(const link_dc_buffers_t *buf , const link_dc_grid_t *g ,
                          const link_elk_desc_t *desc , int64_t n, void *stream);
+int64_t link_dc_k2_tile_map(const link_dc_grid_t *g , int32_t zsplit, int32_t *out , int64_t cap);
 int link_elk_core_dense_forward(const link_dc_buffers_t *buf , const link_dc_grid_t *g ,
                                 const link_elk_desc_t *desc , int64_t n, int32_t build_index,
                                 void *stream);
diff --git a/link_amd/_lib.py b/link_amd/_lib.py
--- a/link_amd/_lib.py
+++ b/link_amd/_lib.py
@@ -238,6 +238,7 @@
     "link_dc_premix_modsum": (c_int, [POINTER(LinkDcBuffers), POINTER(LinkDcGrid), POINTER(LinkElkDesc), c_int64,
                                       c_int32, c_void_p]),
     "link_dc_gather_demod": (c_int, [POINTER(LinkDcBuffers), POINTER(LinkDcGrid), POINTER(LinkElkDesc), c_int64, c_void_p]),
+    "link_dc_k2_tile_map": (c_int64, [POINTER(LinkDcGrid), c_int32, c_void_p, c_int64]),
     "link_dc_demod": (c_int, [c_void_p] * 8 + [POINTER(LinkElkDesc), POINTER(LinkDcGrid), c_int64, c_void_p, c_int32,
                               c_void_p]),
     "link_block_ctx_create": (c_int, [POINTER(c_void_p)]),
diff --git a/link_amd/csrc/dense_batch_impl.h b/link_amd/csrc/dense_batch_impl.h
--- a/link_amd/csrc/dense_batch_impl.h
+++ b/link_amd/csrc/dense_batch_impl.h
@@ -170,7 +170,7 @@
   dc_bt_frames_t fr;
   dc_bt_par_t p;
   link_dc_grid_t g;
-  int nframes, txn, tyn, zsplit, nwg, k1_target;
+  int nframes, zsplit, nwg, k1_target;
   int32_t *sync;
 };
 
@@ -208,8 +208,8 @@
       const link_dc_grid_t g = a->g;
       unsigned tidx = threadIdx.x;
       asm volatile("" : "+v"(tidx));
-      dc_k2q_body<OP, R, false, true>(a->fr.f[f].S, a->fr.f[f].cell_n, a->fr.f[f].slots, a->p.w_pos, nullptr, a->p.ln_w, a->p.ln_b, a->p.cg,
-                                      1.0f, a->p.eps, a->fr.f[f].n, g, a->txn, a->tyn, a->zsplit, a->nwg, a->fr.f[f].out, nullptr, bid, tidx);
+      dc_k2q_body<OP, R, false, true, DC_K2Q_PACK && R == 3>(a->fr.f[f].S, a->fr.f[f].cell_n, a->fr.f[f].slots, a->p.w_pos, nullptr, a->p.ln_w, a->p.ln_b, a->p.cg,
+                                      1.0f, a->p.eps, a->fr.f[f].n, g, a->zsplit, a->nwg, a->fr.f[f].out, nullptr, bid, tidx);
     }
     if (threadIdx.x == CTL_THREAD) {
       const unsigned long long tq1 = DC_BT_PROF ? __builtin_amdgcn_s_memrealtime() : 0;
@@ -247,11 +247,11 @@
   int cpw = (int)((vi + (int64_t)k1_wgs * K1::NW * rpw - 1) / ((int64_t)k1_wgs * K1::NW * rpw));
   if (cpw < 1) cpw = 1;
   const int k1_target = (int)((vi + cpw - 1) / cpw);
-  const int txn = (g.dim[0] + KG::TX - 1) / KG::TX, tyn = (g.dim[1] + KG::TY - 1) / KG::TY;
   static const int zs_env = [] { const char *e = getenv("LINK_DC_BATCH_ZSPLIT"); const int v = e ? atoi(e) : 1; return v < 1 ? 1 : (v > 8 ? 8 : v); }();
   int zsplit = zs_env;
   if (zsplit > g.dim[2]) zsplit = g.dim[2];
-  const int64_t nwg = (int64_t)txn * tyn * g.dim[3] * zsplit;
+  static_assert(KG::TX == DC_K2_T && KG::TY == DC_K2_T, "dense_k2_tiles.h enumerates 4 x 4 tiles");
+  const int64_t nwg = dc_k2_workgroups(g.dim[0], g.dim[1], g.dim[3], zsplit, DC_K2Q_PACK && R == 3);
   if (nwg > (1 << 20)) return LINK_ERR_ARG;
   int wpf = (int)((nmax + 255) / 256);
   if (wpf < 1) wpf = 1;
@@ -265,7 +265,7 @@
   hipLaunchKernelGGL((k_dc_batch_k1<OP, 2>), dim3((unsigned)k1_wgs), dim3(64 * K1::NW), k1_lds, c.sa, fr, p, g, nframes, cpw, k1_target, wpf, sync);
   rc = check_launch("link_elk_core_dense_forward_batch (K1)");
   if (rc != LINK_OK) return rc;
-  const dc_bt_k2_args_t a2{fr, p, g, nframes, txn, tyn, zsplit, (int)nwg, k1_target, sync};
+  const dc_bt_k2_args_t a2{fr, p, g, nframes, zsplit, (int)nwg, k1_target, sync};
   static_assert(sizeof(dc_bt_k2_args_t) <= 4096, "kernel arguments");
   hipLaunchKernelGGL((k_dc_batch_k2<OP, R>), dim3((unsigned)c.cus), dim3(KQ::THREADS), k2_lds, c.sb, a2);
   return check_launch("link_elk_core_dense_forward_batch (K2)");
diff --git a/link_amd/csrc/dense_fused.hip b/link_amd/csrc/dense_fused.hip
--- a/link_amd/csrc/dense_fused.hip
+++ b/link_amd/csrc/dense_fused.hip
@@ -291,6 +291,29 @@
                                     const int32_t *slots, int32_t step, int32_t *nbr, void *stream) {
   return dc_neighbor_map_run(coords, n, g, cnt, slots, step, nbr, nullptr, nullptr, link::S(stream));
 }
+extern "C" int64_t link_dc_k2_tile_map(const link_dc_grid_t *g, int32_t zsplit, int32_t *out, int64_t cap) {
+  if (!g || g->dim[0] <= 0 || g->dim[1] <= 0 || g->dim[2] <= 0 || g->dim[3] <= 0 || cap < 0 || (cap > 0 && !out)) return LINK_ERR_ARG;
+  const int Dx = g->dim[0], Dy = g->dim[1], Dz = g->dim[2];
+  const bool pack = zsplit > 0 ? DC_K2Q_PACK : DC_K2Q_PACK && DC_K2Q_PACK_LAUNCH;
+  if (zsplit <= 0) {
+    zsplit = (int)(512 / ((int64_t)link::dc_k2_tiles_per_item(Dx, Dy, pack) * g->dim[3]));
+    if (zsplit < 1) zsplit = 1;
+  }
+  if (zsplit > Dz) zsplit = Dz;
+  const int64_t nwg = link::dc_k2_workgroups(Dx, Dy, g->dim[3], zsplit, pack);
+  if (nwg > (1 << 20)) return LINK_ERR_ARG;
+  for (int64_t L = 0; L < nwg && (L + 1) * 50 <= cap; L++) {
+    const link::dc_k2_tile_t t = link::dc_k2_tile((int)L, Dx, Dy, Dz, zsplit, pack);
+    int32_t *o = out + L * 50;
+    for (int k = 0; k < 16; k++) {
+      const int ix = k / link::DC_K2_T, iy = k % link::DC_K2_T, h = t.half_of_cell(ix, iy);
+      const bool real = t.cell_real(k);
+      o[3 * k] = real ? t.b : -1; o[3 * k + 1] = real ? t.ox(h) + ix : -1; o[3 * k + 2] = real ? t.oy(h) + iy : -1;
+    }
+    o[48] = t.zs; o[49] = t.ze;
+  }
+  return nwg;
+}
 namespace link {
 int dc_neighbor_map_count_run(const int32_t *coords, int64_t n, const link_dc_grid_t *g, const uint32_t *cnt, const int32_t *slots,
                               int32_t step, int32_t *nbr, int32_t *wg_counts, int32_t *row_info, hipStream_t st) {
diff --git a/link_amd/csrc/dense_fused_impl.h b/link_amd/csrc/dense_fused_impl.h
--- a/link_amd/csrc/dense_fused_impl.h
+++ b/link_amd/csrc/dense_fused_impl.h
@@ -823,17 +823,20 @@
   int k2_pad = b->tune.k2_lds_pad;
   k2_pad = k2_pad < 0 ? 0 : (k2_pad > 4096 ? 4096 : k2_pad);
   const int k2_single = (b->tune.k2_form & 2) ? 1 : 0;
-  if (zsplit <= 0) {
-    const int64_t tiles = (int64_t)txn * tyn * g.dim[3];
-    zsplit = (int)(512 / tiles);
-    if (zsplit < 1) zsplit = 1;
-  }
-  if (zsplit > g.dim[2]) zsplit = g.dim[2];
-  const int64_t nwg = (int64_t)txn * tyn * g.dim[3] * zsplit;
-  const int64_t grid = (nwg + 7) / 8 * 8;
   const bool two_part = d.op == LINK_OP_COS || d.op == LINK_OP_SIN;
   const bool pair = d.c == 2 * d.cg && two_part;
   const bool div = d.coord_div != 1.0f;
+  const bool own = (b->tune.k2_form & 4) || (!(b->tune.k2_form & 1) && !K2::SPLIT_FITS && R == 3);
+  const bool quad = dc_k2q_cfg<OP, R>::FITS && !own && pair && !b->alpha && !(b->tune.k2_form & 9) && !k2_single;
+  const bool pack = quad && DC_K2Q_PACK && DC_K2Q_PACK_LAUNCH && R == 3;
+  const int64_t tiles = (int64_t)dc_k2_tiles_per_item(g.dim[0], g.dim[1], pack) * g.dim[3];
+  if (zsplit <= 0) {
+    zsplit = (int)(512 / tiles);
+    if (zsplit < 1) zsplit = 1;
+  }
+  if (zsplit > g.dim[2]) zsplit = g.dim[2];
+  const int64_t nwg = tiles * zsplit;
+  const int64_t grid = (nwg + 7) / 8 * 8;
 #define LINK_K2S(PP, DD)                                                                                              \
   do {                                                                                                                \
     (void)hipFuncSetAttribute(reinterpret_cast<const void *>(&k_dc_gather_demod_split<OP, R, PP, DD>),                \
@@ -843,7 +846,6 @@
                        b->ln_b, d.cg, d.coord_div, d.eps, n, g, txn, tyn, zsplit, (int)nwg, b->out, k2_single,       \
                        reinterpret_cast<unsigned long long *>(b->tune.k2_dbg));                                       \
   } while (0)
-  const bool own = (b->tune.k2_form & 4) || (!(b->tune.k2_form & 1) && !K2::SPLIT_FITS && R == 3);
   if (own) {
     using KO = dc_k2o_cfg<OP, R>;
 #define LINK_K2O(PP, DD)                                                                                              \
@@ -861,7 +863,7 @@
     return check_launch("link_dc_gather_demod");
   }
   if constexpr (dc_k2q_cfg<OP, R>::FITS) {
-    if (pair && !b->alpha && !(b->tune.k2_form & 9) && !k2_single) {
+    if (quad) {
       using KQ = dc_k2q_cfg<OP, R>;
 #define LINK_K2Q(DD)                                                                                                  \
   do {                                                                                                                \
@@ -869,7 +871,7 @@
                               hipFuncAttributeMaxDynamicSharedMemorySize, KQ::LDS_BYTES + k2_pad);                   \
     hipLaunchKernelGGL((k_dc_gather_demod_quad<OP, R, DD>), dim3((unsigned)grid), dim3(KQ::THREADS), KQ::LDS_BYTES + k2_pad, st, b->S, \
                        b->cell_n, reinterpret_cast<const int4 *>(b->slots), b->w_pos, b->alpha, b->ln_w, b->ln_b, d.cg, \
-                       d.coord_div, d.eps, n, g, txn, tyn, zsplit, (int)nwg, b->out,                                   \
+                       d.coord_div, d.eps, n, g, zsplit, (int)nwg, b->out,                                             \
                        reinterpret_cast<unsigned long long *>(b->tune.k2_dbg));                                       \
   } while (0)
       if (div) LINK_K2Q(true); else LINK_K2Q(false);
diff --git a/link_amd/csrc/dense_gather.h b/link_amd/csrc/dense_gather.h
--- a/link_amd/csrc/dense_gather.h
+++ b/link_amd/csrc/dense_gather.h
@@ -1,5 +1,6 @@
 #pragma once
 #include "dense_common.h"
+#include "dense_k2_tiles.h"
 
 namespace link {
 
diff --git a/link_amd/csrc/dense_gather_quad_impl.h b/link_amd/csrc/dense_gather_quad_impl.h
--- a/link_amd/csrc/dense_gather_quad_impl.h
+++ b/link_amd/csrc/dense_gather_quad_impl.h
@@ -1,8 +1,4 @@
 #pragma once
-#ifndef DC_K2_MAP
-#define DC_K2_MAP 1
-#endif
-
 #ifndef DC_K2Q_CW
 #define DC_K2Q_CW 3
 #endif
@@ -100,11 +96,11 @@
   return v;
 }
 
-template <int OP, int R, bool DIV, bool COH = false>
+template <int OP, int R, bool DIV, bool COH = false, bool PACKED = false>
 __device__ __forceinline__ void dc_k2q_body(
     const float *__restrict__ S_, const int32_t *__restrict__ cell_n, const int4 *__restrict__ slots,
     const float *__restrict__ w_pos, const float *__restrict__ alpha, const float *__restrict__ ln_w,
-    const float *__restrict__ ln_b, int cg, float coord_div, float eps, int64_t n, const link_dc_grid_t &g, int txn, int tyn,
+    const float *__restrict__ ln_b, int cg, float coord_div, float eps, int64_t n, const link_dc_grid_t &g,
     int zsplit, int nwg, void *__restrict__ out, unsigned long long *__restrict__ dbg, const int bid, const unsigned tidx) {
   using K2 = dc_k2_cfg<OP, R>;
   using KQ = dc_k2q_cfg<OP, R>;
@@ -121,25 +117,19 @@
   const int per = (nwg + 7) >> 3;
   const int L = (bid & 7) * per + (bid >> 3);
   if (L >= nwg) return;
-  int t = L;
-  const int zseg = t % zsplit; t /= zsplit;
-#if DC_K2_MAP
-  const int per_b = txn * tyn;
-  const int b = t / per_b;
-  int tt2 = t - b * per_b;
-  const int H = (tyn + 1) >> 1;
-  int tx, ty;
-  if (tt2 < txn * H) { tx = tt2 / H; ty = tt2 - tx * H; }
-  else { tt2 -= txn * H; const int H2 = tyn - H; tx = tt2 / H2; ty = H + tt2 - tx * H2; }
-#else
-  const int ty = t % tyn; t /= tyn;
-  const int tx = t % txn;
-  const int b = t / txn;
-#endif
-  const int Dx = g.dim[0], Dy = g.dim[1], Dz = g.dim[2];
+  static_assert(TX == DC_K2_T && TY == DC_K2_T, "dense_k2_tiles.h enumerates 4 x 4 tiles");
+  constexpr bool PACK = PACKED;
+  static_assert(!PACK || R == 3, "2 x (1 + R - 1) image columns are the 6 of a tile for R = 3 only");
+  const int Dx = g.dim[0], Dy = g.dim[1];
   const int PDx = g.pdim[0], PDy = g.pdim[1], PDz = g.pdim[2];
-  const int x0 = tx * TX, y0 = ty * TY;
-  const int zs = (int)(((long long)Dz * zseg) / zsplit), ze = (int)(((long long)Dz * (zseg + 1)) / zsplit);
+  int Lv = L;
+  asm volatile("" : "+v"(Lv));
+  dc_k2_tile_t tile = dc_k2_tile(Lv, Dx, Dy, g.dim[2], zsplit, PACK);
+  tile.b = __builtin_amdgcn_readfirstlane(tile.b); tile.zs = __builtin_amdgcn_readfirstlane(tile.zs);
+  tile.ze = __builtin_amdgcn_readfirstlane(tile.ze); tile.x0 = __builtin_amdgcn_readfirstlane(tile.x0);
+  tile.y0 = __builtin_amdgcn_readfirstlane(tile.y0); tile.kind = __builtin_amdgcn_readfirstlane(tile.kind);
+  tile.real = (unsigned)__builtin_amdgcn_readfirstlane((int)tile.real);
+  const int b = tile.b, zs = tile.zs, ze = tile.ze;
   if (zs >= ze) return;
   const int nplanes = (ze - zs) + R - 1;
   const int pz0 = zs + 1 - HLO;
@@ -151,7 +141,8 @@
   }
   if (producer) {
     auto col_cell0 = [&](int hx, int hy) {
-      int px = x0 + 1 - HLO + hx, py = y0 + 1 - HLO + hy;
+      const int h = tile.half_of_col(hx, hy);
+      int px = tile.ox(h) + 1 - HLO + hx, py = tile.oy(h) + 1 - HLO + hy;
       px = px < PDx - 1 ? px : PDx - 1;
       py = py < PDy - 1 ? py : PDy - 1;
       return (uint32_t)(((b * PDx + px) * PDy + py) * PDz);
@@ -213,10 +204,10 @@
                                          (__attribute__((address_space(3))) void *)(lds + K2::SPLIT_REC_OFF + (plane & 3) * K2::REC_BYTES + wave * 256), 16, 0, COH ? 16 : 0);
     };
     const int grp = tid >> 4, li = tid & 15;
-    const bool rim_t = DC_K2Q_RIM && (y0 + TY > Dy) && (x0 + TX <= Dx);
+    const bool rim_t = tile.kind == 2 || (DC_K2Q_RIM && tile.kind == 0 && tile.cell_real((TX - 1) * TY) && !tile.cell_real(TY - 1));
     const int ix = rim_t ? grp % TX : grp / TY, iy = rim_t ? grp / TX : grp % TY;
     const int cell = ix * TY + iy;
-    const bool col_ok = (x0 + ix < Dx) && (y0 + iy < Dy);
+    const bool col_ok = tile.cell_real(cell);
     const bool wave_has = (DC_K2Q_RIM && DC_K2Q_PMAP) ? __any(col_ok) : true;
     if (!wave_has && li == 0) {
       lds_wr_b32(ncnt0 + (uint32_t)(cell * 4), 0);
@@ -299,6 +290,7 @@
   }
   constexpr int CW = DC_K2Q_CW, SLOTS = 16 * CW;
   if (DC_K2Q_PMAP && wave == CW) {
+    const unsigned real = tile.real;
     int m3 = 0;
     for (int i = 0; i <= nplanes; i++, m3 = m3 == 2 ? 0 : m3 + 1) {
       asm volatile("s_barrier" ::: "memory");
@@ -317,7 +309,7 @@
         const int nn[4] = {n0, n1, n2, n3};                                                                                  \
         _Pragma("unroll") for (int kk = 0; kk < 4; kk++) {                                                                   \
           const int k = K0 + kk;                                                                                             \
-          const bool okk = (x0 + k / TY < Dx) && (y0 + k % TY < Dy);    \
+          const bool okk = (real >> k) & 1u;    \
           run += okk ? nn[kk] : 0;                                                                                           \
           if (k < 15) {                                                                                                      \
             const bool le = run <= lane;                                                                                     \
@@ -359,6 +351,8 @@
       for (int e = 0; e < 4; e++) b_ |= dc_theta_leaves_fast_range(ax, ay, az, w0[j][e], w1[j][e], w2[j][e], 1.0f);
     slow_k = __any(b_);
   }
+  const int ovf_cell0[2] = {((b * PDx + tile.ox(0) + 1) * PDy + tile.oy(0) + 1) * PDz, ((b * PDx + tile.ox(1) + 1) * PDy + tile.oy(1) + 1) * PDz};
+  const unsigned ovf_half = tile.kind == 1 ? 0xFF00u : (tile.kind == 2 ? 0xCCCCu : 0u);
   int m3p1 = 1;
   for (int i = 0; i <= nplanes; i++, m3p1 = m3p1 == 2 ? 0 : m3p1 + 1) {
     unsigned long long tqa = dbg ? DC_NOW() : 0;
@@ -434,7 +428,7 @@
                      abuf + (uint32_t)(c * RB + C * 4 + q * 16), rq, Av);
       int4 rec = make_int4(__float_as_int(rq.x), __float_as_int(rq.y), __float_as_int(rq.z), __float_as_int(rq.w));
       if (k >= DC_INL) {
-        const int pcell = ((b * PDx + x0 + c / TY + 1) * PDy + y0 + c % TY + 1) * PDz + po;
+        const int pcell = ((ovf_half >> c) & 1 ? ovf_cell0[1] : ovf_cell0[0]) + ((c / TY) * PDy + c % TY) * PDz + po;
         rec = ld16i_c<COH>(dc_rsrc(slots, (uint32_t)((int64_t)g.vp * g.k * 16)), slots, dc_slot(g, pcell, k));
       }
       float x = (float)rec.x, y = (float)rec.y, z = (float)rec.z;
@@ -515,8 +509,8 @@
 __global__ void __launch_bounds__(256 + 64 * (DC_K2Q_CW + (DC_K2Q_PMAP ? 1 : 0)), 4) k_dc_gather_demod_quad(
     const float *__restrict__ S_, const int32_t *__restrict__ cell_n, const int4 *__restrict__ slots,
     const float *__restrict__ w_pos, const float *__restrict__ alpha, const float *__restrict__ ln_w,
-    const float *__restrict__ ln_b, int cg, float coord_div, float eps, int64_t n, link_dc_grid_t g, int txn, int tyn,
+    const float *__restrict__ ln_b, int cg, float coord_div, float eps, int64_t n, link_dc_grid_t g,
     int zsplit, int nwg, void *__restrict__ out, unsigned long long *__restrict__ dbg) {
-  dc_k2q_body<OP, R, DIV>(S_, cell_n, slots, w_pos, alpha, ln_w, ln_b, cg, coord_div, eps, n, g, txn, tyn, zsplit, nwg, out, dbg,
+  dc_k2q_body<OP, R, DIV, false, DC_K2Q_PACK && DC_K2Q_PACK_LAUNCH && R == 3>(S_, cell_n, slots, w_pos, alpha, ln_w, ln_b, cg, coord_div, eps, n, g, zsplit, nwg, out, dbg,
                           (int)blockIdx.x, threadIdx.x);
 }
diff --git a/link_amd/csrc/dense_k2_tiles.h b/link_amd/csrc/dense_k2_tiles.h
--- /dev/null
+++ b/link_amd/csrc/dense_k2_tiles.h
@@ -0,0 +1,100 @@
+#pragma once
+#include <stdint.h>
+
+#ifndef DC_K2_MAP
+#define DC_K2_MAP 1
+#endif
+#ifndef DC_K2Q_PACK
+#define DC_K2Q_PACK 1
+#endif
+#ifndef DC_K2Q_PACK_LAUNCH
+#define DC_K2Q_PACK_LAUNCH 0
+#endif
+
+namespace link {
+
+constexpr int DC_K2_T = 4;
+
+struct dc_k2_tile_t {
+  int b;
+  int zs, ze;
+  int x0, y0;
+  int kind;
+  unsigned real;
+  __host__ __device__ bool cell_real(int cell) const { return (real >> cell) & 1u; }
+  __host__ __device__ int half_of_col(int hx, int hy) const { return kind == 1 ? (hx >= 3) : (kind == 2 ? (hy >= 3) : 0); }
+  __host__ __device__ int half_of_cell(int ix, int iy) const { return half_of_col(ix + 1, iy + 1); }
+  __host__ __device__ int ox(int h) const { return x0 + (h ? (kind == 1 ? -(DC_K2_T - 1) : DC_K2_T) : 0); }
+  __host__ __device__ int oy(int h) const { return y0 + (h ? (kind == 1 ? DC_K2_T : -(DC_K2_T - 1)) : 0); }
+};
+
+__host__ __device__ inline bool dc_k2_packs(int dim, bool pack) { return DC_K2_MAP && pack && (dim & (DC_K2_T - 1)) == 1; }
+
+__host__ __device__ inline int dc_k2_tiles_per_item(int Dx, int Dy, bool pack) {
+  const int txn = (Dx + DC_K2_T - 1) / DC_K2_T, tyn = (Dy + DC_K2_T - 1) / DC_K2_T;
+  const int px = dc_k2_packs(Dx, pack), py = dc_k2_packs(Dy, pack);
+  const int itx = txn - px, ity = tyn - py;
+  return itx * ity + (px ? (tyn + 1) >> 1 : 0) + (py ? (itx + 1) >> 1 : 0);
+}
+__host__ __device__ inline int64_t dc_k2_workgroups(int Dx, int Dy, int items, int zsplit, bool pack) {
+  return (int64_t)dc_k2_tiles_per_item(Dx, Dy, pack) * items * zsplit;
+}
+
+__host__ __device__ inline bool dc_k2_cell_real(const dc_k2_tile_t &t, int Dx, int Dy, int ix, int iy, bool pack) {
+  if (t.kind == 1 && ix != 0 && ix != DC_K2_T - 1) return false;
+  if (t.kind == 2 && iy != 0 && iy != DC_K2_T - 1) return false;
+  const int h = t.half_of_cell(ix, iy);
+  const int xl = t.kind == 2 && dc_k2_packs(Dx, pack) ? Dx - 1 : Dx;
+  return t.ox(h) + ix < xl && t.oy(h) + iy < Dy;
+}
+
+__host__ __device__ inline dc_k2_tile_t dc_k2_tile(int L, int Dx, int Dy, int Dz, int zsplit, bool pack) {
+  dc_k2_tile_t o;
+  int t = L;
+  const int zseg = t % zsplit; t /= zsplit;
+  o.zs = (int)(((long long)Dz * zseg) / zsplit);
+  o.ze = (int)(((long long)Dz * (zseg + 1)) / zsplit);
+  const int txn = (Dx + DC_K2_T - 1) / DC_K2_T, tyn = (Dy + DC_K2_T - 1) / DC_K2_T;
+  o.kind = 0;
+#if DC_K2_MAP
+  const int px = dc_k2_packs(Dx, pack), py = dc_k2_packs(Dy, pack);
+  const int itx = txn - px, ity = tyn - py;
+  const int nxp = px ? (tyn + 1) >> 1 : 0, nyp = py ? (itx + 1) >> 1 : 0;
+  const int per_b = itx * ity + nxp + nyp;
+  o.b = t / per_b;
+  t -= o.b * per_b;
+  const int H = (ity + 1) >> 1, H2 = ity - H;
+  const int nxp1 = nxp < ((H + 1) >> 1) ? nxp : ((H + 1) >> 1);
+  int tx = 0, ty = 0, strip = 0;
+  if (t < itx * H) {
+    tx = t / H; ty = t - tx * H;
+  } else if ((t -= itx * H) < nxp1) {
+    o.kind = 1; strip = 2 * t;
+  } else {
+    t -= nxp1;
+    const int n2 = itx * H2 + nyp;
+    if (t < n2) {
+      const int B2 = 2 * H2 + py;
+      const int blk = t / B2, r = t - blk * B2;
+      const int ncol = itx - 2 * blk >= 2 ? 2 : 1;
+      if (r < ncol * H2) { const int c = r / H2; tx = 2 * blk + c; ty = H + r - c * H2; }
+      else { o.kind = 2; strip = 2 * blk; }
+    } else {
+      o.kind = 1; strip = 2 * (nxp1 + t - n2);
+    }
+  }
+  if (o.kind == 1) { o.x0 = Dx - 1; o.y0 = strip * DC_K2_T; }
+  else if (o.kind == 2) { o.x0 = strip * DC_K2_T; o.y0 = Dy - 1; }
+  else { o.x0 = tx * DC_K2_T; o.y0 = ty * DC_K2_T; }
+#else
+  (void)pack;
+  const int ty = t % tyn; t /= tyn;
+  o.x0 = (t % txn) * DC_K2_T; o.y0 = ty * DC_K2_T;
+  o.b = t / txn;
+#endif
+  o.real = 0;
+  for (int k = 0; k < DC_K2_T * DC_K2_T; k++) o.real |= dc_k2_cell_real(o, Dx, Dy, k / DC_K2_T, k % DC_K2_T, pack) ? 1u << k : 0u;
+  return o;
+}
+
+}
```

Result: slower. 2.923 billion (-1.4%).
